# JunweiLiang/Multiverse

Measured on AMD Instinct MI355X. Metric: trajectories/sec (8-obs/12-pred, multi-scale 18x32+9x16 grid, greedy forward), higher is better.
Workload: dtype f16x3 (fp32 operands as two pre-scaled fp16 planes, fp32 accumulate and state; winograd F(3,3) over image rows on pre-transformed operands, 1.67 fp16 MFMAs issued per fp32 product over the gate kernels; error vs fp64 within 2x of the fp32-MFMA path's -- asserted under checkpoint-like dynamic range (; 1 GPU; BASELINE configs[1]: multi-scale 18x32+9x16 (scene 36x64x11), batch 64/GPU, fp32 forward-only, beam 1, obs 8 / pred 12; gate convolution on the fp16 matrix pipe (f16x3 split, fp32-class error); batch_per_gpu=64, global_batch=64, obs_len=8, pred_len=12, parallelism=batch-sharded x1, no data-path collective

## Files before the change

include/multiverse_hip.h:

```cpp
#ifndef MULTIVERSE_HIP_H_
#define MULTIVERSE_HIP_H_

#include <stdint.h>

#ifdef __cplusplus
extern "C" {
#endif

#define MV_MAX_SCALES 2
#define MV_ABI_VERSION 5

typedef struct mv_engine* mv_handle;

typedef struct mv_config {
  int32_t abi_version;
  int32_t batch_size;
  int32_t obs_len;
  int32_t max_pred_len;
  int32_t scene_h, scene_w, scene_class;
  int32_t scene_conv_dim, scene_conv_kernel;
  int32_t emb_size;
  int32_t hidden_size;
  int32_t convlstm_kernel;
  int32_t num_scales;
// ... 140 lines not shown
int  mv_run_score_resident(mv_handle h);
int  mv_download_scores(mv_handle h, mv_score_outputs* out);
int  mv_time_score_resident(mv_handle h, int32_t iters, float* ms_out);

int  mv_train_init(mv_handle h, const mv_train_config* tc);
int  mv_train_step(mv_handle h, const mv_inputs* in, const mv_targets* tg,
                   mv_losses* out);
int  mv_train_forward_backward(mv_handle h, const mv_inputs* in,
                               const mv_targets* tg, mv_losses* out);
int  mv_upload_targets(mv_handle h, const mv_targets* tg);
int  mv_grad_buffer(mv_handle h, float** device_ptr, int64_t* elems);
int  mv_train_apply(mv_handle h, float grad_scale);
#define MV_COMM_ID_BYTES 128
int  mv_comm_unique_id(uint8_t* id_out );
int  mv_allreduce_init(mv_handle h, int32_t rank, int32_t world,
                       const uint8_t* unique_id );
int  mv_allreduce_info(mv_handle h, int32_t* rank, int32_t* world, int32_t* buckets,
                       double* bytes);
int  mv_attack_begin(mv_handle h);
int  mv_attack_end(mv_handle h);
int  mv_set_scene_feat(mv_handle h, const float* scene_feat);
int  mv_get_scene_feat(mv_handle h, float* out);
int  mv_get_scene_grad(mv_handle h, float* out);
int  mv_attack_step(mv_handle h, float epsilon, float step);
int  mv_scene_mix(mv_handle h, const float* other, float weight);
int  mv_get_sample_losses(mv_handle h, int32_t scale, float* out);
int  mv_set_label_mixup(mv_handle h, const int32_t* const* obs_labels2,
                        const int32_t* const* pred_labels2, float weight,
                        const float* sample_weight);
int  mv_clear_label_mixup(mv_handle h);
int  mv_get_grad(mv_handle h, const char* tf_name, float* out, int64_t capacity_elems);
int  mv_get_global_step(mv_handle h, int64_t* step);
int  mv_set_global_step(mv_handle h, int64_t step);
int  mv_set_dropout_seed(mv_handle h, uint32_t seed);
int  mv_get_opt_scalars(mv_handle h, float* beta1_power, float* beta2_power);
int  mv_set_opt_scalars(mv_handle h, float beta1_power, float beta2_power);
int  mv_get_opt_slot(mv_handle h, const char* tf_name, int32_t slot, float* out,
                     int64_t capacity_elems);
int  mv_set_opt_slot(mv_handle h, const char* tf_name, int32_t slot,
                     const float* data, int64_t elems);

int  mv_set_compute_mode(mv_handle h, int32_t mode);

int  mv_set_graph_mode(mv_handle h, int32_t enabled);

int  mv_set_profiling(mv_handle h, int32_t enabled);
int  mv_reset_kernel_stats(mv_handle h);
int  mv_num_kernel_stats(mv_handle h);
int  mv_kernel_stat(mv_handle h, int32_t i, char* name_out, int32_t name_cap,
                    int64_t* launches, double* total_ms, double* flops,
                    double* bytes);
int  mv_kernel_stat_dense_flops(mv_handle h, int32_t i, double* flops_dense);
int  mv_kernel_stat_mfma_flops(mv_handle h, int32_t i, double* flops_mfma);
int  mv_time_greedy_resident(mv_handle h, int32_t iters, float* ms_out);
int  mv_time_beam_resident(mv_handle h, int32_t iters, float* ms_out);

int  mv_op_convlstm_step(int device, const float* x, const float* c,
                         const float* h, const float* kernel,
                         const float* biases, int32_t M, int32_t H, int32_t W,
                         int32_t Cx, int32_t C, float* c_out, float* h_out);
int  mv_op_convlstm_step16(int device, int32_t variant, const float* x, const float* c,
                           const float* h, const float* kernel, const float* biases,
                           int32_t M, int32_t H, int32_t W, int32_t Cx, int32_t C,
                           float* c_out, float* h_out, float* h16_out);
int  mv_op_gnn(int device, const float* h, const float* scene_mean, int32_t M,
               int32_t H, int32_t W, int32_t C, int32_t D, float* out);
int  mv_op_hidden2grid(int device, const float* h, const float* w, int32_t M,
                       int32_t H, int32_t W, int32_t C, int32_t P, float* out);
int  mv_op_beam_step(int device, const float* logits, const float* prev_logprob,
                     int32_t N, int32_t B, int32_t K, int32_t time,
                     int32_t diverse, float gamma, int32_t fix_num_timestep,
                     float* new_logprob, int32_t* ids, int32_t* parents);

int  mv_op_sbs_step(int device, const float* logits, const float* prev_phi,
                    const float* prev_logprob, const float* prev_gumbel, int32_t N, int32_t B,
                    int32_t K, int32_t t, float temperature, uint32_t seed, float* new_phi,
                    float* new_logprob, float* new_gumbel, int32_t* ids, int32_t* parents);

int  mv_op_sample_step(int device, const float* logits , int32_t R, int32_t S,
                       int32_t K, int32_t t, float temperature, uint32_t seed, int32_t top_k,
                       float top_p, int32_t floor, int32_t* ids, float* lp, float* qlp,
                       uint8_t* keep );

int  mv_op_convlstm_bwd(int device, const float* x, const float* c, const float* h,
                        const float* kernel, const float* biases,
                        const float* dh_new, const float* dc_new, int32_t M,
                        int32_t H, int32_t W, int32_t Cx, int32_t C, float* dx,
                        float* dh, float* dc, float* dkernel, float* dbiases);
int  mv_op_gnn_bwd(int device, const float* h, const float* scene_mean,
                   const float* g, int32_t M, int32_t H, int32_t W, int32_t C,
                   int32_t D, float* dh, float* dscene_mean);

#ifdef __cplusplus
}
#endif
#endif
```

multiverse_amd/_lib.py:

```python

from __future__ import annotations

import ctypes as C
import os

import numpy as np

MV_MAX_SCALES = 2
MV_ABI_VERSION = 5

_HERE = os.path.dirname(os.path.abspath(__file__))
LIB_PATH = os.path.join(_HERE, "libmultiverse_hip.so")

EXPORTED_SYMBOLS = [
    "mv_create", "mv_destroy", "mv_last_error", "mv_abi_version",
    "mv_set_param", "mv_get_param", "mv_num_params", "mv_param_info",
    "mv_forward_greedy", "mv_forward_beam",
    "mv_upload_inputs", "mv_run_greedy_resident", "mv_run_beam_resident",
    "mv_synchronize", "mv_download_outputs", "mv_download_beam_outputs",
    "mv_set_graph_mode", "mv_set_compute_mode", "mv_set_profiling", "mv_reset_kernel_stats", "mv_num_kernel_stats",
    "mv_kernel_stat", "mv_kernel_stat_dense_flops", "mv_kernel_stat_mfma_flops",
    "mv_time_greedy_resident",
    "mv_time_beam_resident",
    "mv_op_convlstm_step", "mv_op_convlstm_step16", "mv_op_gnn", "mv_op_hidden2grid", "mv_op_beam_step",
    "mv_train_init", "mv_train_step", "mv_train_forward_backward",
    "mv_upload_targets", "mv_grad_buffer", "mv_train_apply", "mv_get_grad", "mv_get_global_step",
    "mv_set_global_step", "mv_get_opt_slot", "mv_set_opt_slot",
    "mv_set_dropout_seed", "mv_get_opt_scalars", "mv_set_opt_scalars",
    "mv_comm_unique_id", "mv_allreduce_init", "mv_allreduce_info",
    "mv_attack_begin", "mv_attack_end", "mv_set_scene_feat", "mv_get_scene_feat",
    "mv_get_scene_grad", "mv_attack_step", "mv_scene_mix", "mv_get_sample_losses",
    "mv_set_label_mixup", "mv_clear_label_mixup",
    "mv_op_convlstm_bwd", "mv_op_gnn_bwd",
    "mv_set_grid_centers", "mv_upload_inputs_compact", "mv_upload_targets_compact",
    "mv_pipeline_create", "mv_submit_greedy", "mv_collect_greedy",
    "mv_decode_trajectories", "mv_beam_occupancy", "mv_download_beam_ids",
    "mv_set_pred_lengths", "mv_last_forward_gate_rows", "mv_set_sampling",
    "mv_score_futures", "mv_upload_score_futures", "mv_run_score_resident",
    "mv_download_scores", "mv_time_score_resident",
    "mv_set_sampling_mode", "mv_download_beam_gumbels", "mv_op_sbs_step",
    "mv_set_sampling_truncation", "mv_download_beam_proposal_logprobs", "mv_op_sample_step",
]


class MvError(RuntimeError):
  pass


class mv_config(C.Structure):
  _fields_ = [
      ("abi_version", C.c_int32),
      ("batch_size", C.c_int32),
      ("obs_len", C.c_int32),
      ("max_pred_len", C.c_int32),
      ("scene_h", C.c_int32), ("scene_w", C.c_int32), ("scene_class", C.c_int32),
      ("scene_conv_dim", C.c_int32), ("scene_conv_kernel", C.c_int32),
      ("emb_size", C.c_int32),
      ("hidden_size", C.c_int32),
      ("convlstm_kernel", C.c_int32),
      ("num_scales", C.c_int32),
      ("grid_h", C.c_int32 * MV_MAX_SCALES),
      ("grid_w", C.c_int32 * MV_MAX_SCALES),
      ("use_grid", C.c_int32 * MV_MAX_SCALES),
      ("use_gnn", C.c_int32),
      ("beam_size", C.c_int32),
      ("diverse_beam", C.c_int32),
      ("diverse_gamma", C.c_float),
      ("fix_num_timestep", C.c_int32),
      ("class_feedback_dense", C.c_int32),
      ("use_single_decoder", C.c_int32),
      ("simaug_graph", C.c_int32),
      ("activation", C.c_int32),
  ]


_fp = C.POINTER(C.c_float)
_ip = C.POINTER(C.c_int32)


class mv_inputs(C.Structure):
  _fields_ = [
      ("obs_scene", _ip),
      ("scene_feat", _fp),
      ("num_scene_frames", C.c_int32),
      ("pred_len", C.c_int32),
      ("grid_obs_labels", _ip * MV_MAX_SCALES),
      ("grid_obs_regress", _fp * MV_MAX_SCALES),
  ]


_dp = C.POINTER(C.c_double)
_u8p = C.POINTER(C.c_uint8)


class mv_inputs_compact(C.Structure):
  _fields_ = [
      ("obs_scene", _ip),
      ("scene_feat_u8", _u8p),
      ("num_scene_frames", C.c_int32),
      ("pred_len", C.c_int32),
      ("grid_obs_labels", _ip * MV_MAX_SCALES),
      ("obs_xy", _dp),
      ("num_rows", C.c_int32),
  ]


class mv_targets_compact(C.Structure):
  _fields_ = [
      ("grid_pred_labels", _ip * MV_MAX_SCALES),
      ("pred_xy", _dp),
      ("num_rows", C.c_int32),
  ]


class mv_outputs(C.Structure):
  _fields_ = [
      ("grid_pred_class", _fp * MV_MAX_SCALES),
      ("grid_pred_reg", _fp * MV_MAX_SCALES),
  ]


class mv_beam_outputs(C.Structure):
  _fields_ = [
      ("best_beam", _fp), ("grid_reg", _fp), ("logits", _fp), ("ids", _ip),
# ... 14 lines not shown
      ("optimizer", C.c_int32),
      ("init_lr", C.c_float), ("emb_lr", C.c_float),
      ("use_cosine_lr", C.c_int32),
      ("has_decay", C.c_int32), ("learning_rate_decay", C.c_float),
      ("decay_steps", C.c_int32), ("max_steps", C.c_int32),
      ("do_clip", C.c_int32), ("clip_gradient_norm", C.c_float),
      ("wd", C.c_float),
      ("grid_loss_weight", C.c_float), ("grid_reg_loss_weight", C.c_float),
      ("class_feedback", C.c_int32), ("reg_teacher_forcing", C.c_int32),
      ("use_soft_grid_class", C.c_int32), ("soft_kernel_size", C.c_int32),
      ("soft_kernel", C.c_float * 25),
      ("mask_grid_regression", C.c_int32), ("keep_prob", C.c_float),
  ]


class mv_targets(C.Structure):
  _fields_ = [
      ("grid_pred_labels", _ip * MV_MAX_SCALES),
      ("grid_pred_regress", _fp * MV_MAX_SCALES),
  ]


class mv_losses(C.Structure):
  _fields_ = [
      ("loss", C.c_float), ("wd_loss", C.c_float),
      ("pred_grid_loss", C.c_float * (2 * MV_MAX_SCALES)),
      ("num_pred_grid_loss", C.c_int32),
  ]


_lib = None


def load():
  global _lib
  if _lib is not None:
    return _lib
  path = os.environ.get("MV_LIB_PATH", LIB_PATH)
  if not os.path.exists(path):
    raise MvError(
        "%s not found: the HIP extension has not been built "
        "(run `python -c 'import __graft_entry__ as g; g.build()'`). "
        "There is no CPU fallback." % LIB_PATH)
  lib = C.CDLL(path)
  h = C.c_void_p
  lib.mv_last_error.restype = C.c_char_p
  lib.mv_last_error.argtypes = [h]
  lib.mv_abi_version.argtypes = []
  lib.mv_create.argtypes = [C.POINTER(mv_config), C.c_int, C.POINTER(h)]
  lib.mv_destroy.argtypes = [h]
  lib.mv_set_param.argtypes = [h, C.c_char_p, _fp, C.POINTER(C.c_int64), C.c_int32]
  lib.mv_get_param.argtypes = [h, C.c_char_p, _fp, C.c_int64]
  lib.mv_num_params.argtypes = [h]
  lib.mv_param_info.argtypes = [h, C.c_int32, C.c_char_p, C.c_int32,
                                C.POINTER(C.c_int64)]
  lib.mv_forward_greedy.argtypes = [h, C.POINTER(mv_inputs), C.POINTER(mv_outputs)]
  lib.mv_forward_beam.argtypes = [h, C.POINTER(mv_inputs),
                                  C.POINTER(mv_beam_outputs)]
  lib.mv_upload_inputs.argtypes = [h, C.POINTER(mv_inputs)]
  lib.mv_pipeline_create.argtypes = [h, C.c_int32]
  lib.mv_submit_greedy.argtypes = [h, C.POINTER(mv_inputs)]
  lib.mv_collect_greedy.argtypes = [h, C.POINTER(mv_outputs), C.POINTER(C.c_int32)]
  lib.mv_set_grid_centers.argtypes = [h, C.c_int32, _dp]
  lib.mv_upload_inputs_compact.argtypes = [h, C.POINTER(mv_inputs_compact)]
  lib.mv_upload_targets_compact.argtypes = [h, C.POINTER(mv_targets_compact)]
  lib.mv_run_greedy_resident.argtypes = [h]
  lib.mv_run_beam_resident.argtypes = [h]
  lib.mv_synchronize.argtypes = [h]
  lib.mv_download_outputs.argtypes = [h, C.POINTER(mv_outputs)]
  lib.mv_download_beam_outputs.argtypes = [h, C.POINTER(mv_beam_outputs)]
  lib.mv_decode_trajectories.argtypes = [h, C.c_int32, C.c_int32, _dp]
  lib.mv_beam_occupancy.argtypes = [h, _fp]
  lib.mv_download_beam_ids.argtypes = [h, _ip, _fp]
  lib.mv_set_pred_lengths.argtypes = [h, _ip]
  lib.mv_last_forward_gate_rows.argtypes = [h, C.POINTER(C.c_int64)]
  lib.mv_set_sampling.argtypes = [h, C.c_int32, C.c_float, C.c_uint32]
  lib.mv_set_sampling_mode.argtypes = [h, C.c_int32]
  lib.mv_download_beam_gumbels.argtypes = [h, _fp]
  lib.mv_set_sampling_truncation.argtypes = [h, C.c_int32, C.c_float]
  lib.mv_download_beam_proposal_logprobs.argtypes = [h, _fp]
  lib.mv_op_sample_step.argtypes = [C.c_int, _fp, C.c_int32, C.c_int32, C.c_int32, C.c_int32,
                                    C.c_float, C.c_uint32, C.c_int32, C.c_float, C.c_int32,
                                    _ip, _fp, _fp, _u8p]
  lib.mv_op_sbs_step.argtypes = [C.c_int, _fp, _fp, _fp, _fp, C.c_int32, C.c_int32, C.c_int32,
                                 C.c_int32, C.c_float, C.c_uint32, _fp, _fp, _fp, _ip, _ip]
  lib.mv_score_futures.argtypes = [h, C.POINTER(mv_inputs), C.POINTER(mv_score_futures_in),
                                   C.POINTER(mv_score_outputs)]
  lib.mv_upload_score_futures.argtypes = [h, C.POINTER(mv_score_futures_in)]
  lib.mv_run_score_resident.argtypes = [h]
  lib.mv_download_scores.argtypes = [h, C.POINTER(mv_score_outputs)]
  lib.mv_time_score_resident.argtypes = [h, C.c_int32, _fp]
  lib.mv_set_profiling.argtypes = [h, C.c_int32]
  lib.mv_set_graph_mode.argtypes = [h, C.c_int32]
  lib.mv_set_compute_mode.argtypes = [h, C.c_int32]
  lib.mv_reset_kernel_stats.argtypes = [h]
  lib.mv_num_kernel_stats.argtypes = [h]
  lib.mv_kernel_stat.argtypes = [h, C.c_int32, C.c_char_p, C.c_int32,
                                 C.POINTER(C.c_int64), C.POINTER(C.c_double),
                                 C.POINTER(C.c_double), C.POINTER(C.c_double)]
  lib.mv_kernel_stat_dense_flops.argtypes = [h, C.c_int32, C.POINTER(C.c_double)]
  lib.mv_kernel_stat_mfma_flops.argtypes = [h, C.c_int32, C.POINTER(C.c_double)]
  lib.mv_time_greedy_resident.argtypes = [h, C.c_int32, _fp]
  lib.mv_time_beam_resident.argtypes = [h, C.c_int32, _fp]
  lib.mv_op_convlstm_step.argtypes = [C.c_int, _fp, _fp, _fp, _fp, _fp] + \
      [C.c_int32] * 5 + [_fp, _fp]
  lib.mv_op_convlstm_step16.argtypes = [C.c_int, C.c_int32, _fp, _fp, _fp, _fp, _fp] + \
      [C.c_int32] * 5 + [_fp, _fp, _fp]
  lib.mv_op_gnn.argtypes = [C.c_int, _fp, _fp] + [C.c_int32] * 5 + [_fp]
  lib.mv_op_hidden2grid.argtypes = [C.c_int, _fp, _fp] + [C.c_int32] * 5 + [_fp]
  lib.mv_op_beam_step.argtypes = [C.c_int, _fp, _fp, C.c_int32, C.c_int32,
                                  C.c_int32, C.c_int32, C.c_int32, C.c_float,
                                  C.c_int32, _fp, _ip, _ip]
  lib.mv_train_init.argtypes = [h, C.POINTER(mv_train_config)]
  lib.mv_train_step.argtypes = [h, C.POINTER(mv_inputs), C.POINTER(mv_targets),
                                C.POINTER(mv_losses)]
  lib.mv_train_forward_backward.argtypes = lib.mv_train_step.argtypes
  lib.mv_upload_targets.argtypes = [h, C.POINTER(mv_targets)]
  lib.mv_grad_buffer.argtypes = [h, C.POINTER(_fp), C.POINTER(C.c_int64)]
  lib.mv_train_apply.argtypes = [h, C.c_float]
  lib.mv_get_grad.argtypes = [h, C.c_char_p, _fp, C.c_int64]
  lib.mv_get_global_step.argtypes = [h, C.POINTER(C.c_int64)]
  lib.mv_set_global_step.argtypes = [h, C.c_int64]
  lib.mv_comm_unique_id.argtypes = [_u8p]
  lib.mv_allreduce_init.argtypes = [h, C.c_int32, C.c_int32, _u8p]
  lib.mv_allreduce_info.argtypes = [h, _ip, _ip, _ip, _dp]
  lib.mv_attack_begin.argtypes = [h]
  lib.mv_attack_end.argtypes = [h]
  lib.mv_set_scene_feat.argtypes = [h, _fp]
  lib.mv_get_scene_feat.argtypes = [h, _fp]
  lib.mv_get_scene_grad.argtypes = [h, _fp]
  lib.mv_attack_step.argtypes = [h, C.c_float, C.c_float]
  lib.mv_scene_mix.argtypes = [h, _fp, C.c_float]
  lib.mv_get_sample_losses.argtypes = [h, C.c_int32, _fp]
  lib.mv_set_label_mixup.argtypes = [h, C.POINTER(_ip), C.POINTER(_ip), C.c_float, _fp]
  lib.mv_clear_label_mixup.argtypes = [h]
  lib.mv_set_dropout_seed.argtypes = [h, C.c_uint32]
  lib.mv_get_opt_scalars.argtypes = [h, _fp, _fp]
  lib.mv_set_opt_scalars.argtypes = [h, C.c_float, C.c_float]
  lib.mv_get_opt_slot.argtypes = [h, C.c_char_p, C.c_int32, _fp, C.c_int64]
  lib.mv_set_opt_slot.argtypes = [h, C.c_char_p, C.c_int32, _fp, C.c_int64]
  lib.mv_op_convlstm_bwd.argtypes = [C.c_int] + [_fp] * 7 + [C.c_int32] * 5 + [_fp] * 5
  lib.mv_op_gnn_bwd.argtypes = [C.c_int, _fp, _fp, _fp] + [C.c_int32] * 5 + [_fp, _fp]
  if lib.mv_abi_version() != MV_ABI_VERSION:
    raise MvError("ABI version mismatch: library %d, binding %d"
                  % (lib.mv_abi_version(), MV_ABI_VERSION))
  _lib = lib
  return lib


def f32(a):
  return np.ascontiguousarray(a, dtype=np.float32)


def i32(a):
  return np.ascontiguousarray(a, dtype=np.int32)


def fptr(a):
  return a.ctypes.data_as(_fp) if a is not None else _fp()


def iptr(a):
  return a.ctypes.data_as(_ip) if a is not None else _ip()


def check(rc, handle=None):
# ... 771 lines not shown
  lib = load()
  x = f32(x)
  M, H, W, Cx = x.shape
  Cc = int(kernel.shape[3]) // 4
  kernel, biases = f32(kernel), f32(biases)
  c_out = np.empty((M, H, W, Cc), dtype=np.float32)
  h_out = np.empty((M, H, W, Cc), dtype=np.float32)
  if c is None:
    cp, hp = _fp(), _fp()
  else:
    c, h = f32(c), f32(h)
    cp, hp = fptr(c), fptr(h)
  check(lib.mv_op_convlstm_step(device, fptr(x), cp, hp, fptr(kernel), fptr(biases),
                                M, H, W, Cx, Cc, fptr(c_out), fptr(h_out)))
  return c_out, h_out


def op_convlstm_step16(x, c, h, kernel, biases, variant, device=0):
  lib = load()
  x = f32(x)
  M, H, W, Cx = x.shape
  Cc = int(kernel.shape[3]) // 4
  kernel, biases = f32(kernel), f32(biases)
  c_out = np.empty((M, H, W, Cc), dtype=np.float32)
  h_out = np.empty((M, H, W, Cc), dtype=np.float32)
  h16 = np.empty((M, H, W, Cc), dtype=np.float32)
  if c is None:
    cp, hp = _fp(), _fp()
  else:
    c, h = f32(c), f32(h)
    cp, hp = fptr(c), fptr(h)
  check(lib.mv_op_convlstm_step16(device, int(variant), fptr(x), cp, hp, fptr(kernel),
                                  fptr(biases), M, H, W, Cx, Cc, fptr(c_out), fptr(h_out),
                                  fptr(h16)))
  return c_out, h_out, h16


def op_gnn(h, scene_mean, device=0):
  lib = load()
  h, scene_mean = f32(h), f32(scene_mean)
  M, H, W, Cc = h.shape
  out = np.empty_like(h)
  check(lib.mv_op_gnn(device, fptr(h), fptr(scene_mean), M, H, W, Cc,
                      scene_mean.shape[-1], fptr(out)))
  return out


def op_hidden2grid(h, w, device=0):
  lib = load()
  h, w = f32(h), f32(w)
  M, H, W, Cc = h.shape
  P = w.shape[-1]
  out = np.empty((M, H, W, P), dtype=np.float32)
  check(lib.mv_op_hidden2grid(device, fptr(h), fptr(w), M, H, W, Cc, P, fptr(out)))
  return out


def op_beam_step(logits, prev_lp, time, diverse, gamma, fix_num_timestep, device=0):
  lib = load()
  logits, prev_lp = f32(logits), f32(prev_lp)
  N, B, K = logits.shape
  new_lp = np.empty((N, B), dtype=np.float32)
  ids = np.empty((N, B), dtype=np.int32)
  parents = np.empty((N, B), dtype=np.int32)
  check(lib.mv_op_beam_step(device, fptr(logits), fptr(prev_lp), N, B, K, int(time),
                            1 if diverse else 0, float(gamma), int(fix_num_timestep),
                            fptr(new_lp), iptr(ids), iptr(parents)))
  return new_lp, ids, parents


def op_sbs_step(logits, prev_phi, prev_lp, prev_g, t, temperature=1.0, seed=0, device=0):
  lib = load()
  logits, prev_phi, prev_lp, prev_g = f32(logits), f32(prev_phi), f32(prev_lp), f32(prev_g)
  N, B, K = logits.shape
  phi, lp, g = (np.empty((N, B), dtype=np.float32) for _ in range(3))
  ids = np.empty((N, B), dtype=np.int32)
  parents = np.empty((N, B), dtype=np.int32)
  check(lib.mv_op_sbs_step(device, fptr(logits), fptr(prev_phi), fptr(prev_lp), fptr(prev_g),
                           N, B, K, int(t), float(temperature), int(seed) & 0xFFFFFFFF,
                           fptr(phi), fptr(lp), fptr(g), iptr(ids), iptr(parents)))
  return phi, lp, g, ids, parents


def op_sample_step(logits, S, t, temperature=1.0, seed=0, top_k=0, top_p=1.0, floor=1, device=0):
  lib = load()
  logits = f32(logits)
  R, K = logits.shape
  ids = np.empty(R, dtype=np.int32)
  lp, qlp = (np.empty(R, dtype=np.float32) for _ in range(2))
  keep = np.empty((R, K), dtype=np.uint8)
  check(lib.mv_op_sample_step(device, fptr(logits), R, int(S), K, int(t), float(temperature),
                              int(seed) & 0xFFFFFFFF, int(top_k), float(top_p), int(floor),
                              iptr(ids), fptr(lp), fptr(qlp), keep.ctypes.data_as(_u8p)))
  return ids, lp, qlp, keep.astype(bool)


def op_convlstm_bwd(x, c, h, kernel, biases, dh_new, dc_new, device=0):
  lib = load()
  x = f32(x)
  M, H, W, Cx = x.shape
  Cc = int(kernel.shape[3]) // 4
  kernel, biases = f32(kernel), f32(biases)
  dh_new, dc_new = f32(dh_new), f32(dc_new)
  if c is None:
    cp, hp = _fp(), _fp()
  else:
    c, h = f32(c), f32(h)
    cp, hp = fptr(c), fptr(h)
  dx = np.empty((M, H, W, Cx), dtype=np.float32)
  dh = np.empty((M, H, W, Cc), dtype=np.float32)
  dc = np.empty((M, H, W, Cc), dtype=np.float32)
  dk = np.empty(kernel.shape, dtype=np.float32)
  db = np.empty(biases.shape, dtype=np.float32)
  check(lib.mv_op_convlstm_bwd(device, fptr(x), cp, hp, fptr(kernel), fptr(biases),
                               fptr(dh_new), fptr(dc_new), M, H, W, Cx, Cc, fptr(dx),
                               fptr(dh), fptr(dc), fptr(dk), fptr(db)))
  return dx, dh, dc, dk, db


def op_gnn_bwd(h, scene_mean, g, device=0):
  lib = load()
  h, scene_mean, g = f32(h), f32(scene_mean), f32(g)
  M, H, W, Cc = h.shape
  dh = np.empty_like(h)
  ds = np.empty_like(scene_mean)
  check(lib.mv_op_gnn_bwd(device, fptr(h), fptr(scene_mean), fptr(g), M, H, W, Cc,
                          scene_mean.shape[-1], fptr(dh), fptr(ds)))
  return dh, ds
```

multiverse_amd/csrc/convlstm_mfma.h:

```cpp
#pragma once
#include <hip/hip_runtime.h>
#include <stdint.h>

#include <vector>

namespace mv {

typedef float f32x16 __attribute__((ext_vector_type(16)));
typedef float f32x4 __attribute__((ext_vector_type(4)));

constexpr int kBN = 128;
constexpr int kBK = 32;
constexpr int kChBlock = 32;
constexpr int kWaveRows = 32;
constexpr int kBlockRows = 128;
constexpr int kMaxGroup = 4;

struct ConvLstmArgs {
  const float* x;
  const float* h;
  const float* c;
  const int32_t* src_row_h;
  const int32_t* src_row_c;
  const float* wpack;
  const float* bias;
  float* h_out;
  float* c_out;
  float* gates_out;
  float* out0;
  float* out1;
  int32_t out0_cols, out1_cols;
  int32_t n_colblocks;
  int32_t ng_last;
  int32_t rows, H, W, Cx, C;
  int32_t x_row_stride;
  int32_t n_xchunks;
  int32_t n_hchunks;
  int32_t w_chunks;
  int32_t x_small;
  int32_t zero_state;
  float forget_bias;
  int32_t want_h16;
  int32_t skip_h32;
  const float* sx_bias;
  const float* sx_corr;
  const int32_t* sx_hot;
  const uint32_t* sx_cellyx;
  int32_t sx_hot_stride, sx_hot_div, sx_rad, sx_by_class;
};

struct ConvLstmGroup {
  ConvLstmArgs p[kMaxGroup];
  int32_t block_end[kMaxGroup];
  int32_t n;
};

static inline int convlstm_xchunks(int Cx) {
  if (Cx == 0) return 0;
  if (9 * Cx <= kBK) return 1;
  return 9 * (Cx / kBK);
}
static inline bool convlstm_cx_supported(int Cx) {
  return Cx == 0 || 9 * Cx <= kBK || (Cx % kBK) == 0;
}
static inline size_t convlstm_wpack_elems(int Cx, int C) {
  const size_t nch = (size_t)convlstm_xchunks(Cx) + 9 * (size_t)(C / kBK);
  return (size_t)(C / kChBlock) * nch * kBN * kBK;
}

static inline void pack_convlstm_weights(const float* w, int Cx, int C, float* out) {
  const int Cin = Cx + C, N4 = 4 * C;
  const int nx = convlstm_xchunks(Cx), nh = 9 * (C / kBK), nch = nx + nh;
  const bool small = (Cx > 0 && 9 * Cx <= kBK);
  for (int cb = 0; cb < C / kChBlock; ++cb)
    for (int q = 0; q < nch; ++q) {
      float* tile = out + ((size_t)cb * nch + q) * kBN * kBK;
      for (int kk = 0; kk < 4; ++kk)
        for (int g = 0; g < 4; ++g)
          for (int l = 0; l < 64; ++l)
            for (int j = 0; j < 4; ++j) {
              const int k = kk * 8 + (l >> 5) * 4 + j;
              const int n = g * C + cb * kChBlock + (l & 31);
              int tap = -1, ci = -1;
              if (q < nx) {
                if (small) {
                  if (k < 9 * Cx) { tap = k / Cx; ci = k % Cx; }
                } else {
                  tap = q % 9; ci = (q / 9) * kBK + k;
                }
              } else {
                const int qq = q - nx;
                tap = qq % 9; ci = Cx + (qq / 9) * kBK + k;
              }
              tile[((kk * 4 + g) * 64 + l) * 4 + j] =
                  (tap < 0) ? 0.f : w[((size_t)tap * Cin + ci) * N4 + n];
            }
    }
}

__device__ __forceinline__ float sigm_(float v) {
  const float e = __builtin_amdgcn_exp2f(-1.4426950408889634f * v);
  return __builtin_amdgcn_rcpf(1.0f + e);
}
__device__ __forceinline__ float tanh_(float v) {
  const float e = __builtin_amdgcn_exp2f(-2.8853900817779268f * __builtin_fabsf(v));
  const float t = (1.0f - e) * __builtin_amdgcn_rcpf(1.0f + e);
  return __builtin_copysignf(t, v);
}

template <int NG>
struct ConvFrag {
  f32x4 a;
  f32x4 b[NG];
  uint32_t ok;
};

constexpr int kEpiLstm = 0;
constexpr int kEpiStore = 1;

template <int EPI, int NG>
__device__ __forceinline__ void convlstm_step_body(const ConvLstmArgs& a, int block) {
  const int tid = threadIdx.x;
  const int lane = tid & 63;
  const int wave = tid >> 6;
  const int ncb = a.n_colblocks;
  const int cb = block % ncb;
  const int mt = block / ncb;
  const int H = a.H, W = a.W, HW = H * W, C = a.C, Cx = a.Cx;
  const int M_total = a.rows * HW;
  const int nx = a.n_xchunks;
  const int nchunks = nx + a.n_hchunks;
// ... 271 lines not shown
```

multiverse_amd/csrc/convlstm_wino3.h:

```cpp
#pragma once
#include "convlstm_wino.h"

namespace mv {

template <int NRB>
struct Wn3 {
  static constexpr int kCh = 8 * NRB;
  static constexpr int kChunkVec = 5 * 3 * 2 * NRB * 64;
  static constexpr uint32_t kChunkBytes = kChunkVec * 16;
  static constexpr int kTileFloats = 96 * kCh;
};

static inline size_t wino3_wpack_elems(int Cx16, int C, int nrb) {
  return (size_t)(C / (8 * nrb)) * (size_t)(Cx16 / 16 + C / 16) * 5 * 3 * 2 * nrb * 64 * 8;
}

__global__ void pack_wino3_kernel(const float* __restrict__ w, _Float16* __restrict__ out,
                                  int Cx_total, int Cx16, int C, int nrb, size_t total) {
  const size_t idx = (size_t)blockIdx.x * blockDim.x + threadIdx.x;
  if (idx >= total) return;
  const int e = idx & 7;
  const int l = (idx >> 3) & 63;
  size_t t = idx >> 9;
  const int rb = (int)(t % nrb); t /= nrb;
  const int dx = (int)(t % 3); t /= 3;
  const int comp = (int)(t % 5); t /= 5;
  const int nxc = Cx16 / 16, nch = nxc + C / 16;
  const int chunk = (int)(t % nch), cb = (int)(t / nch);
  const bool is_x = chunk < nxc;
  const int cg = is_x ? chunk : chunk - nxc;
  const int k = 8 * (l >> 5) + e;
  const int cin = (is_x ? 0 : Cx_total) + cg * 16 + k;
  const int row = l & 31;
  const int n = (row >> 3) * C + cb * 8 * nrb + rb * 8 + (row & 7);
  const int Cin = Cx_total + C, N4 = 4 * C;
  const double g0 = w[((size_t)(0 * 3 + dx) * Cin + cin) * N4 + n];
  const double g1 = w[((size_t)(1 * 3 + dx) * Cin + cin) * N4 + n];
  const double g2 = w[((size_t)(2 * 3 + dx) * Cin + cin) * N4 + n];
  double u;
  switch (comp) {
    case 0: u = 0.5 * g0; break;
    case 1: u = -0.5 * (g0 + g1 + g2); break;
    case 2: u = (-g0 + g1 - g2) / 6.0; break;
    case 3: u = (g0 + 2.0 * g1 + 4.0 * g2) / 6.0; break;
    default: u = -g2; break;
  }
  const double sv = u * 256.0;
  note_pack_range(sv);
  const _Float16 v0 = (_Float16)sv;
  const _Float16 v1 = (_Float16)(sv - (double)v0);
  const size_t vec = ((((size_t)cb * nch + chunk) * 5 + comp) * 3 + dx) * 2;
  out[(((vec + 0) * nrb + rb) * 64 + l) * 8 + e] = v0;
  out[(((vec + 1) * nrb + rb) * 64 + l) * 8 + e] = v1;
}

struct Wn3Consts { f16x8 m1, p2, m2; };

template <int KA, int KB>
__device__ __forceinline__ void wn_lin(const f16x8 a_hi, const f16x8 a_lo, const f16x8 b_hi,
                                       const f16x8 b_lo, const Wn3Consts& k, f16x8& hi,
                                       f16x8& lo) {
  static_assert((KA == 1 && (KB == 1 || KB == -1 || KB == -2)) || (KA == 2 && KB == 1), "form");
  const f16x8 nka = KA == 1 ? k.m1 : k.m2;
  f16x8 s, ne2, l1;
  if (KA == 2) {
    s = __builtin_elementwise_fma(a_hi, k.p2, b_hi);
    l1 = __builtin_elementwise_fma(a_lo, k.p2, b_lo);
  } else if (KB == 1) {
    s = a_hi + b_hi;
    l1 = a_lo + b_lo;
  } else {
    s = __builtin_elementwise_fma(b_hi, KB == -1 ? k.m1 : k.m2, a_hi);
    l1 = __builtin_elementwise_fma(b_lo, KB == -1 ? k.m1 : k.m2, a_lo);
  }
  const f16x8 bb = __builtin_elementwise_fma(a_hi, nka, s);
  const f16x8 t = __builtin_elementwise_fma(bb, k.m1, s);
  const f16x8 ne1 = __builtin_elementwise_fma(a_hi, nka, t);
  if (KB == -1) ne2 = bb + b_hi;
  else ne2 = __builtin_elementwise_fma(b_hi, KB == 1 ? k.m1 : k.p2, bb);
  hi = s;
  lo = __builtin_elementwise_fma(ne1 + ne2, k.m1, l1);
}

struct Wn3TransformItem {
  const _Float16* p0;
  int64_t pstride;
  _Float16* out;
  const int32_t* src_row;
  int32_t rows, H, W, Cc;
};
constexpr int kW3TrGroup = 8;
struct Wn3TransformGroup {
  Wn3TransformItem it[kW3TrGroup];
  int32_t blk_end[kW3TrGroup];
  int32_t n;
};
static inline size_t wino3_v_elems(int rows, int H, int W, int Cc) {
  const size_t Q = (size_t)rows * ((H + 2) / 3) * W;
  return ((Q + 31) / 32) * (size_t)(Cc / 16) * 5 * 2 * 64 * 8;
}
static inline unsigned wino3_transform_blocks(int rows, int H, int W, int Cc) {
  const size_t Q = (size_t)rows * ((H + 2) / 3) * W;
  return (unsigned)((((Q + 31) / 32) * (size_t)(Cc / 16) + 3) / 4);
}
__global__ __launch_bounds__(256)
void wino3_transform_kernel(const Wn3TransformGroup g) {
  int block = blockIdx.x, pi = 0;
#pragma unroll
  for (int i = 0; i < kW3TrGroup - 1; ++i)
    if (i + 1 < g.n && (int)blockIdx.x >= g.blk_end[i]) pi = i + 1;
  if (pi > 0) block -= g.blk_end[pi - 1];
  const Wn3TransformItem& it = g.it[pi];
  const int lane = threadIdx.x & 63, wave = threadIdx.x >> 6;
  const int KG = it.Cc >> 4;
  const int H = it.H, W = it.W, HW = H * W;
  const int Kt = ((H + 2) / 3) * W, Q_total = it.rows * Kt;
  const int ntile = (Q_total + 31) >> 5;
  const int wid = block * 4 + wave;
  if (wid >= ntile * KG) return;
  const int tile = wid / KG, cg = wid - tile * KG;
  const int col = lane & 31, half = lane >> 5;
  const int q = tile * 32 + col;
  const bool valid = q < Q_total;
  int r = 0, y0 = 0, xpos = 0;
  if (valid) {
    r = q / Kt;
    const int pc = q - r * Kt;
    const int t = pc / W;
    y0 = 3 * t;
    xpos = pc - t * W;
  }
  const int sr = (valid && it.src_row) ? it.src_row[r] : r;
  f16x8 dh[5], dl[5];
#pragma unroll
  for (int i = 0; i < 5; ++i) {
    const int rho = y0 - 1 + i;
    const bool ok = valid & (rho >= 0) & (rho < H);
    const long long m = (long long)sr * HW + rho * W + xpos;
    const size_t o = ((size_t)(m >> 5) * KG + cg) * 512 + (size_t)(half * 256 + (int)(m & 31) * 8);
    const f16x8 z = {0, 0, 0, 0, 0, 0, 0, 0};
    dh[i] = ok ? *reinterpret_cast<const f16x8*>(it.p0 + o) : z;
    dl[i] = ok ? *reinterpret_cast<const f16x8*>(it.p0 + it.pstride + o) : z;
  }
  uint32_t mone = 0xBC00BC00u, ptwo = 0x40004000u, mtwo = 0xC000C000u;
  asm volatile("" : "+s"(mone), "+s"(ptwo), "+s"(mtwo));
  Wn3Consts kc;
  kc.m1 = __builtin_bit_cast(f16x8, u32x4{mone, mone, mone, mone});
  kc.p2 = __builtin_bit_cast(f16x8, u32x4{ptwo, ptwo, ptwo, ptwo});
  kc.m2 = __builtin_bit_cast(f16x8, u32x4{mtwo, mtwo, mtwo, mtwo});
  f16x8 vh[5], vl[5], th, tl, t3h, t3l;
  wn_lin<1, -1>(dh[3], dl[3], dh[1], dl[1], kc, vh[3], vl[3]);
  wn_lin<1, -1>(dh[0], dl[0], dh[2], dl[2], kc, th, tl);
  wn_lin<2, 1>(th, tl, vh[3], vl[3], kc, vh[0], vl[0]);
  wn_lin<1, -1>(dh[3], dl[3], dh[2], dl[2], kc, t3h, t3l);
  wn_lin<1, -2>(t3h, t3l, dh[1], dl[1], kc, vh[1], vl[1]);
  wn_lin<1, -1>(dh[1], dl[1], dh[2], dl[2], kc, th, tl);
  wn_lin<2, 1>(th, tl, t3h, t3l, kc, vh[2], vl[2]);
  wn_lin<1, -1>(dh[2], dl[2], dh[4], dl[4], kc, th, tl);
  wn_lin<2, 1>(vh[3], vl[3], th, tl, kc, vh[4], vl[4]);
  f16x8* o = reinterpret_cast<f16x8*>(it.out) + ((size_t)tile * KG + cg) * (5 * 2 * 64) + lane;
#pragma unroll
  for (int c = 0; c < 5; ++c) {
    o[(c * 2 + 0) * 64] = vh[c];
    o[(c * 2 + 1) * 64] = vl[c];
  }
}
static inline void launch_wino3_transforms(const Wn3TransformItem* items, int n,
                                           hipStream_t stream) {
  for (int i0 = 0; i0 < n; i0 += kW3TrGroup) {
    Wn3TransformGroup g{};
    g.n = n - i0 < kW3TrGroup ? n - i0 : kW3TrGroup;
    unsigned nb = 0;
    for (int j = 0; j < g.n; ++j) {
      g.it[j] = items[i0 + j];
      nb += wino3_transform_blocks(g.it[j].rows, g.it[j].H, g.it[j].W, g.it[j].Cc);
      g.blk_end[j] = (int32_t)nb;
    }
    for (int j = g.n; j < kW3TrGroup; ++j) g.blk_end[j] = (int32_t)nb;
    if (nb) hipLaunchKernelGGL(wino3_transform_kernel, dim3(nb), dim3(256), 0, stream, g);
  }
}

template <int WAVES, int NRB, bool HALO, bool BF16D = false>
__device__ __forceinline__ void convlstm_wino3_body(const ConvLstmWinoArgs& p, int cb, int mt,
                                                    f16x8* lds) {
  using G = Wn3<NRB>;
  constexpr int CH = G::kCh;
  constexpr int kOwn = HALO ? 30 : 32;
  constexpr int kTriples = WAVES * kOwn;
  constexpr int kPieces = CH / 4;
  constexpr int kPasses = (96 * kPieces + 63) / 64;
  const ConvLstm16Args& q = p.b;
  const ConvLstmArgs& a = q.f;
  const int tid = threadIdx.x;
  const int lane = tid & 63;
  const int wave = tid >> 6;
  const int H = a.H, W = a.W, HW = H * W, C = a.C, Cx = a.Cx;
  const int Ht = (H + 2) / 3, Kt = Ht * W;
  const int Q_total = a.rows * Kt;
  const int q_own = mt * kTriples + wave * kOwn;
  const int q_wave = HALO ? q_own - 1 : q_own;
  const bool wave_live = q_own < Q_total;
  const int col = lane & 31, half = lane >> 5;

  int r = 0, y0 = 0, xpos = 0;
  bool valid;
  {
    const int qq = q_wave + col;
    valid = qq >= 0 && qq < Q_total;
    if (valid) {
      r = qq / Kt;
      const int pc = qq - r * Kt;
      const int t = pc / W;
      y0 = 3 * t;
      xpos = pc - t * W;
    }
  }
  const int srh = (valid && a.src_row_h) ? a.src_row_h[r] : r;
  const bool okx0 = valid & (xpos > 0), okx2 = valid & (xpos + 1 < W);

  uint32_t roffx[5], roffh[5];
  {
    const int KGx = Cx >> 4, KGh = C >> 4;
#pragma unroll
    for (int i = 0; i < 5; ++i) {
      const int rho = y0 - 1 + i;
      const bool ok = valid & (rho >= 0) & (rho < H);
      const int cx = r * HW + rho * W + xpos, chh = srh * HW + rho * W + xpos;
      roffx[i] = ok ? (uint32_t)((((cx >> 5) * KGx) * 512 + half * 256 + (cx & 31) * 8 + kPlanePad) * 2) : 0u;
      roffh[i] = ok ? (uint32_t)((((chh >> 5) * KGh) * 512 + half * 256 + (chh & 31) * 8 + kPlanePad) * 2) : 0u;
    }
  }

  constexpr int kAcc = BF16D ? 3 : 5;
  f32x16 acc[kAcc][NRB];
#pragma unroll
  for (int c = 0; c < kAcc; ++c)
#pragma unroll
    for (int rb = 0; rb < NRB; ++rb)
#pragma unroll
      for (int i = 0; i < 16; ++i) acc[c][rb][i] = 0.f;

  constexpr int kStageVec = BF16D ? 3 * 3 * NRB * 64
                                  : 2 * 3 * 2 * NRB * 64;
  constexpr uint32_t kStageBytes = kStageVec * 16;
  static_assert(2 * kStageVec * 16 >= WAVES * G::kTileFloats * 4, "h' tiles fit the stage buffers");
  float* const ctile = reinterpret_cast<float*>(lds + 2 * kStageVec) + wave * G::kTileFloats;
  uint32_t* const otab = reinterpret_cast<uint32_t*>(
      reinterpret_cast<float*>(lds + 2 * kStageVec) + WAVES * G::kTileFloats) + wave * 192;
  constexpr uint32_t kNone = 0xffffffffu;
  const uint32_t rowb = (uint32_t)C * 4u;
  bool okc[3];
  int cell[3];
  const bool owned = valid && (!HALO || (col >= 1 && col <= 30));
#pragma unroll
  for (int e = 0; e < 3; ++e) {
    okc[e] = owned & (y0 + e < H);
    cell[e] = (y0 + e) * W + xpos;
  }
  if (wave_live) {
    const int src_c0 = (valid && a.src_row_c) ? a.src_row_c[r] : r;
#pragma unroll
    for (int e = 0; e < 3; ++e) {
      otab[e * 32 + col] = okc[e] ? (uint32_t)(src_c0 * HW + cell[e]) * rowb : kNone;
      otab[96 + e * 32 + col] = okc[e] ? (uint32_t)(r * HW + cell[e]) * rowb : kNone;
    }
  }
  const uint32_t colb = (uint32_t)(cb * CH) * 4u;
  if (wave_live && !a.zero_state) {
    const __amdgpu_buffer_rsrc_t c_rs0 = __builtin_amdgcn_make_buffer_rsrc(
        uniform_ptr(const_cast<float*>(a.c)), 0, (uint32_t)(a.rows * HW) * rowb, 0x00020000);
#pragma unroll
    for (int k = 0; k < kPasses; ++k) {
      const int i = k * 64 + lane;
      const int trow = i / kPieces, piece = i - trow * kPieces;
      const uint32_t ro = trow < 96 ? otab[trow] : kNone;
      const uint32_t off = ro != kNone ? ro + colb + (uint32_t)piece * 16u : 0u;
      __builtin_amdgcn_raw_ptr_buffer_load_lds(
          c_rs0, (__attribute__((address_space(3))) void*)(ctile + k * 256), 16, off, 0, 0,
          MV_EPI_LD_AUX);
    }
  }

  if (a.x_small && wave_live) {
    const int Cin = Cx + C, N4 = 4 * C;
    const int nk = 9 * Cx;
    const int n0 = (col >> 3) * C + cb * CH + (col & 7);
    for (int k2 = 0; 2 * k2 < nk; ++k2) {
      const int k = 2 * k2 + half;
      const bool kok = k < nk;
      const int tap = kok ? k / Cx : 0, chn = kok ? k - tap * Cx : 0;
      const int dy = tap / 3 - 1, dx = tap - (tap / 3) * 3 - 1;
      float wv[NRB];
#pragma unroll
      for (int rb = 0; rb < NRB; ++rb) {
        const float tw = p.w_hwio[((size_t)tap * Cin + chn) * N4 + n0 + rb * 8];
        wv[rb] = kok ? tw * (BF16D ? 1.0f : 65536.0f) : 0.f;
      }
#pragma unroll
      for (int e = 0; e < 3; ++e) {
        const int yy = y0 + e + dy, xx = xpos + dx;
        const bool ok = kok & valid & (yy >= 0) & (yy < H) & (xx >= 0) & (xx < W);
        const int off = ok ? r * a.x_row_stride + (yy * W + xx) * Cx + chn : 0;
        const float tv = a.x[off];
        const float v = ok ? tv : 0.f;
#pragma unroll
        for (int rb = 0; rb < NRB; ++rb) {
          if constexpr (BF16D) {
            acc[e][rb] = __builtin_amdgcn_mfma_f32_32x32x2f32(wv[rb], v, acc[e][rb], 0, 0, 0);
          } else if (e == 1) {
            acc[1][rb] = __builtin_amdgcn_mfma_f32_32x32x2f32(wv[rb], 0.5f * v, acc[1][rb], 0, 0, 0);
            acc[2][rb] = __builtin_amdgcn_mfma_f32_32x32x2f32(wv[rb], -0.5f * v, acc[2][rb], 0, 0, 0);
          } else {
            acc[e == 0 ? 0 : 4][rb] =
                __builtin_amdgcn_mfma_f32_32x32x2f32(wv[rb], v, acc[e == 0 ? 0 : 4][rb], 0, 0, 0);
          }
        }
      }
    }
  }

  const int nxc = p.n_xc;
  const int ck_lo = a.sx_corr ? nxc : 0;
  const int ck_hi = a.zero_state ? nxc : nxc + (C >> 4);
  if constexpr (BF16D) {
    if (ck_hi > ck_lo) {
      constexpr int kChunkVecD = 3 * 3 * NRB * 64;
      constexpr int kPiecesD = 3 * 3 * NRB;
      const f16x8* wblk = reinterpret_cast<const f16x8*>(p.wpw) +
                          ((size_t)cb * (nxc + (C >> 4)) + ck_lo) * kChunkVecD;
      const __amdgpu_buffer_rsrc_t wrs = __builtin_amdgcn_make_buffer_rsrc(
          uniform_ptr(const_cast<f16x8*>(wblk)), 0, 0x7fffffff, 0x00020000);
      const __amdgpu_buffer_rsrc_t xrs = __builtin_amdgcn_make_buffer_rsrc(
          uniform_ptr(const_cast<_Float16*>(q.x16 ? q.x16 - kPlanePad : q.h16 - kPlanePad)), 0,
          0x7fffffff, 0x00020000);
      const __amdgpu_buffer_rsrc_t hrs = __builtin_amdgcn_make_buffer_rsrc(
          uniform_ptr(const_cast<_Float16*>(q.h16 ? q.h16 - kPlanePad : q.x16 - kPlanePad)), 0,
          0x7fffffff, 0x00020000);
      const int wave_u = __builtin_amdgcn_readfirstlane(wave);
      const uint32_t lane16 = (uint32_t)lane * 16u;
      auto stage_dma = [&](int st, f16x8* dstbuf) {
#pragma unroll
        for (int i = 0; i < (kPiecesD + WAVES - 1) / WAVES; ++i) {
          const int piece = i * WAVES + wave_u;
// ... 107 lines not shown
                                          is_x ? vxrs : vhrs, (int)(is_x ? vo_x : vo_h), so + 1024, 0));
    };
#define MV_W3_COMP(COMP, CI, VHI, VLO, BUF)                                                   \
  do {                                                                                        \
    _Pragma("unroll") for (int dx = 0; dx < 3; ++dx) {                                        \
      const bool sh_ = dx != 1;                                                               \
      const f16x8 b0 = !sh_ ? (VHI) : wn_lane_shift((VHI), dx == 0, dx == 0 ? okx0 : okx2);   \
      const f16x8 b1 = !sh_ ? (VLO) : wn_lane_shift((VLO), dx == 0, dx == 0 ? okx0 : okx2);   \
      f16x8 w0[NRB], w1[NRB];                                                                 \
      _Pragma("unroll") for (int rb = 0; rb < NRB; ++rb) {                                    \
        w0[rb] = (BUF)[((((CI) * 3 + dx) * 2 + 0) * NRB + rb) * 64 + lane];                   \
        w1[rb] = (BUF)[((((CI) * 3 + dx) * 2 + 1) * NRB + rb) * 64 + lane];                   \
      }                                                                                       \
      _Pragma("unroll") for (int rb = 0; rb < NRB; ++rb)                                      \
        acc[COMP][rb] = __builtin_amdgcn_mfma_f32_32x32x16_f16(w1[rb], b0, acc[COMP][rb], 0, 0, 0); \
      _Pragma("unroll") for (int rb = 0; rb < NRB; ++rb)                                      \
        acc[COMP][rb] = __builtin_amdgcn_mfma_f32_32x32x16_f16(w0[rb], b1, acc[COMP][rb], 0, 0, 0); \
      _Pragma("unroll") for (int rb = 0; rb < NRB; ++rb)                                      \
        acc[COMP][rb] = __builtin_amdgcn_mfma_f32_32x32x16_f16(w0[rb], b0, acc[COMP][rb], 0, 0, 0); \
    }                                                                                         \
  } while (0)
#define MV_W3_STAGE(CA, CB)                                                                   \
  do {                                                                                        \
    f16x8* const buf = lds + ((st & 1) ? kStageVec : 0);                                      \
    f16x8* const nbuf = lds + ((st & 1) ? 0 : kStageVec);                                     \
    if (st + 1 < S_total) {                                                                   \
      stage_dma(st + 1, nbuf);               \
      vload(2 * st + 2, na); vload(2 * st + 3, nb);                  \
    }                                                                                         \
    MV_W3_COMP(CA, 0, va.h, va.l, buf);                                                       \
    if ((CB) >= 0) MV_W3_COMP((CB) < 0 ? 0 : (CB), 1, vb.h, vb.l, buf);                       \
    va = na; vb = nb;                                                                         \
    ++st;                                                                                     \
    __syncthreads();                       \
  } while (0)

    Vc va, vb, na, nb;
    vload(0, va); vload(1, vb);
    na = va; nb = vb;
    stage_dma(0, lds);
    __syncthreads();
    const int nck = ck_hi - ck_lo;
    int st = 0;
    for (int pr = 0; pr < (nck >> 1); ++pr) {
      MV_W3_STAGE(0, 1); MV_W3_STAGE(2, 3); MV_W3_STAGE(4, 0); MV_W3_STAGE(1, 2); MV_W3_STAGE(3, 4);
    }
    if (nck & 1) {
      MV_W3_STAGE(0, 1); MV_W3_STAGE(2, 3); MV_W3_STAGE(4, -1);
    }
#undef MV_W3_COMP
#undef MV_W3_STAGE
  }
  if (!wave_live) return;

  int lane_e = lane;
  asm volatile("" : "+v"(lane_e));
  const int half_e = lane_e >> 5;
  const int ch0 = cb * CH + 4 * half_e;
  const uint32_t out_bytes = (uint32_t)(a.rows * HW) * rowb;
  const __amdgpu_buffer_rsrc_t co_rs = __builtin_amdgcn_make_buffer_rsrc(
      uniform_ptr(a.c_out), 0, out_bytes, 0x00020000);
  const __amdgpu_buffer_rsrc_t ho_rs = __builtin_amdgcn_make_buffer_rsrc(
      uniform_ptr(a.h_out), 0, out_bytes, 0x00020000);
  const __amdgpu_buffer_rsrc_t go_rs = __builtin_amdgcn_make_buffer_rsrc(
      uniform_ptr(a.gates_out ? a.gates_out : a.h_out), 0, a.gates_out ? 4u * out_bytes : 0u,
      0x00020000);
  float* const tl0 = ctile;
  float* const tl1 = reinterpret_cast<float*>(lds) + wave * G::kTileFloats;
  const int wr_idx = (lane_e & 31) * CH + half_e * 4;
  f32x4 cprev[3][NRB];
#pragma unroll
  for (int e = 0; e < 3; ++e)
#pragma unroll
    for (int rb = 0; rb < NRB; ++rb) cprev[e][rb] = f32x4{0.f, 0.f, 0.f, 0.f};
  if (!a.zero_state) {
    asm volatile("s_waitcnt vmcnt(0)" ::: "memory");
#pragma unroll
    for (int e = 0; e < 3; ++e)
#pragma unroll
      for (int rb = 0; rb < NRB; ++rb)
        cprev[e][rb] = *reinterpret_cast<const f32x4*>(tl0 + wr_idx + e * 32 * CH + rb * 8);
  }
  int hot_y = 0, hot_x = 0;
  if (a.sx_corr) {
    const int hr = a.sx_hot_div > 1 ? r / a.sx_hot_div : r;
    const uint32_t hyx = a.sx_cellyx[a.sx_hot[(size_t)hr * a.sx_hot_stride]];
    hot_y = (int)(hyx >> 16); hot_x = (int)(hyx & 0xffffu);
  }
  const float un = BF16D ? 1.0f : kF16Unscale;
  const bool planes = q.h16_out != nullptr;
  u32x2 ph[3][NRB], pl[3][NRB];
#pragma unroll
  for (int e = 0; e < 3; ++e) {
    const int y = y0 + e;
    const uint32_t mcell = (uint32_t)(r * HW + cell[e]);
#pragma unroll
    for (int rb = 0; rb < NRB; ++rb) {
      const int ch = ch0 + rb * 8;
      f32x4 add[4];
      {
        const float* bsrc = a.bias;
        if (a.sx_corr && a.sx_bias) {
          const int cls = 3 * (y == 0 ? 0 : (y == H - 1 ? 2 : 1)) +
                          (xpos == 0 ? 0 : (xpos == W - 1 ? 2 : 1));
          bsrc = a.sx_bias + (size_t)(okc[e] ? cls : 4) * 4 * C;
        }
#pragma unroll
        for (int g = 0; g < 4; ++g)
          add[g] = *reinterpret_cast<const f32x4*>(bsrc + g * C + ch);
        if (a.sx_corr) {
          const int dy = y - hot_y, dxh = xpos - hot_x, rad = a.sx_rad;
          const bool inr = okc[e] && dy >= -rad && dy <= rad && dxh >= -rad && dxh <= rad;
          const int dyc = dy < -rad ? -rad : (dy > rad ? rad : dy);
          const int dxc = dxh < -rad ? -rad : (dxh > rad ? rad : dxh);
          const int side = 2 * rad + 1;
          const int idx = a.sx_by_class
                              ? 3 * (hot_y == 0 ? 0 : (hot_y == H - 1 ? 2 : 1)) +
                                    (hot_x == 0 ? 0 : (hot_x == W - 1 ? 2 : 1))
                              : (valid ? r : 0);
          const float* ct = a.sx_corr +
              ((size_t)idx * side * side + (dyc + rad) * side + (dxc + rad)) * 4 * C + ch;
          const float keep = inr ? 1.0f : 0.0f;
#pragma unroll
          for (int g = 0; g < 4; ++g) {
            const f32x4 cv = *reinterpret_cast<const f32x4*>(ct + g * C);
            add[g][0] = __builtin_fmaf(cv[0], keep, add[g][0]);
            add[g][1] = __builtin_fmaf(cv[1], keep, add[g][1]);
            add[g][2] = __builtin_fmaf(cv[2], keep, add[g][2]);
            add[g][3] = __builtin_fmaf(cv[3], keep, add[g][3]);
          }
        }
      }
      f32x4 cn4, hn4, si4, tj4, sf4, so4;
#pragma unroll
      for (int j = 0; j < 4; ++j) {
        float pre[4];
#pragma unroll
        for (int g = 0; g < 4; ++g) {
          const int reg = g * 4 + j;
          float yv;
          if constexpr (BF16D) {
            yv = acc[e][rb][reg];
          } else {
            const float m0 = acc[0][rb][reg], m1 = acc[1][rb][reg], m2 = acc[2][rb][reg],
                        m3 = acc[3][rb][reg], m4 = acc[kAcc - 1][rb][reg];
            if (e == 0) yv = (m0 + m1) + (m2 + m3);
            else if (e == 1) yv = (m1 - m2) + 2.0f * m3;
            else yv = (m1 + m2) + (4.0f * m3 + m4);
          }
          pre[g] = __builtin_fmaf(yv, un, add[g][j]);
        }
        const float si = sigm_(pre[0]), tj = tanh_(pre[1]), sf = sigm_(pre[2] + a.forget_bias),
                    so = sigm_(pre[3]);
        float cn = sf * cprev[e][rb][j];
        cn = cn + si * tj;
        const float hn = tanh_(cn) * so;
        cn4[j] = cn; hn4[j] = hn; si4[j] = si; tj4[j] = tj; sf4[j] = sf; so4[j] = so;
      }
      *reinterpret_cast<f32x4*>(tl0 + wr_idx + e * 32 * CH + rb * 8) = cn4;
      if (!a.skip_h32) *reinterpret_cast<f32x4*>(tl1 + wr_idx + e * 32 * CH + rb * 8) = hn4;
      if (a.gates_out && okc[e]) {
        const uint32_t g0 = (mcell * 4u * (uint32_t)C + (uint32_t)ch) * 4u;
        __builtin_amdgcn_raw_buffer_store_b128(__builtin_bit_cast(u32x4, si4), go_rs, (int)g0,
                                               0, MV_EPI_ST_AUX);
        __builtin_amdgcn_raw_buffer_store_b128(__builtin_bit_cast(u32x4, tj4), go_rs,
                                               (int)(g0 + rowb), 0, MV_EPI_ST_AUX);
        __builtin_amdgcn_raw_buffer_store_b128(__builtin_bit_cast(u32x4, sf4), go_rs,
                                               (int)(g0 + 2 * rowb), 0, MV_EPI_ST_AUX);
        __builtin_amdgcn_raw_buffer_store_b128(__builtin_bit_cast(u32x4, so4), go_rs,
                                               (int)(g0 + 3 * rowb), 0, MV_EPI_ST_AUX);
      }
      if (planes) {
        f16x4 p0, p1;
#pragma unroll
        for (int j = 0; j < 4; ++j) {
          if constexpr (BF16D) {
            p0[j] = bf16_as_half(hn4[j]);
            p1[j] = p0[j];
          } else {
            const float sc = hn4[j] * kF16Scale;
            const _Float16 h0 = (_Float16)sc;
            p0[j] = h0;
            p1[j] = (_Float16)(sc - (float)h0);
          }
        }
        ph[e][rb] = __builtin_bit_cast(u32x2, p0);
        pl[e][rb] = __builtin_bit_cast(u32x2, p1);
      }
    }
  }
  asm volatile("s_waitcnt lgkmcnt(0)" ::: "memory");
  {
#pragma unroll
    for (int k = 0; k < kPasses; ++k) {
      const int i = k * 64 + lane_e;
      const int trow = i / kPieces, piece = i - trow * kPieces;
      if (96 * kPieces % 64 == 0 || trow < 96) {
        const uint32_t ro = otab[96 + trow];
        const u32x4 cv = *reinterpret_cast<const u32x4*>(tl0 + i * 4);
        u32x4 hv = cv;
        if (!a.skip_h32) hv = *reinterpret_cast<const u32x4*>(tl1 + i * 4);
        if (ro != kNone) {
// ... 192 lines not shown
```

multiverse_amd/csrc/engine.hip:

```cpp
#include "../../include/multiverse_hip.h"

#include <hip/hip_runtime.h>

#include <cmath>
#include <cstdio>
#include <cstdlib>
#include <cstring>
#include <algorithm>
#include <map>
#include <memory>
#include <mutex>
#include <set>
#include <string>
#include <tuple>
#include <type_traits>
#include <vector>

#include "convlstm_mfma.h"
#include "convlstm_wgrad.h"
#include "convlstm_f16x3.h"
#include "convlstm_wino.h"
#include "convlstm_wino3.h"
#include "convlstm_generic.h"
#include "convlstm_wgrad_f16x3.h"
// ... 773 lines not shown
      HIP_CHECK(hipMemcpy(t.sc[s].pred_labels2.p, pred_labels2[s],
                          (size_t)N * Tp * sizeof(int32_t), hipMemcpyHostToDevice));
    }
    if (sample_weight)
      HIP_CHECK(hipMemcpy(t.sample_w.p, sample_weight, (size_t)N * sizeof(float),
                          hipMemcpyHostToDevice));
    t.mix_on = true; t.mix_sw = sample_weight != nullptr; t.mix_w = weight;
  });
}

int mv_clear_label_mixup(mv_handle h) {
  if (!h || !h->train) return 1;
  TS(h).mix_on = TS(h).mix_sw = false;
  TS(h).mix_w = 1.f;
  return 0;
}

int mv_set_dropout_seed(mv_handle h, uint32_t seed) {
  if (!h || !h->train) return 1;
  h->train->st.dropout_seed = seed;
  return 0;
}

int mv_get_opt_scalars(mv_handle h, float* beta1_power, float* beta2_power) {
  if (!h || !h->train || !beta1_power || !beta2_power) return 1;
  *beta1_power = h->train->st.beta1_power;
  *beta2_power = h->train->st.beta2_power;
  return 0;
}

int mv_set_opt_scalars(mv_handle h, float beta1_power, float beta2_power) {
  if (!h || !h->train) return 1;
  h->train->st.beta1_power = beta1_power;
  h->train->st.beta2_power = beta2_power;
  return 0;
}

int mv_get_opt_slot(mv_handle h, const char* tf_name, int32_t slot, float* out,
                    int64_t capacity) {
  if (!h) return 1;
  return guarded(h, [&] {
    MV_REQUIRE(h->train, "mv_train_init has not been called");
    MV_REQUIRE(slot == 0 || slot == 1, "slot must be 0 or 1 (see multiverse_hip.h)");
    Param* p = find_param(h, tf_name);
    MV_REQUIRE(out && (size_t)capacity >= p->elems(), "buffer too small for %s", tf_name);
    const float* src = (slot == 0 ? TS(h).accum.p : TS(h).accum_update.p) +
                       TS(h).goff[param_index(h, p)];
    HIP_CHECK(hipMemcpy(out, src, p->elems() * sizeof(float), hipMemcpyDeviceToHost));
  });
}

int mv_set_opt_slot(mv_handle h, const char* tf_name, int32_t slot, const float* data,
                    int64_t elems) {
  if (!h) return 1;
  return guarded(h, [&] {
    MV_REQUIRE(h->train, "mv_train_init has not been called");
    MV_REQUIRE(slot == 0 || slot == 1, "slot must be 0 or 1 (see multiverse_hip.h)");
    Param* p = find_param(h, tf_name);
    MV_REQUIRE(data && (size_t)elems == p->elems(), "size mismatch for %s", tf_name);
    float* dst = (slot == 0 ? TS(h).accum.p : TS(h).accum_update.p) +
                 TS(h).goff[param_index(h, p)];
    HIP_CHECK(hipMemcpy(dst, data, p->elems() * sizeof(float), hipMemcpyHostToDevice));
  });
}

int mv_set_compute_mode(mv_handle h, int32_t mode) {
  if (!h) return 1;
  return guarded(h, [&] {
    MV_REQUIRE(mode >= 0 && mode <= 2, "compute mode %d (0 = fp32 MFMA, 1 = f16x3, 2 = bf16)",
               mode);
    MV_REQUIRE(mode == 0 || h->cfg.convlstm_kernel == 3,
               "compute mode %d needs convlstm_kernel 3 (%d given: the matrix-pipe gate kernels "
               "are 3 x 3 stencils; mode 0 runs the generic fp32 loops)", mode,
               h->cfg.convlstm_kernel);
    if (mode != 0) {
      const mv_config& c = h->cfg;
      size_t K = 0;
      for (int s = 0; s < c.num_scales; ++s)
        if (h->sc[s].use) K = std::max(K, (size_t)h->sc[s].K);
      const size_t xc = (size_t)std::max(c.scene_conv_dim, c.emb_size);
      for (int i = 0; i < mv::kMaxGroup; ++i) {
        const size_t rows = (size_t)c.batch_size * ((i % 2 == 0) ? c.beam_size : 1);
        h->px16[i].alloc(2 * (rows * K * xc + mv::kPlaneSlack + mv::kPlanePad));
        h->ph16[i].alloc(2 * (rows * K * c.hidden_size + mv::kPlaneSlack + mv::kPlanePad));
        HIP_CHECK(hipMemset(h->px16[i].p, 0, h->px16[i].n * sizeof(_Float16)));
        if (c.activation != 0) h->xexp[i].alloc(65);
        if (wino3_possible(mode, c.activation)) {
          size_t vx = 0, vh = 0;
          for (int s = 0; s < c.num_scales; ++s) {
            if (!h->sc[s].use) continue;
            vx = std::max(vx, wino3_scratch_elems((int)rows, h->sc[s].H, h->sc[s].W, (int)xc));
            vh = std::max(vh, wino3_scratch_elems((int)rows, h->sc[s].H, h->sc[s].W, c.hidden_size));
          }
          if (vx) h->pv3x[i].alloc(vx);
          if (vh) h->pv3h[i].alloc(vh);
        }
        HIP_CHECK(hipMemset(h->ph16[i].p, 0, h->ph16[i].n * sizeof(_Float16)));
      }
    }
    if (mode != 0 && h->planes.empty()) {
      for (int s = 0; s < h->cfg.num_scales; ++s) {
        ScaleState& S = h->sc[s];
        if (!S.use) continue;
        for (DevBuf<float>* b : {&S.cls_h[0], &S.cls_h[1], &S.reg_h[0], &S.reg_h[1],
                                 &S.cls_hg, &S.xbuf_cls, &S.xbuf_reg}) {
          if (!b->p) continue;
          h->plane_store.emplace_back(new DevBuf<_Float16>());
          DevBuf<_Float16>& pb = *h->plane_store.back();
          pb.alloc(2 * (b->n + mv::kPlaneSlack + mv::kPlanePad));
          HIP_CHECK(hipMemset(pb.p, 0, pb.n * sizeof(_Float16)));
          h->planes[b->p] = mv_engine::PlaneBuf{pb.p + mv::kPlanePad,
                                                b->n + mv::kPlaneSlack + mv::kPlanePad, false};
          if (b == &S.xbuf_cls || b == &S.xbuf_reg) h->xbufs.insert(b->p);
        }
      }
    }
    for (auto& kv : h->planes) kv.second.valid = false;
    if (h->compute_mode != mode) {
      h->drop_graphs();
      h->train_packs_valid = false;
    }
    h->compute_mode = mode;
  });
}

int mv_set_graph_mode(mv_handle h, int32_t enabled) {
  if (!h) return 1;
  h->graph_mode = enabled != 0;
  return 0;
}

int mv_reset_kernel_stats(mv_handle h) {
  if (!h) return 1;
  return guarded(h, [&] {
    HIP_CHECK(hipStreamSynchronize(h->stream));
    drain_events(h);
    h->stats.clear();
  });
}

int mv_num_kernel_stats(mv_handle h) { return h ? (int)h->stats.size() : -1; }

int mv_kernel_stat_dense_flops(mv_handle h, int32_t i, double* flops_dense) {
  if (!h || i < 0 || i >= (int)h->stats.size() || !flops_dense) return 1;
  *flops_dense = h->stats[i].flops_dense;
  return 0;
}

int mv_kernel_stat_mfma_flops(mv_handle h, int32_t i, double* flops_mfma) {
  if (!h || i < 0 || i >= (int)h->stats.size() || !flops_mfma) return 1;
  *flops_mfma = h->stats[i].flops_mfma;
  return 0;
}

int mv_kernel_stat(mv_handle h, int32_t i, char* name_out, int32_t name_cap,
                   int64_t* launches, double* total_ms, double* flops, double* bytes) {
  if (!h || i < 0 || i >= (int)h->stats.size()) return 1;
  const KernelStat& s = h->stats[i];
  if (name_out && name_cap > 0) {
    strncpy(name_out, s.name.c_str(), name_cap - 1);
    name_out[name_cap - 1] = 0;
  }
  if (launches) *launches = s.launches;
  if (total_ms) *total_ms = s.total_ms;
  if (flops) *flops = s.flops;
  if (bytes) *bytes = s.bytes;
  return 0;
}

static int time_resident(mv_handle h, int32_t iters, float* ms_out, ForwardKind kind) {
  return guarded(h, [&] {
    MV_REQUIRE(iters >= 1 && ms_out, "bad arguments");
    struct Event {
      hipEvent_t ev = nullptr;
      ~Event() { if (ev) (void)hipEventDestroy(ev); }
// ... 26 lines not shown
```

multiverse_amd/csrc/engine_forward.h:

```cpp
#pragma once

namespace {


using mv::ConvLstmArgs;

void set_sparse_x(mv_engine* e, ScaleState& S, ConvLstmArgs& a, bool decoder,
                  const int32_t* hot, int hot_stride, int hot_div) {
  a.sx_bias = decoder ? S.sx_dec_bias.p : nullptr;
  a.sx_corr = decoder ? S.sx_dec_corr.p : S.sx_enc_corr.p;
  a.sx_hot = hot; a.sx_hot_stride = hot_stride; a.sx_hot_div = hot_div;
  a.sx_cellyx = S.sx_cellyx.p;
  a.sx_rad = decoder ? 2 : 1;
  a.sx_by_class = decoder ? 1 : 0;
}

ConvLstmArgs conv_problem(mv_engine* e, const ConvCell& cc, const float* x,
                          const float* h, const float* c, const int32_t* src_row_h,
                          const int32_t* src_row_c, float* h_out, float* c_out,
                          int rows, int H, int W, bool zero_state,
                          size_t x_row_stride = 0, bool want_h16 = true) {
  ConvLstmArgs a{};
  const size_t xrs = x_row_stride ? x_row_stride : (size_t)H * W * cc.Cx;
  MV_REQUIRE((size_t)rows * H * W * e->cfg.hidden_size < ((size_t)1 << 31) &&
// ... 61 lines not shown
    q.n_xk = a.x_small ? 0 : xpass * mv::f16x3_xksteps(a.Cx);
    q.n_hk = a.zero_state ? 0 : 9 * (a.C / 16);
    q.w_ksteps = (a.x_small ? 0 : xpass * mv::f16x3_xksteps(a.Cx)) + 9 * (a.C / 16);
    if (bf16)
      MV_REQUIRE((q.n_xk / 3) % MV_BF16_UNITS == 0 && (q.n_hk / 3) % MV_BF16_UNITS == 0,
                 "bf16 mode: %d x / %d h k-steps do not fill whole LDS stages (emb_size and "
                 "scene_conv_dim must be multiples of 32)", q.n_xk, q.n_hk);
    q.x16 = nullptr; q.h16 = nullptr;
    q.x_plane_stride = q.h_plane_stride = 0;
    q.h16_out = nullptr;
    q.h16_out_stride = 0;
    e->plane_invalidate(a.h_out);
    if (gate_knobs().epi_planes && a.want_h16 && !a.gates_out) {
      size_t pst = 0;
      if (_Float16* po = e->plane_out(a.h_out, &pst)) {
        q.h16_out = po;
        q.h16_out_stride = (int64_t)pst;
      }
    }
    q.f.skip_h32 = (a.skip_h32 && q.h16_out && !e->train) ? 1 : 0;
    if (has_dense_x(a)) {
      MV_REQUIRE((size_t)a.x_row_stride == (size_t)a.H * a.W * a.Cx,
                 "internal: f16x3 needs a contiguous x operand");
      if (const auto* pb = ready(a.x)) {
        q.x16 = pb->p; q.x_plane_stride = (int64_t)pb->n;
      } else {
        const size_t pst = ncell * a.Cx + mv::kPlaneSlack + mv::kPlanePad;
        MV_REQUIRE(e->px16[sl].n >= 2 * pst, "internal: f16x3 x plane scratch");
        _Float16* p0 = e->px16[sl].p + mv::kPlanePad;
        q.x16 = p0; q.x_plane_stride = (int64_t)pst;
        if (e->dyn_x()) {
          MV_REQUIRE(e->xexp[sl].p, "internal: x exponent scratch");
          q.x_exp = e->xexp[sl].p + 64;
          dyn_splits.push_back(DynItem{a.x, p0, p0 + pst, (int)ncell, a.Cx, e->xexp[sl].p});
        } else {
          splits.push_back(SplitItem{a.x, p0, bf16 ? (_Float16*)nullptr : p0 + pst, (int)ncell, a.Cx});
        }
      }
      MV_REQUIRE(!(bf16 && e->dyn_x()) || q.x_exp, "internal: bf16 mode, unbounded activations: "
                 "a dense x operand came as producer planes, without its exponent");
    }
    if (!a.zero_state) {
      if (const auto* pb = ready(a.h)) {
        q.h16 = pb->p; q.h_plane_stride = (int64_t)pb->n;
      } else {
        const size_t pst = ncell * a.C + mv::kPlaneSlack + mv::kPlanePad;
        MV_REQUIRE(e->ph16[sl].n >= 2 * pst, "internal: f16x3 h plane scratch");
        _Float16* p0 = e->ph16[sl].p + mv::kPlanePad;
        q.h16 = p0; q.h_plane_stride = (int64_t)pst;
        splits.push_back(SplitItem{a.h, p0, bf16 ? (_Float16*)nullptr : p0 + pst, (int)ncell, a.C});
      }
    }
  }
  for (const DynItem& it : dyn_splits) {
    launch(e, "split_planes", 0, 12.0 * (double)it.cells * it.C, [&] {
      HIP_CHECK(hipMemsetAsync(it.bits, 0, 64 * sizeof(int32_t), e->issue));
      hipLaunchKernelGGL(mv::absmax_bits_kernel, dim3(256), dim3(256), 0, e->issue, it.in,
                         (size_t)it.cells * it.C, it.bits);
      hipLaunchKernelGGL(mv::split_planes_dyn_kernel,
                         dim3(mv::split_planes_blocks((size_t)it.cells, it.C)), dim3(256), 0,
                         e->issue, it.in, it.p0, it.p1, it.cells, it.C, it.bits, it.bits + 64);
    });
  }
  for (size_t s0 = 0; s0 < splits.size(); s0 += mv::kSplitGroup) {
    mv::SplitGroup g{};
    double sbytes = 0;
    unsigned nb = 0;
    g.n = (int)std::min<size_t>(mv::kSplitGroup, splits.size() - s0);
    for (int j = 0; j < g.n; ++j) {
      const SplitItem& it = splits[s0 + j];
      g.in[j] = it.in; g.p0[j] = it.p0; g.p1[j] = it.p1; g.M[j] = it.cells; g.C[j] = it.C;
      nb += mv::split_planes_blocks((size_t)it.cells, it.C);
      g.blk_end[j] = nb;
      sbytes += (bf16 ? 6.0 : 8.0) * (double)it.cells * it.C;
    }
    launch(e, "split_planes", 0, sbytes, [&] {
      hipLaunchKernelGGL(mv::split_planes_group_kernel, dim3(nb), dim3(256), 0, e->issue, g);
    });
  }
}

double queue_wino3_transform(std::vector<mv::Wn3TransformItem>& tr, const mv::Wn3TransformItem& it) {
  tr.push_back(it);
  return (double)it.rows * it.H * it.W * it.Cc * 4.0 * (1.0 + 5.0 / 3.0);
}

void launch_gate_group(const ForwardPlan& pl, const mv::ConvLstm16Args* p16,
                       const _Float16* const* packs, const float* const* w_hwio,
                       _Float16* const* v3x, _Float16* const* v3h, int n, hipStream_t stream) {
  if (pl.form == GateForm::Direct16)
    return mv::launch_convlstm16_steps(p16, n, pl.shift, pl.map_mode, stream);
  if (pl.form == GateForm::Bf16)
    return mv::launch_convlstm_bf16_steps(p16, n, pl.shift, pl.map_mode, pl.x_passes == 3, stream);
  mv::ConvLstmWinoArgs pw[mv::kMaxGroup] = {};
  for (int i = 0; i < n; ++i) {
    pw[i].b = p16[i];
    pw[i].wpw = packs[i];
    pw[i].w_hwio = w_hwio[i];
    pw[i].n_xc = p16[i].f.x_small ? 0 : p16[i].f.Cx / 16;
    pw[i].v3x = v3x ? v3x[i] : nullptr;
    pw[i].v3h = v3h ? v3h[i] : nullptr;
  }
  if (pl.form == GateForm::Wino2) mv::launch_convlstm_wino_steps(pw, n, pl.map_mode, stream);
  else if (pl.form == GateForm::Wino3)
    mv::launch_convlstm_wino3_steps(pw, n, pl.halo, pl.map_mode, stream);
  else mv::launch_convlstm_bf16t_steps(pw, n, pl.halo, pl.map_mode, stream);
}

struct GatePrep {
  std::vector<ConvCell*> cells;
  std::vector<mv::ConvLstm16Args> p16;
  int slot0 = 0;
  double flops = 0, bytes = 0, dense = 0;
  int n() const { return (int)p16.size(); }
};

void gate_group_cost(const std::vector<ConvLstmArgs>& probs, double& flops, double& bytes,
                     double& dense) {
  flops = bytes = dense = 0;
  for (const auto& a : probs) {
    const double M = (double)a.rows * a.H * a.W;
    dense += 2.0 * M * 9.0 * (a.Cx + a.C) * 4.0 * a.C;
    const double cx = a.sx_corr ? 0.0 : (double)a.Cx;
    flops += 2.0 * M * 9.0 * (cx + (a.zero_state ? 0 : a.C)) * 4.0 * a.C;
    bytes += M * (cx + (a.zero_state ? 2.0 : 4.0) * a.C) * 4.0;
  }
}

GatePrep prepare_gate_group(mv_engine* e, const std::vector<ConvLstmArgs>& probs) {
  GatePrep g;
  const int n = (int)probs.size();
  MV_REQUIRE(e->slot0 + n <= mv::kMaxGroup, "internal: gate group of %d problems from slot %d",
             n, e->slot0);
  g.slot0 = e->slot0;
  g.cells.resize(n);
  for (int i = 0; i < n; ++i) g.cells[i] = cell_of_pack(e, probs[i].wpack);
  g.p16.resize(n);
  prepare_gate_operands(e, probs, g.cells, g.p16);
  gate_group_cost(probs, g.flops, g.bytes, g.dense);
  return g;
}

ForwardPlan plan_gate_groups(mv_engine* e, const GatePrep* const* groups, int ngroups) {
  ForwardProblem fp[mv::kMaxGroup];
  int n = 0;
  for (int g = 0; g < ngroups; ++g)
    for (int i = 0; i < groups[g]->n(); ++i) {
      MV_REQUIRE(n < mv::kMaxGroup, "internal: more than %d gate problems in a step", mv::kMaxGroup);
      const int sl = groups[g]->slot0 + i;
      fp[n++] = ForwardProblem{&groups[g]->p16[i], groups[g]->cells[i], e->pv3x[sl].n, e->pv3h[sl].n};
    }
  return plan_forward_group(e->compute_mode, fp, n);
}

void issue_gate_group(mv_engine* e, const GatePrep& g, const ForwardPlan& pl) {
  const int n = g.n();
  const _Float16* packs[mv::kMaxGroup] = {};
  const float* w_hwio[mv::kMaxGroup] = {};
  _Float16 *v3x[mv::kMaxGroup] = {}, *v3h[mv::kMaxGroup] = {};
  std::vector<mv::Wn3TransformItem> tr3;
  double tr3_bytes = 0;
  for (int i = 0; i < n; ++i) {
    const mv::ConvLstm16Args& q = g.p16[i];
    const ConvLstmArgs& a = q.f;
    const int sl = g.slot0 + i;
    w_hwio[i] = g.cells[i]->kernel->dev.p;
    packs[i] = pl.form == GateForm::Wino2 ? g.cells[i]->wpw.p
             : pl.form == GateForm::Wino3 ? g.cells[i]->wpw3.p
             : pl.form == GateForm::Bf16T ? g.cells[i]->wpbt.p : nullptr;
    if (pl.form != GateForm::Wino3) continue;
    if (!a.zero_state) {
      v3h[i] = e->pv3h[sl].p;
      tr3_bytes += queue_wino3_transform(tr3, {q.h16, q.h_plane_stride, v3h[i], a.src_row_h,
                                               a.rows, a.H, a.W, a.C});
    }
    if (has_dense_x(a)) {
      v3x[i] = e->pv3x[sl].p;
      tr3_bytes += queue_wino3_transform(tr3, {q.x16, q.x_plane_stride, v3x[i], nullptr,
                                               a.rows, a.H, a.W, a.Cx});
    }
  }
  if (!tr3.empty())
    launch(e, "wino3_transform", 0, tr3_bytes, [&] {
      mv::launch_wino3_transforms(tr3.data(), (int)tr3.size(), e->issue);
    });
  for (int i = 0; i < n; ++i) e->gate_rows += g.p16[i].f.rows;
  launch(e, "convlstm_step", g.flops, g.bytes, [&] {
    launch_gate_group(pl, g.p16.data(), packs, w_hwio, v3x, v3h, n, e->issue);
  }, g.dense, pl.mfma_factor);
}

void run_conv_group_f16x3(mv_engine* e, const std::vector<ConvLstmArgs>& probs) {
  const GatePrep g = prepare_gate_group(e, probs);
  const GatePrep* gp = &g;
  issue_gate_group(e, g, plan_gate_groups(e, &gp, 1));
}

void run_conv_group(mv_engine* e, const std::vector<ConvLstmArgs>& probs) {
  if (probs.empty()) return;
  if (e->compute_mode != 0) {
    run_conv_group_f16x3(e, probs);
    return;
  }
  double flops = 0, bytes = 0, dense = 0;
  gate_group_cost(probs, flops, bytes, dense);
  for (const auto& a : probs) e->gate_rows += a.rows;
  if (e->cfg.convlstm_kernel != 3) {
    const double kk = (double)e->cfg.convlstm_kernel * e->cfg.convlstm_kernel / 9.0;
    launch(e, "convlstm_step", flops * kk, bytes, [&] {
      for (const auto& a : probs) {
        mv::ConvGenericArgs ga{};
        ga.f = a;
        ga.w = cell_of_bias(e, a.bias)->kernel->dev.p;
        ga.ksize = e->cfg.convlstm_kernel;
        mv::launch_convlstm_generic_step(ga, e->issue);
      }
    }, dense * kk, 0.0);
    return;
  }
  launch(e, "convlstm_step", flops, bytes, [&] {
    mv::launch_convlstm_steps(probs.data(), (int)probs.size(), e->issue);
  }, dense, 1.0);
}

void run_conv_pairs(mv_engine* e, const std::vector<ConvLstmArgs>& a,
                    const std::vector<ConvLstmArgs>& b) {
  if (e->compute_mode == 0 || a.empty() || b.empty()) {
    { IssueOn on(e, 0); run_conv_group(e, a); }
    { IssueOn on(e, 1); run_conv_group(e, b); }
    return;
  }
  MV_REQUIRE(a.size() <= 2 && b.size() <= 2, "internal: chain pairs of %zu / %zu problems",
             a.size(), b.size());
  GatePrep ga, gb;
  { IssueOn on(e, 0); ga = prepare_gate_group(e, a); }
  { IssueOn on(e, 1); gb = prepare_gate_group(e, b); }
  const GatePrep* both[2] = {&gb, &ga};
  const ForwardPlan pl = plan_gate_groups(e, both, 2);
  { IssueOn on(e, 0); issue_gate_group(e, ga, pl); }
  { IssueOn on(e, 1); issue_gate_group(e, gb, pl); }
}

void run_scene(mv_engine* e) {
  const mv_config& c = e->cfg;
  const int U = e->num_frames;
  const float* in = e->scene_feat.p;
  int Hi = c.scene_h, Wi = c.scene_w, Ci = c.scene_class;
  const int k = c.scene_conv_kernel;
  for (int i = 0; i < c.num_scales; ++i) {
    const int Ho = e->conv_h[i], Wo = e->conv_w[i], Co = c.scene_conv_dim;
    const int pad_h = std::max((Ho - 1) * 2 + k - Hi, 0);
    const int pad_w = std::max((Wo - 1) * 2 + k - Wi, 0);
    const size_t total = (size_t)U * Ho * Wo * Co;
    float* out = e->scene_conv[i].p;
    const float *w = e->scene_W[i]->dev.p, *b = e->scene_b[i]->dev.p;
    if (k == 1 && Co <= 64) {
      const size_t M = (size_t)U * Ho * Wo;
      launch(e, "scene_proj1x1_mfma", 2.0 * M * Ci * Co,
             4.0 * (total + (double)M * Ci), [&] {
        hipLaunchKernelGGL(mv::scene_proj1x1_mfma_kernel, dim3(cdiv(M, 128)), dim3(256), 0,
                           e->issue, in, w, b, out, U, Hi, Wi, Ci, Ho, Wo, Co, c.activation);
      });
    } else {
    launch(e, "scene_conv_s2_tanh", 2.0 * total * k * k * Ci,
           4.0 * (total + (double)U * Hi * Wi * Ci), [&] {
      hipLaunchKernelGGL(mv::scene_conv_s2_tanh_kernel, dim3(cdiv(total, 256)),
                         dim3(256), 0, e->issue, in, w, b, out, U, Hi, Wi, Ci,
                         Ho, Wo, Co, k, pad_h / 2, pad_w / 2, c.activation);
    });
    }
    in = out; Hi = Ho; Wi = Wo; Ci = Co;
  }
  for (int s = 0; s < c.num_scales; ++s) {
    ScaleState& S = e->sc[s];
    if (!S.use) continue;
    const int rows = e->rows_at(0);
    const size_t total = (size_t)rows * S.K * c.scene_conv_dim;
    launch(e, "scene_mean", (double)total * c.obs_len,
           4.0 * total * (c.obs_len + 1), [&] {
      hipLaunchKernelGGL(mv::scene_mean_kernel, dim3(cdiv(total, 256)), dim3(256),
                         0, e->issue, e->scene_conv[s].p, e->obs_scene.p,
                         S.scene_mean.p, rows, c.obs_len, S.K,
                         c.scene_conv_dim);
    });
  }
}

struct Cursors {
  int cls[MV_MAX_SCALES] = {0, 0};
  int reg[MV_MAX_SCALES] = {0, 0};
};

static bool beam_shared_first() {
  static const bool on =
      !(getenv("MV_BEAM_SHARED_FIRST") && atoi(getenv("MV_BEAM_SHARED_FIRST")) == 0);
  return on;
}

enum : int { kChainCls = 1, kChainReg = 2, kChainAll = 3 };

void encoder_step_problems(mv_engine* e, Cursors& cur, int t, int chains,
                           std::vector<ConvLstmArgs>& probs) {
  const mv_config& c = e->cfg;
  const int N = e->rows_at(0), Nb = c.batch_size, T = c.obs_len, D = c.scene_conv_dim;
  for (int s = 0; s < c.num_scales; ++s) {
    {
      ScaleState& S = e->sc[s];
      if (!S.use) continue;
      if (chains & kChainCls) {
      const size_t total = (size_t)N * S.K * D;
      const bool sparse = sparse_x_on(e, S);
      const size_t nc = (size_t)Nb * 9 * 4 * c.hidden_size;
      if (e->no_scene()) {
        if (!sparse) {
          const int E = S.enc_cls.Cx;
          const size_t tx = (size_t)N * S.K * E;
          launch(e, "enc_grid_emb_onehot", (double)tx, 4.0 * tx, [&] {
            size_t pst = 0;
            _Float16* p16 = e->plane_out(S.xbuf_cls.p, &pst);
            hipLaunchKernelGGL(mv::enc_grid_emb_onehot_kernel, dim3(cdiv(tx, 256)), dim3(256),
                               0, e->issue, S.labels.p, T, t, 1, e->enc_emb_W->dev.p,
                               e->enc_emb_b->dev.p, S.xbuf_cls.p, N, S.H, S.W, E, p16, pst,
                               c.activation);
          });
        }
      } else if (sparse) {
        if (t == 0)
          launch(e, "sx_encoder_corr", 2.0 * nc * D * T, 4.0 * nc * T, [&] {
            hipLaunchKernelGGL(mv::sx_encoder_corr_kernel,
                               dim3(cdiv((size_t)4 * c.hidden_size, 256), 9,
                                    cdiv((size_t)Nb, mv::kSxRows) * T),
                               dim3(256), 0, e->issue, S.enc_cls.kernel->dev.p,
                               e->scene_conv[s].p, e->obs_scene.p, S.labels.p, Nb, T, -1, S.K, D,
                               c.hidden_size, S.sx_enc_corr.p);
          });
      } else {
      launch(e, "enc_class_input", 0, 4.0 * total, [&] {
        size_t pst = 0;
        _Float16* p16 = e->plane_out(S.xbuf_cls.p, &pst);
        hipLaunchKernelGGL(mv::enc_class_input_kernel, dim3(cdiv(total, 256)),
                           dim3(256), 0, e->issue, e->scene_conv[s].p,
                           e->obs_scene.p, S.labels.p, S.xbuf_cls.p, N, T, t, S.K, D, p16,
                           pst);
      });
      }
      const int cc = cur.cls[s];
      probs.push_back(conv_problem(e, S.enc_cls, S.xbuf_cls.p, S.cls_h[cc].p,
                                   S.cls_c[cc].p, nullptr, nullptr, S.cls_h[cc ^ 1].p,
                                   S.cls_c[cc ^ 1].p, N, S.H, S.W, t == 0, 0,
                                   t + 1 < T || !c.use_gnn));
      probs.back().skip_h32 =
          (t + 1 < T || (!c.use_gnn && (c.beam_size == 1 || beam_shared_first()))) ? 1 : 0;
      if (sparse && e->no_scene()) {
        set_sparse_x(e, S, probs.back(), true, S.labels.p + t, T, 1);
        probs.back().sx_bias = S.sx_enc_bias.p;
        probs.back().sx_corr = S.sx_enc_tab.p;
      } else if (sparse) {
        set_sparse_x(e, S, probs.back(), false, S.labels.p + t, T, 1);
        probs.back().sx_corr = S.sx_enc_corr.p + (size_t)t * nc;
      }
      cur.cls[s] ^= 1;
      }
      if (!(chains & kChainReg)) continue;
      const size_t row = (size_t)S.K * 2;
      const int cr = cur.reg[s];
      if (!c.use_single_decoder)
        probs.push_back(conv_problem(e, S.enc_reg, S.obs_reg.p + (size_t)t * row,
                                     S.reg_h[cr].p, S.reg_c[cr].p, nullptr, nullptr,
                                     S.reg_h[cr ^ 1].p, S.reg_c[cr ^ 1].p, N, S.H, S.W,
                                     t == 0, (size_t)T * row));
      if (!c.use_single_decoder) probs.back().skip_h32 = 1;
      cur.reg[s] ^= 1;
    }
  }
}

void run_encoders(mv_engine* e, Cursors& cur, bool pairs) {
  for (int t = 0; t < e->cfg.obs_len; ++t) {
    if (!pairs) {
      std::vector<ConvLstmArgs> probs;
      encoder_step_problems(e, cur, t, kChainAll, probs);
      run_conv_group(e, probs);
      continue;
    }
    std::vector<ConvLstmArgs> pa, pb;
    { IssueOn on(e, 0); encoder_step_problems(e, cur, t, kChainCls, pa); }
    { IssueOn on(e, 1); encoder_step_problems(e, cur, t, kChainReg, pb); }
    run_conv_pairs(e, pa, pb);
  }
}

static int gnn_version() {
  const char* v = getenv("MV_GNN");
  if (v && strcmp(v, "v1") == 0) return 1;
  if (v && strcmp(v, "v2") == 0) return 2;
  return 3;
}

struct GnnJob {
  ScaleState* S; const float* h; const int32_t* src_row; float* out; int rows, sm_div;
  const int32_t* row_ref = nullptr;
};

void run_gnn_jobs(mv_engine* e, const std::vector<GnnJob>& jobs) {
  const mv_config& c = e->cfg;
  static const int env_ver = gnn_version();
  const size_t max_rows = (size_t)c.batch_size * (size_t)std::max(1, c.beam_size);
  auto v3_ok = [&](const GnnJob& J) {
    return (gnn_scene_dim(e) == 0 || gnn_scene_dim(e) == 64) &&
           max_rows * J.S->K * c.hidden_size * 4 < ((size_t)1 << 32);
  };
  for (size_t j0 = 0; j0 < jobs.size();) {
    const GnnJob& A = jobs[j0];
    const bool tiled = env_ver >= 2 && A.S->W <= 32 && c.hidden_size == 256 && c.scene_conv_dim <= 64;
    size_t nj = 1;
    if (tiled && j0 + 1 < jobs.size() && jobs[j0 + 1].S->W <= 32) nj = 2;
    const int ver = env_ver >= 3 && !(v3_ok(A) && (nj == 1 || v3_ok(jobs[j0 + 1]))) ? 2 : env_ver;
    mv::GnnGroup grp{};
    double flops = 0, bytes = 0;
    unsigned nblocks = 0;
    for (size_t j = 0; j < nj; ++j) {
      const GnnJob& J = jobs[j0 + j];
      const size_t cells = (size_t)J.rows * J.S->K;
      size_t pst = 0;
      _Float16* p16 = e->plane_out(J.out, &pst);
      const bool need_f32 = !(tiled && p16 && !e->train && e->compute_mode != 0);
      flops += cells * (9.0 * 2 * 2 * (c.hidden_size + gnn_scene_dim(e)) +
                        9.0 * 2 * c.hidden_size);
      bytes += 4.0 * cells * c.hidden_size *
                   (1.0 + (need_f32 ? 1.0 : 0.0) + (p16 ? 1.0 : 0.0)) +
               4.0 * (cells / J.sm_div) * gnn_scene_dim(e);
      int ng = 0;
      const unsigned nb = ver >= 3 ? mv::gnn_v3_blocks(cells, &ng) : mv::gnn_v2_blocks(cells, &ng);
// ... 792 lines not shown
```

multiverse_amd/csrc/engine_io.h:

```cpp
#pragma once

namespace {

void check_inputs(const mv_engine* e, int num_scene_frames, int pred_len,
                  const int32_t* obs_scene, int num_rows = 0) {
  const mv_config& c = e->cfg;
  const size_t N = c.batch_size, T = c.obs_len;
  const bool scene = !e->no_scene();
  MV_REQUIRE(!scene || (num_scene_frames >= 1 && (size_t)num_scene_frames <= N * T),
             "num_scene_frames %d not in [1, N*T_o=%zu]", num_scene_frames, N * T);
  MV_REQUIRE(pred_len >= 1 && pred_len <= c.max_pred_len,
             "pred_len %d not in [1, max_pred_len=%d]", pred_len, c.max_pred_len);
  MV_REQUIRE(num_rows >= 0 && (size_t)num_rows <= N, "num_rows %d not in [0, N=%zu]",
             num_rows, N);
  for (size_t i = 0; scene && i < N * T; ++i)
    MV_REQUIRE(obs_scene[i] >= 0 && obs_scene[i] < num_scene_frames,
               "obs_scene[%zu] = %d out of range [0,%d)", i, obs_scene[i], num_scene_frames);
}

void check_labels(const mv_engine* e, int s, const int32_t* labels) {
  const size_t NT = (size_t)e->cfg.batch_size * e->cfg.obs_len;
  const int K = e->sc[s].K;
  for (size_t i = 0; i < NT; ++i)
    MV_REQUIRE(labels[i] >= 0 && labels[i] < K,
               "grid_obs_labels[%d][%zu] = %d out of range [0,%d)", s, i, labels[i], K);
}

void upload_inputs(mv_engine* e, const mv_inputs* in) {
  const mv_config& c = e->cfg;
  const size_t N = c.batch_size, T = c.obs_len;
  const bool scene = !e->no_scene();
  MV_REQUIRE(!scene || (in->obs_scene && in->scene_feat), "obs_scene / scene_feat is NULL");
  check_inputs(e, in->num_scene_frames, in->pred_len, in->obs_scene);
  e->num_frames = scene ? in->num_scene_frames : 0;
  e->pred_len = in->pred_len;
  if (scene) {
    HIP_CHECK(hipMemcpyAsync(e->obs_scene.p, in->obs_scene, N * T * sizeof(int32_t),
                             hipMemcpyHostToDevice, e->stream));
    HIP_CHECK(hipMemcpyAsync(e->scene_feat.p, in->scene_feat,
                             (size_t)e->num_frames * c.scene_h * c.scene_w *
                                 c.scene_class * sizeof(float),
                             hipMemcpyHostToDevice, e->stream));
  }
  for (int s = 0; s < c.num_scales; ++s) {
    ScaleState& S = e->sc[s];
    if (!S.use) continue;
    MV_REQUIRE(in->grid_obs_labels[s] && in->grid_obs_regress[s],
               "grid_obs_labels/grid_obs_regress[%d] is NULL for an enabled scale", s);
    check_labels(e, s, in->grid_obs_labels[s]);
    HIP_CHECK(hipMemcpyAsync(S.labels.p, in->grid_obs_labels[s],
                             N * T * sizeof(int32_t), hipMemcpyHostToDevice, e->stream));
    HIP_CHECK(hipMemcpyAsync(S.obs_reg.p, in->grid_obs_regress[s],
                             N * T * S.K * 2 * sizeof(float), hipMemcpyHostToDevice,
                             e->stream));
  }
  HIP_CHECK(hipStreamSynchronize(e->stream));
  e->inputs_ready = true;
}

void upload_inputs_compact(mv_engine* e, const mv_inputs_compact* in) {
  const mv_config& c = e->cfg;
  const size_t N = c.batch_size, T = c.obs_len;
  const bool scene = !e->no_scene();
  MV_REQUIRE(in->obs_xy && (!scene || (in->obs_scene && in->scene_feat_u8)),
             "obs_scene / scene_feat_u8 / obs_xy is NULL");
  check_inputs(e, in->num_scene_frames, in->pred_len, in->obs_scene, in->num_rows);
  e->num_frames = scene ? in->num_scene_frames : 0;
  e->pred_len = in->pred_len;
  if (scene) {
    HIP_CHECK(hipMemcpyAsync(e->obs_scene.p, in->obs_scene, N * T * sizeof(int32_t),
                             hipMemcpyHostToDevice, e->stream));
    const size_t nscene = (size_t)e->num_frames * c.scene_h * c.scene_w * c.scene_class;
    e->scene_u8.alloc(N * T * c.scene_h * c.scene_w * c.scene_class);
    HIP_CHECK(hipMemcpyAsync(e->scene_u8.p, in->scene_feat_u8, nscene, hipMemcpyHostToDevice,
                             e->stream));
    hipLaunchKernelGGL(mv::u8_to_f32_kernel, dim3(cdiv(nscene, 256)), dim3(256), 0,
                       e->stream, e->scene_u8.p, e->scene_feat.p, nscene);
  }
  e->xy_dev.alloc(2 * N * std::max<size_t>(T, c.max_pred_len));
  HIP_CHECK(hipMemcpyAsync(e->xy_dev.p, in->obs_xy, 2 * N * T * sizeof(double),
                           hipMemcpyHostToDevice, e->stream));
  for (int s = 0; s < c.num_scales; ++s) {
    ScaleState& S = e->sc[s];
    if (!S.use) continue;
    MV_REQUIRE(in->grid_obs_labels[s], "grid_obs_labels[%d] is NULL for an enabled scale", s);
    MV_REQUIRE(S.centers.p, "mv_set_grid_centers(%d) has not been called", s);
    check_labels(e, s, in->grid_obs_labels[s]);
    HIP_CHECK(hipMemcpyAsync(S.labels.p, in->grid_obs_labels[s],
                             N * T * sizeof(int32_t), hipMemcpyHostToDevice, e->stream));
    hipLaunchKernelGGL(mv::regress_from_xy_kernel, dim3(cdiv(N * T * S.K, 256)), dim3(256), 0,
                       e->stream, e->xy_dev.p, S.centers.p, S.obs_reg.p, (int)(N * T), (int)T,
                       S.K, in->num_rows);
  }
  HIP_CHECK(hipStreamSynchronize(e->stream));
  e->inputs_ready = true;
}

void download_outputs(mv_engine* e, mv_outputs* out) {
  const mv_config& c = e->cfg;
  const size_t N = c.batch_size, Tp = e->pred_len;
  for (int s = 0; s < c.num_scales; ++s) {
    ScaleState& S = e->sc[s];
    if (!S.use) continue;
    if (out->grid_pred_class[s])
      HIP_CHECK(hipMemcpyAsync(out->grid_pred_class[s], S.out_cls.p,
                               N * Tp * S.K * sizeof(float), hipMemcpyDeviceToHost,
                               e->stream));
    if (out->grid_pred_reg[s])
      HIP_CHECK(hipMemcpyAsync(out->grid_pred_reg[s], S.out_reg.p,
                               N * Tp * S.K * 2 * sizeof(float), hipMemcpyDeviceToHost,
                               e->stream));
  }
  HIP_CHECK(hipStreamSynchronize(e->stream));
}

struct PipeLayout {
  size_t obs_scene = 0, scene_feat = 0, labels[MV_MAX_SCALES] = {0, 0},
         obs_reg[MV_MAX_SCALES] = {0, 0}, in_bytes = 0;
  size_t out_cls[MV_MAX_SCALES] = {0, 0}, out_reg[MV_MAX_SCALES] = {0, 0}, out_bytes = 0;
};
static PipeLayout pipe_layout(const mv_engine* e) {
  const mv_config& c = e->cfg;
  const size_t N = c.batch_size, T = c.obs_len, Tp = c.max_pred_len;
  auto al = [](size_t v) { return (v + 255) & ~(size_t)255; };
  PipeLayout L;
  size_t o = 0;
  L.obs_scene = o; o = al(o + N * T * sizeof(int32_t));
  const size_t frames = e->no_scene() ? 0 : N * T;
  L.scene_feat = o; o = al(o + frames * c.scene_h * c.scene_w * c.scene_class * sizeof(float));
  for (int s = 0; s < c.num_scales; ++s) {
    if (!e->sc[s].use) continue;
    const size_t K = e->sc[s].K;
    L.labels[s] = o; o = al(o + N * T * sizeof(int32_t));
    L.obs_reg[s] = o; o = al(o + N * T * K * 2 * sizeof(float));
  }
  L.in_bytes = o;
  for (int s = 0; s < c.num_scales; ++s) {
    if (!e->sc[s].use) continue;
    const size_t K = e->sc[s].K;
    L.out_cls[s] = o; o = al(o + N * Tp * K * sizeof(float));
    L.out_reg[s] = o; o = al(o + N * Tp * K * 2 * sizeof(float));
  }
  L.out_bytes = o - L.in_bytes;
  return L;
}

void pipeline_create(mv_engine* e, int depth) {
  MV_REQUIRE(depth >= 1 && depth <= 8, "pipeline depth %d not in [1, 8]", depth);
  MV_REQUIRE(e->cfg.beam_size == 1, "the pipelined forward is the greedy one");
  MV_REQUIRE(e->pipe.empty(), "pipeline already created");
  const PipeLayout L = pipe_layout(e);
  HIP_CHECK(hipStreamCreateWithFlags(&e->copy_stream, hipStreamNonBlocking));
  HIP_CHECK(hipStreamCreateWithFlags(&e->fetch_stream, hipStreamNonBlocking));
  e->pipe.resize(depth);
  for (auto& sl : e->pipe) {
    sl.in_bytes = L.in_bytes; sl.out_bytes = L.out_bytes;
    HIP_CHECK(hipHostMalloc(&sl.pin, L.in_bytes + L.out_bytes, hipHostMallocDefault));
    HIP_CHECK(hipMalloc((void**)&sl.dev, L.in_bytes + L.out_bytes));
    HIP_CHECK(hipEventCreateWithFlags(&sl.h2d, hipEventDisableTiming));
    HIP_CHECK(hipEventCreateWithFlags(&sl.done, hipEventDisableTiming));
    HIP_CHECK(hipEventCreateWithFlags(&sl.d2h, hipEventDisableTiming));
  }
  e->pipe_head = e->pipe_tail = 0;
}

void pipeline_destroy(mv_engine* e) {
  for (auto& sl : e->pipe) {
    if (sl.pin) (void)hipHostFree(sl.pin);
    if (sl.dev) (void)hipFree(sl.dev);
    if (sl.h2d) (void)hipEventDestroy(sl.h2d);
    if (sl.done) (void)hipEventDestroy(sl.done);
    if (sl.d2h) (void)hipEventDestroy(sl.d2h);
  }
  e->pipe.clear();
  if (e->copy_stream) { (void)hipStreamDestroy(e->copy_stream); e->copy_stream = nullptr; }
  if (e->fetch_stream) { (void)hipStreamDestroy(e->fetch_stream); e->fetch_stream = nullptr; }
}

void pipeline_submit(mv_engine* e, const mv_inputs* in) {
  const mv_config& c = e->cfg;
  const size_t N = c.batch_size, T = c.obs_len;
  MV_REQUIRE(!e->pipe.empty(), "mv_pipeline_create has not been called");
  mv_engine::PipeSlot& sl = e->pipe[e->pipe_head % e->pipe.size()];
  MV_REQUIRE(!sl.busy, "pipeline full: %zu submissions not collected (mv_collect_greedy)",
             e->pipe.size());
  const bool scene = !e->no_scene();
  MV_REQUIRE(!scene || (in->obs_scene && in->scene_feat), "obs_scene / scene_feat is NULL");
  check_inputs(e, in->num_scene_frames, in->pred_len, in->obs_scene);
  const PipeLayout L = pipe_layout(e);
  char* pin = static_cast<char*>(sl.pin);
  const size_t sf_bytes = scene ? (size_t)in->num_scene_frames * c.scene_h * c.scene_w *
                                      c.scene_class * sizeof(float) : 0;
  if (scene) {
    memcpy(pin + L.obs_scene, in->obs_scene, N * T * sizeof(int32_t));
    memcpy(pin + L.scene_feat, in->scene_feat, sf_bytes);
  }
  for (int s = 0; s < c.num_scales; ++s) {
    ScaleState& S = e->sc[s];
    if (!S.use) continue;
    MV_REQUIRE(in->grid_obs_labels[s] && in->grid_obs_regress[s],
               "grid_obs_labels/grid_obs_regress[%d] is NULL for an enabled scale", s);
    check_labels(e, s, in->grid_obs_labels[s]);
    memcpy(pin + L.labels[s], in->grid_obs_labels[s], N * T * sizeof(int32_t));
    memcpy(pin + L.obs_reg[s], in->grid_obs_regress[s], N * T * S.K * 2 * sizeof(float));
  }
  MV_REQUIRE(!e->lens_set, "mv_submit_greedy: per-row prediction lengths are set "
             "(mv_set_pred_lengths); the pipelined forward is uniform -- clear them first");
  sl.num_frames = scene ? in->num_scene_frames : 0; sl.pred_len = in->pred_len;
  HIP_CHECK(hipMemcpyAsync(sl.dev, sl.pin, L.in_bytes, hipMemcpyHostToDevice, e->copy_stream));
  HIP_CHECK(hipEventRecord(sl.h2d, e->copy_stream));
  HIP_CHECK(hipStreamWaitEvent(e->stream, sl.h2d, 0));
  auto d2d = [&](void* dst, const void* src, size_t n) {
    HIP_CHECK(hipMemcpyAsync(dst, src, n, hipMemcpyDeviceToDevice, e->stream));
  };
  if (scene) {
    d2d(e->obs_scene.p, sl.dev + L.obs_scene, N * T * sizeof(int32_t));
    d2d(e->scene_feat.p, sl.dev + L.scene_feat, sf_bytes);
  }
  for (int s = 0; s < c.num_scales; ++s) {
    ScaleState& S = e->sc[s];
    if (!S.use) continue;
    d2d(S.labels.p, sl.dev + L.labels[s], N * T * sizeof(int32_t));
    d2d(S.obs_reg.p, sl.dev + L.obs_reg[s], N * T * S.K * 2 * sizeof(float));
  }
  e->num_frames = sl.num_frames;
  e->pred_len = sl.pred_len;
  e->inputs_ready = true;
  run_forward(e, ForwardKind::Greedy);
  const size_t Tp = sl.pred_len;
  for (int s = 0; s < c.num_scales; ++s) {
    ScaleState& S = e->sc[s];
    if (!S.use) continue;
    d2d(sl.dev + L.out_cls[s], S.out_cls.p, N * Tp * S.K * sizeof(float));
    d2d(sl.dev + L.out_reg[s], S.out_reg.p, N * Tp * S.K * 2 * sizeof(float));
  }
  HIP_CHECK(hipEventRecord(sl.done, e->stream));
  HIP_CHECK(hipStreamWaitEvent(e->fetch_stream, sl.done, 0));
  HIP_CHECK(hipMemcpyAsync(pin + L.in_bytes, sl.dev + L.in_bytes, L.out_bytes,
                           hipMemcpyDeviceToHost, e->fetch_stream));
  HIP_CHECK(hipEventRecord(sl.d2h, e->fetch_stream));
  sl.busy = true;
  e->pipe_head += 1;
}

void pipeline_collect(mv_engine* e, mv_outputs* out) {
  const mv_config& c = e->cfg;
  MV_REQUIRE(!e->pipe.empty(), "mv_pipeline_create has not been called");
  mv_engine::PipeSlot& sl = e->pipe[e->pipe_tail % e->pipe.size()];
  MV_REQUIRE(sl.busy, "mv_collect_greedy: nothing submitted");
  HIP_CHECK(hipEventSynchronize(sl.d2h));
  const PipeLayout L = pipe_layout(e);
  const char* pin = static_cast<const char*>(sl.pin);
  const size_t N = c.batch_size, Tp = sl.pred_len;
  for (int s = 0; s < c.num_scales; ++s) {
    ScaleState& S = e->sc[s];
    if (!S.use) continue;
    if (out->grid_pred_class[s])
      memcpy(out->grid_pred_class[s], pin + L.out_cls[s], N * Tp * S.K * sizeof(float));
    if (out->grid_pred_reg[s])
      memcpy(out->grid_pred_reg[s], pin + L.out_reg[s], N * Tp * S.K * 2 * sizeof(float));
  }
  sl.busy = false;
  e->pipe_tail += 1;
}

void download_beam(mv_engine* e, mv_beam_outputs* out) {
  const mv_config& c = e->cfg;
  const size_t N = c.batch_size, Tp = e->pred_len, B = c.beam_size;
  ScaleState& S = e->sc[beam_scale(e)];
  const size_t K = S.K;
  if (out->logits)
    HIP_CHECK(hipMemcpyAsync(out->logits, e->bm_out_logits.p, N * B * Tp * K * sizeof(float),
                             hipMemcpyDeviceToHost, e->stream));
  if (out->ids)
    HIP_CHECK(hipMemcpyAsync(out->ids, e->bm_out_ids.p, N * B * Tp * sizeof(int32_t),
                             hipMemcpyDeviceToHost, e->stream));
  if (out->logprobs)
    HIP_CHECK(hipMemcpyAsync(out->logprobs, e->bm_lp[0].p, N * B * sizeof(float),
                             hipMemcpyDeviceToHost, e->stream));
  if (out->grid_reg) {
    if (c.use_single_decoder)
      HIP_CHECK(hipMemcpyAsync(out->grid_reg, e->bm_out_reg.p,
                               N * B * Tp * K * 2 * sizeof(float), hipMemcpyDeviceToHost,
                               e->stream));
    else
    HIP_CHECK(hipMemcpyAsync(out->grid_reg, S.out_reg.p, N * Tp * K * 2 * sizeof(float),
                             hipMemcpyDeviceToHost, e->stream));
  }
  if (out->best_beam)
    HIP_CHECK(hipMemcpy2DAsync(out->best_beam, Tp * K * sizeof(float),
                               e->bm_out_logits.p, B * Tp * K * sizeof(float),
                               Tp * K * sizeof(float), N, hipMemcpyDeviceToHost,
                               e->stream));
  HIP_CHECK(hipStreamSynchronize(e->stream));
}

static void mf_require_forward(const mv_engine* e, const char* who) {
  const mv_config& c = e->cfg;
  MV_REQUIRE(!(c.beam_size > 1 && c.use_single_decoder),
             "%s: use_single_decoder with beam search decodes on the host (the offsets come "
             "per beam, and the reference's own reshape of them mixes beams)", who);
  MV_REQUIRE(e->last != ForwardKind::None, "%s: no forward has run on this handle", who);
  MV_REQUIRE(e->last_on_beams() == (c.beam_size > 1),
             "%s: the last forward of this beam handle was a greedy one", who);
}

// ... 203 lines not shown
```

multiverse_amd/csrc/engine_ops.h:

```cpp
#pragma once

extern "C" {


int mv_op_convlstm_step(int device, const float* x, const float* c, const float* h,
                        const float* kernel, const float* biases, int32_t M,
                        int32_t H, int32_t W, int32_t Cx, int32_t C, float* c_out,
                        float* h_out) {
  return guarded(nullptr, [&] {
    MV_REQUIRE(C % mv::kChBlock == 0 && C % mv::kBK == 0, "C %d must be a multiple of 32", C);
    MV_REQUIRE(mv::convlstm_cx_supported(Cx), "Cx %d unsupported (multiple of 32, or <= 3)", Cx);
    OpCtx ctx(device);
    const size_t cells = (size_t)M * H * W;
    DevBuf<float> dx, dc, dh, dw, db, dco, dho;
    ctx.up(dx, x, cells * Cx);
    ctx.up(db, biases, (size_t)4 * C);
    std::vector<float> packed(mv::convlstm_wpack_elems(Cx, C));
    mv::pack_convlstm_weights(kernel, Cx, C, packed.data());
    ctx.up(dw, packed.data(), packed.size());
    const bool zero = (c == nullptr && h == nullptr);
    if (!zero) {
      MV_REQUIRE(c && h, "c and h must both be given or both be NULL");
      ctx.up(dc, c, cells * C);
      ctx.up(dh, h, cells * C);
// ... 230 lines not shown
    ensure_beam_step_lds(device, lds);
    DevBuf<float> dl, dp, dn;
    DevBuf<int32_t> di, dpa;
    ctx.up(dl, logits, (size_t)N * B * K);
    ctx.up(dp, prev_logprob, (size_t)N * B);
    dn.alloc((size_t)N * B); di.alloc((size_t)N * B); dpa.alloc((size_t)N * B);
    DevBuf<float> dc;
    dc.alloc((size_t)N * B * K);
    launch_beam_step(ctx.stream, dl.p, dp.p, dc.p, N, B, K, time, diverse, logf(gamma),
                     fix_num_timestep, dn.p, di.p, dpa.p, (int32_t*)nullptr, B);
    ctx.down(new_logprob, dn, (size_t)N * B);
    ctx.down(ids, di, (size_t)N * B);
    ctx.down(parents, dpa, (size_t)N * B);
  });
}

int mv_op_sbs_step(int device, const float* logits, const float* prev_phi,
                   const float* prev_logprob, const float* prev_gumbel, int32_t N, int32_t B,
                   int32_t K, int32_t t, float temperature, uint32_t seed, float* new_phi,
                   float* new_logprob, float* new_gumbel, int32_t* ids, int32_t* parents) {
  return guarded(nullptr, [&] {
    MV_REQUIRE(N > 0 && B > 0 && K > 0 && t >= 0, "mv_op_sbs_step: N, B, K > 0 and t >= 0");
    MV_REQUIRE(temperature > 0.f, "mv_op_sbs_step: temperature %g must be > 0",
               (double)temperature);
    OpCtx ctx(device);
    ensure_beam_step_lds(device, ((size_t)2 * B * K + 512) * sizeof(float));
    const size_t R = (size_t)N * B;
    DevBuf<float> dl, dphi, dlp, dg, nphi, nlp, ng, cand, lpp, qp;
    DevBuf<int32_t> di, dpa;
    DevBuf<uint32_t> dprm;
    const uint32_t params[4] = {seed, __builtin_bit_cast(uint32_t, temperature), 0u,
                                __builtin_bit_cast(uint32_t, 1.f)};
    ctx.up(dl, logits, R * K);
    ctx.up(dphi, prev_phi, R); ctx.up(dlp, prev_logprob, R); ctx.up(dg, prev_gumbel, R);
    ctx.up(dprm, params, (size_t)4);
    nphi.alloc(R); nlp.alloc(R); ng.alloc(R); di.alloc(R); dpa.alloc(R);
    cand.alloc(R * K); lpp.alloc(R * K); qp.alloc(R * K);
    launch_sbs_step(ctx.stream, dl.p, dphi.p, dlp.p, dg.p, cand.p, lpp.p, qp.p, dprm.p, N, B, K,
                    t, nphi.p, nlp.p, ng.p, di.p, dpa.p, (int32_t*)nullptr, B);
    ctx.down(new_phi, nphi, R); ctx.down(new_logprob, nlp, R); ctx.down(new_gumbel, ng, R);
    ctx.down(ids, di, R); ctx.down(parents, dpa, R);
  });
}

int mv_op_sample_step(int device, const float* logits, int32_t R, int32_t S, int32_t K, int32_t t,
                      float temperature, uint32_t seed, int32_t top_k, float top_p, int32_t floor,
                      int32_t* ids, float* lp, float* qlp, uint8_t* keep) {
  return guarded(nullptr, [&] {
    MV_REQUIRE(R > 0 && S > 0 && K > 0 && t >= 0, "mv_op_sample_step: R, S, K > 0 and t >= 0");
    MV_REQUIRE(R % S == 0, "mv_op_sample_step: R = %d rows are not S = %d futures per sample",
               (int)R, (int)S);
    MV_REQUIRE(K <= 64 * mv::kBeamRankJ, "mv_op_sample_step: K = %d cells (one wave holds a row "
               "of at most %d)", (int)K, 64 * mv::kBeamRankJ);
    MV_REQUIRE(temperature > 0.f, "mv_op_sample_step: temperature %g must be > 0",
               (double)temperature);
    MV_REQUIRE(top_k >= 0, "mv_op_sample_step: top_k %d must be >= 0 (0 = off)", (int)top_k);
    MV_REQUIRE(top_p > 0.f && top_p <= 1.f, "mv_op_sample_step: top_p %g not in (0, 1] (1 = off)",
               (double)top_p);
    MV_REQUIRE(floor >= 1, "mv_op_sample_step: floor %d must be >= 1", (int)floor);
    OpCtx ctx(device);
    DevBuf<float> dl, dlp, dq;
    DevBuf<int32_t> di;
    DevBuf<uint8_t> dk;
    DevBuf<uint32_t> dprm;
    const uint32_t params[4] = {seed, __builtin_bit_cast(uint32_t, temperature), (uint32_t)top_k,
                                __builtin_bit_cast(uint32_t, top_p)};
    ctx.up(dl, logits, (size_t)R * K);
    ctx.up(dprm, params, (size_t)4);
    dlp.alloc(R); dq.alloc(R); di.alloc(R); dk.alloc((size_t)R * K);
    HIP_CHECK(hipMemsetAsync(dlp.p, 0, (size_t)R * sizeof(float), ctx.stream));
    HIP_CHECK(hipMemsetAsync(dq.p, 0, (size_t)R * sizeof(float), ctx.stream));
    const dim3 grid(cdiv((size_t)R, 4)), block(256);
    with_rank_j(K, [&](auto j) {
      hipLaunchKernelGGL(mv::sample_step_kernel<decltype(j)::value>, grid, block, 0, ctx.stream,
                         dl.p, (int64_t)K, R, S, K, t, 0, dprm.p, floor, (const int32_t*)nullptr,
                         dlp.p, dq.p, di.p, 1, (int32_t*)nullptr, dk.p);
    });
    HIP_CHECK(hipGetLastError());
    ctx.down(ids, di, R); ctx.down(lp, dlp, R); ctx.down(qlp, dq, R);
    ctx.down(keep, dk, (size_t)R * K);
  });
}

int mv_op_convlstm_bwd(int device, const float* x, const float* c, const float* h,
                       const float* kernel, const float* biases, const float* dh_new,
                       const float* dc_new, int32_t M, int32_t H, int32_t W, int32_t Cx,
                       int32_t C, float* dx, float* dh, float* dc, float* dkernel,
                       float* dbiases) {
  return guarded(nullptr, [&] {
    MV_REQUIRE(C % 128 == 0 && C <= 512, "convlstm_bwd: C 128, 256, 384 or 512");
    MV_REQUIRE(mv::convlstm_cx_supported(Cx), "Cx %d unsupported", Cx);
    OpCtx ctx(device);
    const size_t cells = (size_t)M * H * W;
    DevBuf<float> dx_, dc_, dh_, dw, db, dco, dho, dg, ddh, ddc, dwd, dxo, dho2, part, dW,
        dB, tmp;
    dx_.alloc(cells * Cx ? cells * Cx : 1, mv::kWgradPad);
    if (cells * Cx)
      HIP_CHECK(hipMemcpy(dx_.p, x, cells * Cx * sizeof(float), hipMemcpyHostToDevice));
    ctx.up(db, biases, (size_t)4 * C);
    std::vector<float> packed(mv::convlstm_wpack_elems(Cx, C));
    mv::pack_convlstm_weights(kernel, Cx, C, packed.data());
    ctx.up(dw, packed.data(), packed.size());
    std::vector<float> packedT(mv::convlstm_dgrad_wpack_elems(Cx, C));
    mv::pack_convlstm_dgrad_weights(kernel, Cx, C, packedT.data());
    ctx.up(dwd, packedT.data(), packedT.size());
    const bool zero = (c == nullptr && h == nullptr);
    dc_.alloc(cells * C); dh_.alloc(cells * C, mv::kWgradPad);
    if (!zero) {
      MV_REQUIRE(c && h, "c and h must both be given or both be NULL");
      HIP_CHECK(hipMemcpy(dc_.p, c, cells * C * sizeof(float), hipMemcpyHostToDevice));
      HIP_CHECK(hipMemcpy(dh_.p, h, cells * C * sizeof(float), hipMemcpyHostToDevice));
    } else {
      HIP_CHECK(hipMemset(dc_.p, 0, cells * C * sizeof(float)));
      HIP_CHECK(hipMemset(dh_.p, 0, cells * C * sizeof(float)));
    }
    dco.alloc(cells * C); dho.alloc(cells * C); dg.alloc(cells * 4 * C, mv::kWgradPad);
    ctx.up(ddh, dh_new, cells * C);
    ctx.up(ddc, dc_new, cells * C);
    mv::ConvLstmArgs a{};
    a.x = dx_.p; a.h = dh_.p; a.c = dc_.p; a.wpack = dw.p; a.bias = db.p;
    a.h_out = dho.p; a.c_out = dco.p; a.gates_out = dg.p;
    a.rows = M; a.H = H; a.W = W; a.Cx = Cx; a.C = C;
    mv::convlstm_finish_args(a, zero);
    mv::launch_convlstm_steps(&a, 1, ctx.stream);
    const size_t total = cells * C;
    hipLaunchKernelGGL(mv::lstm_gate_bwd_kernel, dim3(cdiv(total, 256)), dim3(256), 0,
                       ctx.stream, dg.p, dc_.p, dco.p, ddh.p, ddc.p, total, C);
    dxo.alloc(cells * (Cx ? Cx : 1)); dho2.alloc(cells * C);
    mv::ConvLstmArgs d{};
    mv::convlstm_dgrad_args(d, dg.p, dwd.p, dho2.p, dxo.p, M, H, W, Cx, C, true, Cx > 0);
    mv::launch_convlstm_dgrads(&d, 1, ctx.stream);
    const WgradPlan wpl = plan_wgrad(0, 3, M, H, W, Cx, C);
    mv::WgradArgs wa = wpl.fp32;
    wa.x = Cx ? dx_.p : nullptr; wa.h = dh_.p; wa.g = dg.p;
    part.alloc(wpl.partial_elems);
    wa.partial = part.p;
    mv::launch_convlstm_wgrad(wa, ctx.stream);
    const size_t ncols = (size_t)9 * (Cx + C) * 4 * C;
    dW.alloc(ncols);
    hipLaunchKernelGGL(mv::colsum_kernel, dim3(1, cdiv(ncols, 256)), dim3(256), 0,
                       ctx.stream, part.p, dW.p, (size_t)wa.nsplit, ncols,
                       (size_t)wa.nsplit);
    dB.alloc((size_t)4 * C);
    hipLaunchKernelGGL(mv::colsum_kernel, dim3(1, cdiv((size_t)4 * C, 256)), dim3(256), 0,
                       ctx.stream, dg.p, dB.p, cells, (size_t)4 * C, cells);
    {
      DevBuf<float> wsrc, p1, p2;
      ctx.up(wsrc, kernel, (size_t)9 * (Cx + C) * 4 * C);
      const int nx = mv::convlstm_xchunks(Cx), nch = nx + 9 * (C / mv::kBK);
      p1.alloc(packed.size()); p2.alloc(packedT.size());
      hipLaunchKernelGGL(mv::pack_fwd_kernel, dim3(cdiv(packed.size(), 256)), dim3(256), 0,
                         ctx.stream, wsrc.p, p1.p, Cx, C, nx, nch, x_is_small(Cx) ? 1 : 0,
                         packed.size());
      hipLaunchKernelGGL(mv::pack_dgrad_kernel, dim3(cdiv(packedT.size(), 256)), dim3(256),
                         0, ctx.stream, wsrc.p, p2.p, Cx, C, 9 * (4 * C / mv::kBK),
                         packedT.size());
      std::vector<float> c1(packed.size()), c2(packedT.size());
      ctx.down(c1.data(), p1, c1.size());
      ctx.down(c2.data(), p2, c2.size());
      MV_REQUIRE(memcmp(c1.data(), packed.data(), c1.size() * 4) == 0,
                 "device forward weight pack differs from the host pack");
      MV_REQUIRE(memcmp(c2.data(), packedT.data(), c2.size() * 4) == 0,
                 "device dgrad weight pack differs from the host pack");
    }
    HIP_CHECK(hipGetLastError());
    if (dx && Cx) ctx.down(dx, dxo, cells * Cx);
// ... 59 lines not shown
```

multiverse_amd/csrc/engine_setup.h:

```cpp
#pragma once

namespace {

inline unsigned cdiv(size_t a, size_t b) { return (unsigned)((a + b - 1) / b); }

void ensure_beam_step_lds(int device, size_t lds) {
  static std::mutex mu;
  static std::map<int, size_t> granted;
  std::lock_guard<std::mutex> lk(mu);
  MV_REQUIRE(lds <= 160 * 1024, "beam_size*K too large for the LDS beam step (%zu B)", lds);
  size_t& cur = granted[device];
  if (lds > cur) {
    HIP_CHECK(hipFuncSetAttribute(reinterpret_cast<const void*>(mv::beam_step_kernel),
                                  hipFuncAttributeMaxDynamicSharedMemorySize, (int)lds));
    HIP_CHECK(hipFuncSetAttribute(reinterpret_cast<const void*>(mv::beam_select_kernel),
                                  hipFuncAttributeMaxDynamicSharedMemorySize, (int)lds));
    HIP_CHECK(hipFuncSetAttribute(reinterpret_cast<const void*>(mv::sbs_select_kernel),
                                  hipFuncAttributeMaxDynamicSharedMemorySize, (int)lds));
    cur = lds;
  }
}

template <typename F>
void with_rank_j(int K, F&& fn) {
// ... 183 lines not shown
        e->decode_reg_W = e->add_param("person_pred/decode_reg/out_dec_grid/W", {3, 3, C, 2});
      S.out_reg_W = e->decode_reg_W;
      continue;
    }
    cell(S.dec_reg, "decoder_grid_reg_%d/decoder_rnn/dec_grid_reg_%d", E);
    snprintf(nm, sizeof(nm), "person_pred/decoder_grid_reg_%d/decoder_rnn/grid_emb/W", s);
    S.emb_reg_W = e->add_param(nm, {3, 3, 2, E});
    snprintf(nm, sizeof(nm), "person_pred/decoder_grid_reg_%d/decoder_rnn/grid_emb/b", s);
    S.emb_reg_b = e->add_param(nm, {E});
    snprintf(nm, sizeof(nm), "person_pred/hidden2grid_decoder_grid_reg_%d/out_dec_grid/W", s);
    S.out_reg_W = e->add_param(nm, {3, 3, C, 2});
  }
}

std::vector<ConvCell*> active_cells(const mv_engine* e, ScaleState& S) {
  if (e->cfg.use_single_decoder) return {&S.enc_cls, &S.dec_cls};
  return {&S.enc_cls, &S.enc_reg, &S.dec_cls, &S.dec_reg};
}

void validate_config(const mv_config& c) {
  MV_REQUIRE(c.abi_version == MV_ABI_VERSION, "mv_config.abi_version %d != %d",
             c.abi_version, MV_ABI_VERSION);
  MV_REQUIRE(c.activation >= 0 && c.activation <= 2, "mv_config.activation %d (0 tanh, 1 relu, "
             "2 lrelu; reference code/pred_utils.py:86-94)", c.activation);
  MV_REQUIRE(c.batch_size > 0 && c.obs_len > 0 && c.max_pred_len > 0,
             "batch_size/obs_len/max_pred_len must be positive");
  MV_REQUIRE(c.num_scales >= 1 && c.num_scales <= MV_MAX_SCALES,
             "num_scales %d not in [1,%d]", c.num_scales, MV_MAX_SCALES);
  MV_REQUIRE(c.hidden_size == 128 || c.hidden_size == 256 || c.hidden_size == 512,
             "hidden_size %d unsupported (128, 256 or 512)", c.hidden_size);
  MV_REQUIRE(c.convlstm_kernel >= 1 && c.convlstm_kernel <= 9,
             "convlstm_kernel %d unsupported (1 .. 9)", c.convlstm_kernel);
  MV_REQUIRE(c.scene_conv_dim == 0 ||
             (c.scene_conv_dim > 0 && c.scene_conv_dim <= 128 &&
              mv::convlstm_cx_supported(c.scene_conv_dim)),
             "scene_conv_dim %d unsupported (0 = no scene encoder, or a multiple of 32 up to "
             "128)", c.scene_conv_dim);
  MV_REQUIRE(c.emb_size >= 32 && c.emb_size % 32 == 0 && c.emb_size <= 512 &&
             mv::convlstm_cx_supported(c.emb_size),
             "emb_size %d unsupported (a multiple of 32 up to 512)", c.emb_size);
  MV_REQUIRE(c.beam_size >= 1, "beam_size must be >= 1");
  MV_REQUIRE(!(c.class_feedback_dense && c.beam_size > 1), "class_feedback_dense: greedy only "
             "(grid_decoder_beam_search always feeds one-hot ids)");
  int hh = c.scene_h, ww = c.scene_w, used = 0;
  for (int s = 0; s < c.num_scales; ++s) {
    hh = (hh + 1) / 2; ww = (ww + 1) / 2;
    MV_REQUIRE(c.grid_h[s] == hh && c.grid_w[s] == ww,
               "scene_grids[%d] = %dx%d does not match the stride-2 conv chain "
               "(%dx%d); only scene_grid_strides 2,4,.. are supported",
               s, c.grid_h[s], c.grid_w[s], hh, ww);
    used += c.use_grid[s] != 0;
  }
  MV_REQUIRE(used >= 1, "no grid scale enabled");
  if (c.beam_size > 1)
    MV_REQUIRE(used == 1, "beam search: only one scale at a time "
               "(reference pred_models.py:262)");
}

void alloc_buffers(mv_engine* e) {
  const mv_config& c = e->cfg;
  const size_t N = c.batch_size, T = c.obs_len, Tp = c.max_pred_len,
               C = c.hidden_size, D = c.scene_conv_dim, B = c.beam_size;
  const size_t maxU = N * T;
  const bool scene = !e->no_scene();
  e->obs_scene.alloc(N * T);
  e->lens_dev.alloc(N);
  if (scene) e->scene_feat.alloc(maxU * c.scene_h * c.scene_w * c.scene_class);
  int hh = c.scene_h, ww = c.scene_w;
  for (int i = 0; i < c.num_scales; ++i) {
    hh = (hh + 1) / 2; ww = (ww + 1) / 2;
    e->conv_h.push_back(hh); e->conv_w.push_back(ww);
    if (scene) e->scene_conv[i].alloc(maxU * hh * ww * D);
  }
  const size_t xc = (size_t)std::max((int)D, c.emb_size);
  for (int s = 0; s < c.num_scales; ++s) {
    ScaleState& S = e->sc[s];
    if (!S.use) continue;
    const size_t K = S.K, R = N * B;
    S.scene_mean.alloc(N * K * std::max<size_t>(D, 1));
    if (!scene) HIP_CHECK(hipMemset(S.scene_mean.p, 0, N * K * sizeof(float)));
    S.labels.alloc(N * T);
    S.obs_reg.alloc(N * T * K * 2);
    for (int i = 0; i < 2; ++i) {
      S.cls_c[i].alloc(R * K * C); S.cls_h[i].alloc(R * K * C);
      S.reg_c[i].alloc(N * K * C); S.reg_h[i].alloc(N * K * C);
    }
    if (c.use_gnn) S.cls_hg.alloc(R * K * C);
    S.xbuf_cls.alloc(R * K * xc);
    S.xbuf_reg.alloc(N * K * xc);
    S.out_cls.alloc(N * Tp * K);
    S.out_reg.alloc(N * Tp * K * 2);
    S.ids.alloc(R);
    S.q_cls.alloc(R * K * 9); S.q_reg.alloc((c.use_single_decoder ? R : N) * K * 18);
    S.wq_cls.alloc(C * 32); S.wq_reg.alloc(C * 32);
    S.sx_cellyx.alloc(K);
    S.sx_dec_bias.alloc(9 * 4 * C); S.sx_dec_corr.alloc(9 * 25 * 4 * C);
    if (scene) S.sx_enc_corr.alloc(T * N * 9 * 4 * C);
    else { S.sx_enc_bias.alloc(9 * 4 * C); S.sx_enc_tab.alloc(9 * 25 * 4 * C); }
    if (B > 1) {
      e->bm_logits.alloc(Tp * R * K);
      e->bm_ids.alloc(Tp * R);
      e->bm_parents.alloc(Tp * R);
      e->bm_lp[0].alloc(R); e->bm_lp[1].alloc(R);
      e->bm_lp_final.alloc(R);
      e->bm_cand.alloc((size_t)R * K);
      for (int i = 0; i < 2; ++i) { e->bm_phi[i].alloc(R); e->bm_g[i].alloc(R); }
      e->bm_g_final.alloc(R); e->bm_phi_final.alloc(R);
      e->lq_acc.alloc(R);
      e->bm_sbs_lp.alloc((size_t)R * K); e->bm_sbs_q.alloc((size_t)R * K);
      e->bm_src_row.alloc(R);
      e->bm_ref.alloc(R);
      e->bm_trace.alloc(R * Tp);
      e->bm_out_logits.alloc(R * Tp * K);
      e->bm_out_ids.alloc(R * Tp);
      if (c.use_single_decoder) {
        e->bm_reg_steps.alloc(Tp * R * K * 2);
        e->bm_out_reg.alloc(R * Tp * K * 2);
      }
    }
  }
}

void ensure_packed(mv_engine* e, ConvCell& cc) {
  MV_REQUIRE(cc.kernel->set, "parameter %s not set", cc.kernel->name.c_str());
  MV_REQUIRE(cc.biases->set, "parameter %s not set", cc.biases->name.c_str());
  if (cc.wpack.p) return;
  if (e->cfg.convlstm_kernel != 3) return;
  const int C = e->cfg.hidden_size;
  std::vector<float> packed(mv::convlstm_wpack_elems(cc.Cx, C));
  mv::pack_convlstm_weights(cc.kernel->host.data(), cc.Cx, C, packed.data());
  cc.wpack.alloc(packed.size());
  HIP_CHECK(hipMemcpy(cc.wpack.p, packed.data(), packed.size() * sizeof(float),
                      hipMemcpyHostToDevice));
}

CellPacks packs_of(const mv_engine* e, const ConvCell& cc) {
  return cell_packs(e->compute_mode, e->cfg.activation, cc.Cx, e->cfg.hidden_size,
                    cc.wino_numerics_ok);
}

std::vector<float> kernel_h_rows(const float* kernel, int Cx, int C) {
  const int Cin = Cx + C, N4 = 4 * C;
  std::vector<float> wh((size_t)9 * C * N4);
  for (int t = 0; t < 9; ++t)
    memcpy(&wh[(size_t)t * C * N4], &kernel[((size_t)t * Cin + Cx) * N4],
           (size_t)C * N4 * sizeof(float));
  return wh;
}
std::vector<float> small_x_chunk(const float* kernel, int Cx, int C, float scale) {
  std::vector<float> packed(mv::convlstm_wpack_elems(Cx, C));
  mv::pack_convlstm_weights(kernel, Cx, C, packed.data());
  const int nch = mv::convlstm_xchunks(Cx) + 9 * (C / mv::kBK);
  std::vector<float> wx((size_t)(C / mv::kChBlock) * mv::kBN * mv::kBK);
  for (int cb = 0; cb < C / mv::kChBlock; ++cb)
    for (int i = 0; i < mv::kBN * mv::kBK; ++i)
      wx[(size_t)cb * mv::kBN * mv::kBK + i] =
          packed[((size_t)cb * nch + 0) * mv::kBN * mv::kBK + i] * scale;
  return wx;
}
template <typename T>
void upload(DevBuf<T>& dst, const std::vector<T>& src) {
  dst.alloc(src.size());
  HIP_CHECK(hipMemcpy(dst.p, src.data(), src.size() * sizeof(T), hipMemcpyHostToDevice));
}
void refresh_host_copy(ConvCell& cc) {
  if (!cc.host_stale) return;
  HIP_CHECK(hipMemcpy(cc.kernel->host.data(), cc.kernel->dev.p,
// ... 44 lines not shown
    cc.wino_numerics_ok = ok;
  }
  std::vector<_Float16> p16(mv::f16x3_wpack_elems(x_chunk16(cc.Cx), C));
  if (x_is_small(cc.Cx)) {
    mv::pack_f16x3_weights(kernel_h_rows(cc.kernel->host.data(), cc.Cx, C).data(), 0, C, p16.data());
    upload(cc.wx32, small_x_chunk(cc.kernel->host.data(), cc.Cx, C, 65536.0f));
  } else {
    mv::pack_f16x3_weights(cc.kernel->host.data(), cc.Cx, C, p16.data());
  }
  upload(cc.wp16, p16);
}

void pack_wino(hipStream_t stream, const float* w, int Cx, int C, DevBuf<_Float16>& dst) {
  const size_t halves = mv::wino_wpack_elems(x_chunk16(Cx), C);
  mv::wino_init_attributes();
  dst.alloc(halves);
  hipLaunchKernelGGL(mv::pack_wino_kernel, dim3(cdiv(halves / 2, 256)), dim3(256), 0, stream, w,
                     dst.p, Cx, x_chunk16(Cx), C, halves / 2);
}
void pack_wino3(hipStream_t stream, const float* w, int Cx, int C, DevBuf<_Float16>& dst) {
  const size_t halves = mv::wino3_wpack_elems(x_chunk16(Cx), C, mv::kW3Nrb);
  mv::wino3_init_attributes();
  dst.alloc(halves);
  hipLaunchKernelGGL(mv::pack_wino3_kernel, dim3(cdiv(halves / 2, 256)), dim3(256), 0, stream, w,
                     dst.p, Cx, x_chunk16(Cx), C, mv::kW3Nrb, halves / 2);
}
void pack_bf16t(hipStream_t stream, const float* w, int Cx, int C, DevBuf<_Float16>& dst) {
  const size_t halves = mv::bf16t_wpack_elems(x_chunk16(Cx), C, mv::kW3Nrb);
  dst.alloc(halves);
  hipLaunchKernelGGL(mv::pack_bf16t_kernel, dim3(cdiv(halves, 256)), dim3(256), 0, stream, w,
                     dst.p, Cx, x_chunk16(Cx), C, mv::kW3Nrb, halves);
}
void pack_tile_forms(mv_engine* e, ConvCell& cc) {
  const CellPacks p = packs_of(e, cc);
  const int C = e->cfg.hidden_size;
  if (e->compute_mode == 1) {
    if (p.wpw) pack_wino(e->stream, cc.kernel->dev.p, cc.Cx, C, cc.wpw); else cc.wpw.release();
    if (p.wpw3) pack_wino3(e->stream, cc.kernel->dev.p, cc.Cx, C, cc.wpw3); else cc.wpw3.release();
  } else if (e->compute_mode == 2) {
    if (p.wpbt) pack_bf16t(e->stream, cc.kernel->dev.p, cc.Cx, C, cc.wpbt); else cc.wpbt.release();
  }
}

void ensure_packed_bf16(mv_engine* e, ConvCell& cc) {
  if (cc.wpb.p) return;
  const int C = e->cfg.hidden_size;
  MV_REQUIRE(mv::f16x3_cx_supported(cc.Cx), "bf16: Cx %d unsupported", cc.Cx);
  refresh_host_copy(cc);
  const bool xf16 = bf16_x_passes(2, e->dyn_x(), x_is_small(cc.Cx)) == 3;
  std::vector<_Float16> pb(mv::bf16_wpack_elems(x_chunk16(cc.Cx), C, xf16));
  if (x_is_small(cc.Cx)) {
    mv::pack_bf16_weights(kernel_h_rows(cc.kernel->host.data(), cc.Cx, C).data(), 0, C, pb.data());
    upload(cc.wx32u, small_x_chunk(cc.kernel->host.data(), cc.Cx, C, 1.0f));
  } else {
    if (xf16) {
      const int Cin = cc.Cx + C, N4 = 4 * C;
      float mx = 0.f;
      for (int t = 0; t < 9; ++t)
        for (int ci = 0; ci < cc.Cx; ++ci)
          for (int n = 0; n < N4; ++n)
            mx = std::max(mx, std::fabs(cc.kernel->host[((size_t)t * Cin + ci) * N4 + n]));
      MV_REQUIRE(mx * mv::kF16Scale < 60000.f, "bf16 mode, unbounded activations: the x rows of "
                 "%s reach %g, outside the scaled fp16 range; use compute mode f32",
                 cc.kernel->name.c_str(), mx);
    }
    mv::pack_bf16_weights(cc.kernel->host.data(), cc.Cx, C, pb.data(), xf16);
  }
  upload(cc.wpb, pb);
  pack_tile_forms(e, cc);
}

int gnn_scene_dim(const mv_engine* e) {
  return (e->cfg.simaug_graph && e->cfg.beam_size == 1) ? 0 : e->cfg.scene_conv_dim;
}

bool sparse_x_on(const mv_engine* e, const ScaleState& S) {
  static const bool off = getenv("MV_SPARSE_X") && atoi(getenv("MV_SPARSE_X")) == 0;
  const mv_config& c = e->cfg;
  return !off && e->compute_mode != 0 && !e->train && S.use && S.H >= 3 && S.W >= 3 &&
         S.dec_cls.Cx == c.emb_size && c.emb_size % 16 == 0 && c.scene_conv_dim % 16 == 0 &&
         c.scene_conv_dim <= 64;
}

void ensure_params(mv_engine* e) {
  for (auto& p : e->params)
    MV_REQUIRE(p->set, "parameter %s not set (mv_set_param)", p->name.c_str());
  for (int s = 0; s < e->cfg.num_scales; ++s) {
    ScaleState& S = e->sc[s];
    if (!S.use) continue;
    for (ConvCell* cc : active_cells(e, S)) ensure_packed(e, *cc);
    if (e->compute_mode == 1)
      for (ConvCell* cc : active_cells(e, S)) ensure_packed16(e, *cc);
    if (e->compute_mode == 1)
      for (ConvCell* cc : active_cells(e, S))
        if (packs_of(e, *cc).wpw && !cc->wpw.p) pack_tile_forms(e, *cc);
    if (e->compute_mode == 2)
      for (ConvCell* cc : active_cells(e, S)) ensure_packed_bf16(e, *cc);
    if (!S.wq_valid) {
      const int C = e->cfg.hidden_size;
      hipLaunchKernelGGL(mv::pack_h2g_kernel, dim3(cdiv((size_t)C * 32, 256)), dim3(256), 0,
                         e->stream, S.out_cls_W->dev.p, S.wq_cls.p, C, 1);
      hipLaunchKernelGGL(mv::pack_h2g_kernel, dim3(cdiv((size_t)C * 32, 256)), dim3(256), 0,
                         e->stream, S.out_reg_W->dev.p, S.wq_reg.p, C, 2);
      S.wq_valid = true;
    }
    if (!S.sx_valid && sparse_x_on(e, S)) {
      const int C = e->cfg.hidden_size;
      hipLaunchKernelGGL(mv::cell_yx_kernel, dim3(cdiv((size_t)S.K, 256)), dim3(256), 0,
                         e->stream, S.sx_cellyx.p, S.H, S.W);
      hipLaunchKernelGGL(mv::sx_decoder_tables_kernel,
                         dim3(cdiv((size_t)(9 + 9 * 25) * 4 * C, 256)), dim3(256), 0, e->stream,
                         S.dec_cls.kernel->dev.p, S.dec_cls.biases->dev.p, S.emb_cls_W->dev.p,
                         S.emb_cls_b->dev.p, S.dec_cls.Cx, C, S.sx_dec_bias.p, S.sx_dec_corr.p,
                         e->cfg.activation);
      if (e->no_scene())
        hipLaunchKernelGGL(mv::sx_decoder_tables_kernel,
                           dim3(cdiv((size_t)(9 + 9 * 25) * 4 * C, 256)), dim3(256), 0,
                           e->stream, S.enc_cls.kernel->dev.p, S.enc_cls.biases->dev.p,
                           e->enc_emb_W->dev.p, e->enc_emb_b->dev.p, S.enc_cls.Cx, C,
                           S.sx_enc_bias.p, S.sx_enc_tab.p, e->cfg.activation);
      S.sx_valid = true;
    }
  }
}

}
```

multiverse_amd/csrc/engine_state.h:

```cpp
#pragma once

struct mv_train_holder;

namespace {

thread_local std::string g_create_error;



struct HipError { std::string msg; };

#define HIP_CHECK(expr)                                                       \
  do {                                                                        \
    hipError_t _e = (expr);                                                   \
    if (_e != hipSuccess) {                                                   \
      char _b[512];                                                           \
      snprintf(_b, sizeof(_b), "%s failed: %s (%s:%d)", #expr,                \
               hipGetErrorString(_e), __FILE__, __LINE__);                    \
      throw HipError{_b};                                                     \
    }                                                                         \
  } while (0)

#define MV_REQUIRE(cond, ...)                                                 \
  do {                                                                        \
// ... 36 lines not shown
  bool no_grad = false;
  size_t elems() const {
    size_t e = 1;
    for (auto d : shape) e *= (size_t)d;
    return e;
  }
};

struct ConvCell {
  Param* kernel = nullptr;
  Param* biases = nullptr;
  DevBuf<float> wpack;
  DevBuf<_Float16> wp16;
  DevBuf<float> wx32;
  DevBuf<_Float16> wpb;
  DevBuf<float> wx32u;
  DevBuf<_Float16> wpw;
  DevBuf<_Float16> wpw3;
  DevBuf<_Float16> wpbt;
  bool host_stale = false;
  bool wino_numerics_ok = true;
  int Cx = 0;
};
constexpr float kWinoOutlierRatio = 4096.f;

struct KernelStat {
  std::string name;
  int64_t launches = 0;
  double total_ms = 0, flops = 0, bytes = 0, flops_dense = 0;
  double flops_mfma = 0;
};

struct PendingEvent {
  int stat;
  hipEvent_t a, b;
};

enum class ForwardKind { None, Greedy, Beam, Sampled, Scored, SampledWor };

struct LengthPlan {
  bool ragged = false;
  int steps = 0;
  std::vector<int> act_rows;
  void reset() { ragged = false; steps = 0; }
  void build(const std::vector<int32_t>& L, int pred_len) {
    act_rows.assign((size_t)pred_len + 1, 0);
    steps = 0;
    for (int n = 0; n < (int)L.size(); ++n) {
      for (int t = 0; t < L[n]; ++t) act_rows[t] = n + 1;
      steps = std::max(steps, (int)L[n]);
    }
    ragged = true;
  }
  int rows_at(int t, int batch) const {
    if (!ragged) return batch;
    return t < (int)act_rows.size() ? act_rows[t] : 0;
  }
};

struct ScaleState {
  int H = 0, W = 0, K = 0;
  bool use = false;
  ConvCell enc_cls, enc_reg, dec_cls, dec_reg;
  Param *emb_cls_W = nullptr, *emb_cls_b = nullptr, *emb_reg_W = nullptr,
        *emb_reg_b = nullptr, *out_cls_W = nullptr, *out_reg_W = nullptr;
  DevBuf<float> scene_mean;
  DevBuf<int32_t> labels;
  DevBuf<float> obs_reg;
  DevBuf<double> centers;
  DevBuf<float> cls_c[2], cls_h[2], cls_hg;
  DevBuf<float> reg_c[2], reg_h[2];
  DevBuf<float> xbuf_cls, xbuf_reg;
  DevBuf<float> out_cls;
  DevBuf<float> out_reg;
  DevBuf<int32_t> ids;
  DevBuf<float> q_cls, q_reg;
  DevBuf<float> wq_cls, wq_reg;
  bool wq_valid = false;
  DevBuf<uint32_t> sx_cellyx;
  DevBuf<float> sx_dec_bias, sx_dec_corr;
  DevBuf<float> sx_enc_corr;
  DevBuf<float> sx_enc_bias, sx_enc_tab;
  bool sx_valid = false;
};

}

struct mv_engine {
  mv_config cfg{};
  int device = 0;
  hipStream_t stream = nullptr;
  hipStream_t stream_b = nullptr;
  hipEvent_t fork_ev = nullptr, join_ev = nullptr;
  hipStream_t issue = nullptr;
  int slot0 = 0;
  std::string err;
  std::vector<std::unique_ptr<Param>> params;
  Param* decode_reg_W = nullptr;
  std::map<std::string, Param*> by_name;
  std::vector<Param*> scene_W, scene_b;
  Param *enc_emb_W = nullptr, *enc_emb_b = nullptr;
  bool no_scene() const { return cfg.scene_conv_dim == 0; }
  ScaleState sc[MV_MAX_SCALES];
  DevBuf<int32_t> obs_scene;
  DevBuf<float> scene_feat;
  DevBuf<uint8_t> scene_u8;
  DevBuf<double> xy_dev;
  DevBuf<float> scene_conv[MV_MAX_SCALES];
  std::vector<int> conv_h, conv_w;
  int num_frames = 0;
  int pred_len = 0;
  bool inputs_ready = false;
  std::vector<int32_t> lens_host;
  DevBuf<int32_t> lens_dev;
  bool lens_set = false;
  LengthPlan len;
  int rows_at(int t) const { return len.rows_at(t, cfg.batch_size); }
  int64_t gate_rows = 0;
  std::map<std::tuple<ForwardKind, int, int>, int64_t> graph_gate_rows;
  DevBuf<float> bm_logits;
  DevBuf<int32_t> bm_ids, bm_parents;
  DevBuf<float> bm_lp[2];
  DevBuf<float> bm_lp_final;
  DevBuf<float> bm_cand;
  DevBuf<float> bm_phi[2], bm_g[2];
  DevBuf<float> bm_g_final;
  DevBuf<float> bm_phi_final;
  DevBuf<float> bm_sbs_lp, bm_sbs_q;
  DevBuf<int32_t> bm_src_row;
  DevBuf<int32_t> bm_ref;
  DevBuf<int32_t> bm_trace;
  DevBuf<float> bm_out_logits;
  DevBuf<float> bm_reg_steps;
  DevBuf<float> bm_out_reg;
  DevBuf<int32_t> bm_out_ids;
  bool sampling = false;
  int sampling_mode = 0;
  int32_t samp_top_k = 0;
  float samp_top_p = 1.f;
  DevBuf<uint32_t> samp_params;
  DevBuf<float> lq_acc;
  bool score_ready = false;
  int score_pred_len = 0;
  bool score_uniform = true;
  std::vector<int32_t> score_L;
  DevBuf<int32_t> score_ids;
  DevBuf<int32_t> score_len;
  DevBuf<float> score_step_lp;
  DevBuf<int32_t> score_rank;
  ForwardKind last = ForwardKind::None;
  bool last_on_beams() const { return last != ForwardKind::None && last != ForwardKind::Greedy; }
  DevBuf<double> mf_traj;
  DevBuf<float> mf_occ;
  int compute_mode = 0;
  DevBuf<_Float16> px16[mv::kMaxGroup], ph16[mv::kMaxGroup];
  DevBuf<_Float16> pv3x[mv::kMaxGroup], pv3h[mv::kMaxGroup];
  DevBuf<int32_t> xexp[mv::kMaxGroup];
  std::set<const float*> xbufs;
  bool dyn_x() const { return compute_mode != 0 && cfg.activation != 0; }
  struct PlaneBuf { _Float16* p; size_t n; bool valid; };
  std::map<const float*, PlaneBuf> planes;
  std::vector<std::unique_ptr<DevBuf<_Float16>>> plane_store;
  _Float16* plane_out(const float* dst, size_t* stride) {
    if (compute_mode == 0) return nullptr;
    if (dyn_x() && xbufs.count(dst)) return nullptr;
    auto it = planes.find(dst);
// ... 51 lines not shown
```

multiverse_amd/csrc/gate_plan.h:

```cpp
#pragma once

namespace {

struct GateKnobs {
  bool wino, wino3, bf16t, wino_dgrad;
  int wino_map_f23;
  int wino_map_f33;
  int wino_map_bf16t;
  bool conv_shift;
  int conv_map;
  bool epi_planes;
  int dgrad_kslices;
  bool transpose3;
  bool bf16_bwd;
  bool bf16_fused_split;
  bool wgrad_splits_set; int wgrad_splits;
  bool wgrad_wide;
  int wgrad_wide_map;
  int wgrad_wide_splits;
  bool wgrad_wide_x;
  bool wgrad_wino, wgrad_wino_bf16;
  int wgrad_x_splits;
};

inline const GateKnobs& gate_knobs() {
  static const GateKnobs k = [] {
    auto num = [](const char* name, int unset) {
      const char* v = getenv(name);
      return v ? atoi(v) : unset;
    };
    auto on = [&](const char* name) { return num(name, 1) != 0; };
    GateKnobs g{};
    g.wino = on("MV_WINO"); g.wino3 = on("MV_WINO3"); g.bf16t = on("MV_BF16T");
    g.wino_dgrad = on("MV_WINO_DGRAD");
    g.wino_map_f23 = num("MV_WINO_MAP", 1);
    g.wino_map_f33 = num("MV_WINO_MAP", 2);
    g.wino_map_bf16t = num("MV_WINO_MAP", 2);
    g.conv_shift = on("MV_CONV_SHIFT");
    g.conv_map = num("MV_CONV_MAP", 0);
    g.epi_planes = on("MV_EPI_PLANES");
    g.dgrad_kslices = num("MV_DGRAD_KSLICES", 0);
    g.transpose3 = on("MV_TRANSPOSE3");
    g.bf16_bwd = on("MV_BF16_BWD");
    g.bf16_fused_split = on("MV_BF16_FUSED_SPLIT");
    g.wgrad_splits_set = getenv("MV_WGRAD_SPLITS") != nullptr;
    g.wgrad_splits = num("MV_WGRAD_SPLITS", 0);
    g.wgrad_wide = on("MV_WGRAD_WIDE");
    g.wgrad_wide_map = num("MV_WGRAD_WIDE_MAP", 0);
    g.wgrad_wide_splits = num("MV_WGRAD_WIDE_SPLITS", 0);
    g.wgrad_wide_x = num("MV_WGRAD_WIDE_X", 0) == 1;
    g.wgrad_wino = on("MV_WGRAD_WINO"); g.wgrad_wino_bf16 = on("MV_WGRAD_WINO_BF16");
    g.wgrad_x_splits = num("MV_WGRAD_X_SPLITS", 12);
    return g;
  }();
  return k;
}

inline bool x_is_small(int Cx) { return Cx > 0 && 9 * Cx <= mv::kBK; }
inline int x_chunk16(int Cx) { return x_is_small(Cx) ? 0 : Cx; }
inline int bf16_x_passes(int mode, bool dyn_x, bool x_small) {
  return (mode == 2 && dyn_x && !x_small) ? 3 : 1;
}

struct CellPacks {
  bool wp16, wpw, wpw3;
  bool wpb, wpbt;
  bool wd16, wdw, wdb;
};
inline CellPacks cell_packs(int mode, int activation, int Cx, int C, bool wino_numerics_ok) {
  const GateKnobs& k = gate_knobs();
  const bool blocks_ok = C % mv::kWnCh == 0 && (Cx % 16 == 0 || x_is_small(Cx));
  CellPacks p{};
  p.wp16 = mode == 1;
  p.wpw = mode == 1 && k.wino && blocks_ok && wino_numerics_ok;
  p.wpw3 = p.wpw && k.wino3;
  p.wpb = mode == 2;
  p.wpbt = mode == 2 && k.bf16t && blocks_ok && activation == 0;
  p.wdb = mode == 2 && k.bf16_bwd;
  p.wd16 = mode != 0 && !p.wdb;
  p.wdw = p.wd16 && mode == 1 && k.wino && k.wino_dgrad;
  return p;
}

inline size_t wino3_scratch_elems(int rows, int H, int W, int Cc) {
  return H < 3 ? 0 : mv::wino3_v_elems(rows, H, W, (Cc + 15) / 16 * 16);
}
inline bool wino3_possible(int mode, int activation) {
  return mode == 1 && gate_knobs().wino && gate_knobs().wino3 && activation == 0;
}

enum class GateForm { Direct16, Wino2, Wino3, Bf16, Bf16T };
struct ForwardPlan {
  GateForm form = GateForm::Direct16;
  bool halo = false;
  bool shift = false;
  int map_mode = 0;
  int x_passes = 1;
  double mfma_factor = 3.0;
};
struct ForwardProblem {
  const mv::ConvLstm16Args* q;
  const ConvCell* cell;
  size_t v3x_cap, v3h_cap;
};
inline bool has_dense_x(const mv::ConvLstmArgs& a) { return !a.x_small && a.Cx > 0 && !a.sx_corr; }

inline ForwardPlan plan_forward_group(int mode, const ForwardProblem* p, int n) {
  const GateKnobs& k = gate_knobs();
  ForwardPlan pl;
  bool halo = false, halo_ok = true, shift = k.conv_shift, x_exp = false;
  for (int i = 0; i < n; ++i) {
    const mv::ConvLstmArgs& a = p[i].q->f;
    halo = halo || mv::wino3_needs_halo(a);
    halo_ok = halo_ok && mv::wino3_halo_addressable(a);
    shift = shift && a.W > 0 && 32 % a.W == 0;
    x_exp = x_exp || p[i].q->x_exp != nullptr;
  }
  const bool tile3_ok = !halo || halo_ok;
  bool wino = mode == 1 && k.wino, wino3 = wino && k.wino3 && tile3_ok;
  bool bf16t = mode == 2 && k.bf16t && tile3_ok;
  for (int i = 0; i < n; ++i) {
    const mv::ConvLstm16Args& q = *p[i].q;
    const mv::ConvLstmArgs& a = q.f;
    wino = wino && mv::wino_geometry_ok(a) && p[i].cell->wpw.p;
    wino3 = wino3 && mv::wino3_geometry_ok(a, q) && p[i].cell->wpw3.p &&
            (a.zero_state || p[i].v3h_cap >= wino3_scratch_elems(a.rows, a.H, a.W, a.C)) &&
            (!has_dense_x(a) || p[i].v3x_cap >= wino3_scratch_elems(a.rows, a.H, a.W, a.Cx));
    bf16t = bf16t && mv::bf16t_geometry_ok(a, q) && p[i].cell->wpbt.p;
  }
  pl.shift = shift;
  pl.map_mode = k.conv_map;
  if (mode == 2) {
    pl.form = bf16t ? GateForm::Bf16T : GateForm::Bf16;
    pl.mfma_factor = 1.0;
    if (bf16t) { pl.halo = halo; pl.map_mode = k.wino_map_bf16t; }
    else pl.x_passes = x_exp ? 3 : 1;
    return pl;
  }
  if (!wino && !wino3) return pl;
  pl.form = wino3 ? GateForm::Wino3 : GateForm::Wino2;
  pl.halo = wino3 && halo;
  pl.map_mode = wino3 ? k.wino_map_f33 : k.wino_map_f23;
  double num = 0, den = 0;
  for (int i = 0; i < n; ++i) {
    const mv::ConvLstmArgs& a = p[i].q->f;
    const double cx = a.sx_corr ? 0.0 : (double)a.Cx;
    const double fl = (double)a.rows * a.H * a.W * (cx + (a.zero_state ? 0 : a.C));
    const double per = wino3 ? 5.0 * ((a.H + 2) / 3) / a.H * (mv::wino3_needs_halo(a) ? 32.0 / 30.0 : 1.0)
                             : 4.0 * ((a.H + 1) / 2) / a.H;
    num += fl * per; den += fl;
  }
  pl.mfma_factor = den > 0 ? num / den : (wino3 ? 5.0 / 3.0 : 2.0);
  return pl;
}

struct DgradPlan {
  bool bf16 = false;
  bool wino = false;
  bool shift = false;
  double mfma_factor = 3.0;
  struct Slices { int nks_main, nks_x, n_kslice; } s[mv::kMaxGroup];
};
inline bool wino_dgrad_geometry_ok(const mv::ConvLstmArgs& a) {
  return a.W > 0 && 32 % a.W == 0 && a.H >= 2 && a.out0_cols % 64 == 0 && (a.C / 16) % 8 == 0;
}
inline DgradPlan plan_dgrad_group(int mode, const mv::ConvLstmArgs* probs, const bool* has_wdw,
                                  int n) {
  const GateKnobs& k = gate_knobs();
  DgradPlan pl;
  pl.bf16 = mode == 2 && k.bf16_bwd;
  pl.wino = mode == 1 && k.wino && k.wino_dgrad;
  pl.shift = k.conv_shift;
  for (int i = 0; i < n; ++i) {
    pl.wino = pl.wino && wino_dgrad_geometry_ok(probs[i]) && has_wdw[i];
    pl.shift = pl.shift && probs[i].W > 0 && 32 % probs[i].W == 0;
  }
  pl.mfma_factor = pl.wino ? 2.0 : (pl.bf16 ? 1.0 : 3.0);
  for (int i = 0; i < n; ++i) {
    const mv::ConvLstmArgs& a = probs[i];
    DgradPlan::Slices& s = pl.s[i];
    s = DgradPlan::Slices{0, 0, 0};
    if (pl.wino) {
      const int ncm = a.out0_cols / 64;
      int nkm = std::max(1, 8 / ncm);
      while ((a.C / 16) % nkm != 0) nkm /= 2;
      s.nks_main = nkm;
      s.nks_x = (a.out1 && a.out1_cols > 0) ? 8 : 1;
      continue;
    }
    const int nstages = 9 * (a.C / 16) / 3;
    const int ks = k.dgrad_kslices > 0 ? k.dgrad_kslices : (pl.bf16 ? 1 : 4);
    if (pl.bf16)
      MV_REQUIRE(nstages % MV_BF16_UNITS == 0, "internal: bf16 dgrad stage count %d", nstages);
    if (ks > 1 && nstages % (2 * ks) == 0) s.n_kslice = ks;
  }
  return pl;
}

struct WgradPlan {
  bool generic = false;
  bool f16 = false;
  bool one = false;
  bool wino = false;
  bool wide = false;
  bool wide_x = false;
  bool transpose3 = true;
  int map_mode = 0;
  int nsplit = 0;
  int nsplit_x = 0;
  int ntaps = 9;
  long long Mtot = 0, Mrow = 0;
  long long Mtot3 = 0, Mrow3 = 0;
  long long Mgemm = 0;
  double mfma_factor = 1.0;
  size_t partial_elems = 0;
  mv::WgradArgs fp32{};
};
inline WgradPlan plan_wgrad(int mode, int ksize, int R, int H, int W, int Cx, int C) {
  const GateKnobs& k = gate_knobs();
  WgradPlan pl;
  pl.Mtot = (long long)R * H * W;
  pl.Mrow = (pl.Mtot + 63) / 64 * 64;
  pl.Mtot3 = pl.Mtot / 3;
  pl.Mrow3 = (pl.Mtot3 + 63) / 64 * 64;
  pl.Mgemm = pl.Mtot;
  if (ksize != 3) { pl.generic = true; pl.mfma_factor = 0.0; return pl; }
  mv::WgradArgs& wa = pl.fp32;
  wa.R = R; wa.H = H; wa.W = W; wa.Cx = Cx; wa.C = C;
  mv::wgrad_plan(wa, 3072, k.wgrad_splits_set ? &k.wgrad_splits : nullptr);
  pl.nsplit = pl.nsplit_x = wa.nsplit;
  pl.partial_elems = mv::wgrad_partial_elems(wa);
  pl.f16 = mode != 0 && mv::wgrad16_ok(W, C);
  if (!pl.f16) return pl;
  pl.one = mode == 2 && k.bf16_bwd;
  pl.wino = k.wgrad_wino && (k.wgrad_wino_bf16 || !pl.one) && mv::wgrad16_wino3_ok(H);
  pl.transpose3 = k.transpose3;
// ... 16 lines not shown
```

Baseline: 4322 trajectories/sec.

## Restrict class-encoder ConvLSTM steps to the light cone of observed cells

Adds a host-built per-timestep list of Winograd F(3,3) tiles that can differ from a shared background row, derived from each trajectory's observed grid cells dilated by the receptive field over time. The class encoder then computes gates and transforms only for the listed tiles. Unlisted tiles read a shared extra background row that holds the state of an all-background input. This skips encoder work on grid regions that have not yet been reached by any observation. In exchange it adds one extra row to the state buffers, host-side cone construction and upload per batch, and geometry restrictions (W=32, H divisible by 3, wino3 path only).

```diff
diff --git a/include/multiverse_hip.h b/include/multiverse_hip.h
--- a/include/multiverse_hip.h
+++ b/include/multiverse_hip.h
@@ -246,6 +246,9 @@
                        float top_p, int32_t floor, int32_t* ids, float* lp, float* qlp,
                        uint8_t* keep );
 
+int  mv_enc_cone_build(const int32_t* labels, int32_t N, int32_t T, int32_t H, int32_t W,
+                       int32_t r0, int32_t* lists, int64_t* cells);
+
 int  mv_op_convlstm_bwd(int device, const float* x, const float* c, const float* h,
                         const float* kernel, const float* biases,
                         const float* dh_new, const float* dc_new, int32_t M,
diff --git a/multiverse_amd/_lib.py b/multiverse_amd/_lib.py
--- a/multiverse_amd/_lib.py
+++ b/multiverse_amd/_lib.py
@@ -40,6 +40,7 @@
     "mv_download_scores", "mv_time_score_resident",
     "mv_set_sampling_mode", "mv_download_beam_gumbels", "mv_op_sbs_step",
     "mv_set_sampling_truncation", "mv_download_beam_proposal_logprobs", "mv_op_sample_step",
+    "mv_enc_cone_build",
 ]
 
 
@@ -220,6 +221,8 @@
   lib.mv_op_sample_step.argtypes = [C.c_int, _fp, C.c_int32, C.c_int32, C.c_int32, C.c_int32,
                                     C.c_float, C.c_uint32, C.c_int32, C.c_float, C.c_int32,
                                     _ip, _fp, _fp, _u8p]
+  if hasattr(lib, "mv_enc_cone_build"):
+    lib.mv_enc_cone_build.argtypes = [_ip] + [C.c_int32] * 5 + [_ip, C.POINTER(C.c_int64)]
   lib.mv_op_sbs_step.argtypes = [C.c_int, _fp, _fp, _fp, _fp, C.c_int32, C.c_int32, C.c_int32,
                                  C.c_int32, C.c_float, C.c_uint32, _fp, _fp, _fp, _ip, _ip]
   lib.mv_score_futures.argtypes = [h, C.POINTER(mv_inputs), C.POINTER(mv_score_futures_in),
@@ -1157,6 +1160,22 @@
   return phi, lp, g, ids, parents
 
 
+def enc_cone_build(labels, H, W, r0=1):
+  lib = load()
+  labels = np.ascontiguousarray(labels, dtype=np.int32)
+  N, T = labels.shape
+  ip = lambda a: a.ctypes.data_as(_ip)
+  ntile = lib.mv_enc_cone_build(None, N, T, int(H), int(W), int(r0), None, None)
+  if ntile < 0:
+    raise MvError("mv_enc_cone_build: bad arguments")
+  lists = np.zeros((T, 4 + 2 * ntile), np.int32)
+  cells = np.zeros((T,), np.int64)
+  if lib.mv_enc_cone_build(ip(labels), N, T, int(H), int(W), int(r0), ip(lists),
+                           cells.ctypes.data_as(C.POINTER(C.c_int64))) < 0:
+    raise MvError("mv_enc_cone_build: a label is not a cell of the %d x %d grid" % (H, W))
+  return lists, cells, int(ntile)
+
+
 def op_sample_step(logits, S, t, temperature=1.0, seed=0, top_k=0, top_p=1.0, floor=1, device=0):
   lib = load()
   logits = f32(logits)
diff --git a/multiverse_amd/csrc/convlstm_mfma.h b/multiverse_amd/csrc/convlstm_mfma.h
--- a/multiverse_amd/csrc/convlstm_mfma.h
+++ b/multiverse_amd/csrc/convlstm_mfma.h
@@ -47,6 +47,10 @@
   const int32_t* sx_hot;
   const uint32_t* sx_cellyx;
   int32_t sx_hot_stride, sx_hot_div, sx_rad, sx_by_class;
+  const int32_t* cone_list;
+  const int32_t* cone_prev;
+  int32_t cone_on;
+  int32_t cone_cells;
 };
 
 struct ConvLstmGroup {
diff --git a/multiverse_amd/csrc/convlstm_wino3.h b/multiverse_amd/csrc/convlstm_wino3.h
--- a/multiverse_amd/csrc/convlstm_wino3.h
+++ b/multiverse_amd/csrc/convlstm_wino3.h
@@ -88,6 +88,9 @@
   _Float16* out;
   const int32_t* src_row;
   int32_t rows, H, W, Cc;
+  const int32_t* cone_list;
+  const int32_t* cone_prev;
+  int32_t cone_cells;
 };
 constexpr int kW3TrGroup = 8;
 struct Wn3TransformGroup {
@@ -118,7 +121,12 @@
   const int ntile = (Q_total + 31) >> 5;
   const int wid = block * 4 + wave;
   if (wid >= ntile * KG) return;
-  const int tile = wid / KG, cg = wid - tile * KG;
+  int tile = wid / KG;
+  const int cg = wid - tile * KG;
+  if (it.cone_list) {
+    if (tile >= it.cone_list[0]) return;
+    tile = it.cone_list[4 + tile];
+  }
   const int col = lane & 31, half = lane >> 5;
   const int q = tile * 32 + col;
   const bool valid = q < Q_total;
@@ -131,12 +139,20 @@
     xpos = pc - t * W;
   }
   const int sr = (valid && it.src_row) ? it.src_row[r] : r;
+  int sr_up = sr, sr_mid = sr, sr_dn = sr;
+  if (it.cone_prev && valid) {
+    const int bg = it.rows - 1;
+    const int* prev = it.cone_prev;
+    sr_mid = prev[q >> 5] ? sr : bg;
+    sr_up = (y0 > 0 && !prev[(q - W) >> 5]) ? bg : sr;
+    sr_dn = (y0 + 3 < H && !prev[(q + W) >> 5]) ? bg : sr;
+  }
   f16x8 dh[5], dl[5];
 #pragma unroll
   for (int i = 0; i < 5; ++i) {
     const int rho = y0 - 1 + i;
     const bool ok = valid & (rho >= 0) & (rho < H);
-    const long long m = (long long)sr * HW + rho * W + xpos;
+    const long long m = (long long)(i == 0 ? sr_up : (i == 4 ? sr_dn : sr_mid)) * HW + rho * W + xpos;
     const size_t o = ((size_t)(m >> 5) * KG + cg) * 512 + (size_t)(half * 256 + (int)(m & 31) * 8);
     const f16x8 z = {0, 0, 0, 0, 0, 0, 0, 0};
     dh[i] = ok ? *reinterpret_cast<const f16x8*>(it.p0 + o) : z;
@@ -198,7 +214,16 @@
   const int H = a.H, W = a.W, HW = H * W, C = a.C, Cx = a.Cx;
   const int Ht = (H + 2) / 3, Kt = Ht * W;
   const int Q_total = a.rows * Kt;
-  const int q_own = mt * kTriples + wave * kOwn;
+  int q_own = mt * kTriples + wave * kOwn;
+  constexpr bool kCone = !HALO && !BF16D;
+  bool cone_bg_src = false;
+  if (kCone && a.cone_list) {
+    const int cnt = a.cone_list[0];
+    if (mt * WAVES >= cnt) return;
+    const int li = mt * WAVES + wave;
+    q_own = li < cnt ? 32 * a.cone_list[4 + li] : Q_total;
+  }
+  if (kCone && a.cone_prev && q_own < Q_total) cone_bg_src = a.cone_prev[q_own >> 5] == 0;
   const int q_wave = HALO ? q_own - 1 : q_own;
   const bool wave_live = q_own < Q_total;
   const int col = lane & 31, half = lane >> 5;
@@ -259,7 +284,7 @@
     cell[e] = (y0 + e) * W + xpos;
   }
   if (wave_live) {
-    const int src_c0 = (valid && a.src_row_c) ? a.src_row_c[r] : r;
+    const int src_c0 = cone_bg_src ? a.rows - 1 : ((valid && a.src_row_c) ? a.src_row_c[r] : r);
 #pragma unroll
     for (int e = 0; e < 3; ++e) {
       otab[e * 32 + col] = okc[e] ? (uint32_t)(src_c0 * HW + cell[e]) * rowb : kNone;
@@ -533,8 +558,9 @@
         cprev[e][rb] = *reinterpret_cast<const f32x4*>(tl0 + wr_idx + e * 32 * CH + rb * 8);
   }
   int hot_y = 0, hot_x = 0;
+  const bool bg_row = kCone && a.cone_on && r == a.rows - 1;
   if (a.sx_corr) {
-    const int hr = a.sx_hot_div > 1 ? r / a.sx_hot_div : r;
+    const int hr = bg_row ? 0 : (a.sx_hot_div > 1 ? r / a.sx_hot_div : r);
     const uint32_t hyx = a.sx_cellyx[a.sx_hot[(size_t)hr * a.sx_hot_stride]];
     hot_y = (int)(hyx >> 16); hot_x = (int)(hyx & 0xffffu);
   }
@@ -561,14 +587,14 @@
           add[g] = *reinterpret_cast<const f32x4*>(bsrc + g * C + ch);
         if (a.sx_corr) {
           const int dy = y - hot_y, dxh = xpos - hot_x, rad = a.sx_rad;
-          const bool inr = okc[e] && dy >= -rad && dy <= rad && dxh >= -rad && dxh <= rad;
+          const bool inr = okc[e] && !bg_row && dy >= -rad && dy <= rad && dxh >= -rad && dxh <= rad;
           const int dyc = dy < -rad ? -rad : (dy > rad ? rad : dy);
           const int dxc = dxh < -rad ? -rad : (dxh > rad ? rad : dxh);
           const int side = 2 * rad + 1;
           const int idx = a.sx_by_class
                               ? 3 * (hot_y == 0 ? 0 : (hot_y == H - 1 ? 2 : 1)) +
                                     (hot_x == 0 ? 0 : (hot_x == W - 1 ? 2 : 1))
-                              : (valid ? r : 0);
+                              : ((valid && !bg_row) ? r : 0);
           const float* ct = a.sx_corr +
               ((size_t)idx * side * side + (dyc + rad) * side + (dxc + rad)) * 4 * C + ch;
           const float keep = inr ? 1.0f : 0.0f;
diff --git a/multiverse_amd/csrc/engine.hip b/multiverse_amd/csrc/engine.hip
--- a/multiverse_amd/csrc/engine.hip
+++ b/multiverse_amd/csrc/engine.hip
@@ -879,7 +879,7 @@
       for (int i = 0; i < mv::kMaxGroup; ++i) {
         const size_t rows = (size_t)c.batch_size * ((i % 2 == 0) ? c.beam_size : 1);
         h->px16[i].alloc(2 * (rows * K * xc + mv::kPlaneSlack + mv::kPlanePad));
-        h->ph16[i].alloc(2 * (rows * K * c.hidden_size + mv::kPlaneSlack + mv::kPlanePad));
+        h->ph16[i].alloc(2 * ((rows + 1) * K * c.hidden_size + mv::kPlaneSlack + mv::kPlanePad));
         HIP_CHECK(hipMemset(h->px16[i].p, 0, h->px16[i].n * sizeof(_Float16)));
         if (c.activation != 0) h->xexp[i].alloc(65);
         if (wino3_possible(mode, c.activation)) {
@@ -887,7 +887,7 @@
           for (int s = 0; s < c.num_scales; ++s) {
             if (!h->sc[s].use) continue;
             vx = std::max(vx, wino3_scratch_elems((int)rows, h->sc[s].H, h->sc[s].W, (int)xc));
-            vh = std::max(vh, wino3_scratch_elems((int)rows, h->sc[s].H, h->sc[s].W, c.hidden_size));
+            vh = std::max(vh, wino3_scratch_elems((int)rows + 1, h->sc[s].H, h->sc[s].W, c.hidden_size));
           }
           if (vx) h->pv3x[i].alloc(vx);
           if (vh) h->pv3h[i].alloc(vh);
diff --git a/multiverse_amd/csrc/engine_forward.h b/multiverse_amd/csrc/engine_forward.h
--- a/multiverse_amd/csrc/engine_forward.h
+++ b/multiverse_amd/csrc/engine_forward.h
@@ -167,7 +167,8 @@
 
 double queue_wino3_transform(std::vector<mv::Wn3TransformItem>& tr, const mv::Wn3TransformItem& it) {
   tr.push_back(it);
-  return (double)it.rows * it.H * it.W * it.Cc * 4.0 * (1.0 + 5.0 / 3.0);
+  const double cells = it.cone_cells ? (double)it.cone_cells : (double)it.rows * it.H * it.W;
+  return cells * it.Cc * 4.0 * (1.0 + 5.0 / 3.0);
 }
 
 void launch_gate_group(const ForwardPlan& pl, const mv::ConvLstm16Args* p16,
@@ -204,8 +205,9 @@
                      double& dense) {
   flops = bytes = dense = 0;
   for (const auto& a : probs) {
-    const double M = (double)a.rows * a.H * a.W;
-    dense += 2.0 * M * 9.0 * (a.Cx + a.C) * 4.0 * a.C;
+    const double Md = (double)(a.rows - (a.cone_on ? 1 : 0)) * a.H * a.W;
+    const double M = a.cone_cells ? (double)a.cone_cells : (double)a.rows * a.H * a.W;
+    dense += 2.0 * Md * 9.0 * (a.Cx + a.C) * 4.0 * a.C;
     const double cx = a.sx_corr ? 0.0 : (double)a.Cx;
     flops += 2.0 * M * 9.0 * (cx + (a.zero_state ? 0 : a.C)) * 4.0 * a.C;
     bytes += M * (cx + (a.zero_state ? 2.0 : 4.0) * a.C) * 4.0;
@@ -235,7 +237,9 @@
       const int sl = groups[g]->slot0 + i;
       fp[n++] = ForwardProblem{&groups[g]->p16[i], groups[g]->cells[i], e->pv3x[sl].n, e->pv3h[sl].n};
     }
-  return plan_forward_group(e->compute_mode, fp, n);
+  const ForwardPlan pl = plan_forward_group(e->compute_mode, fp, n);
+  check_cone_plan(pl, fp, n);
+  return pl;
 }
 
 void issue_gate_group(mv_engine* e, const GatePrep& g, const ForwardPlan& pl) {
@@ -257,7 +261,8 @@
     if (!a.zero_state) {
       v3h[i] = e->pv3h[sl].p;
       tr3_bytes += queue_wino3_transform(tr3, {q.h16, q.h_plane_stride, v3h[i], a.src_row_h,
-                                               a.rows, a.H, a.W, a.C});
+                                               a.rows, a.H, a.W, a.C, a.cone_list, a.cone_prev,
+                                               a.cone_cells});
     }
     if (has_dense_x(a)) {
       v3x[i] = e->pv3x[sl].p;
@@ -269,7 +274,8 @@
     launch(e, "wino3_transform", 0, tr3_bytes, [&] {
       mv::launch_wino3_transforms(tr3.data(), (int)tr3.size(), e->issue);
     });
-  for (int i = 0; i < n; ++i) e->gate_rows += g.p16[i].f.rows;
+  for (int i = 0; i < n; ++i)
+    e->gate_rows += g.p16[i].f.rows - (g.p16[i].f.cone_on ? 1 : 0);
   launch(e, "convlstm_step", g.flops, g.bytes, [&] {
     launch_gate_group(pl, g.p16.data(), packs, w_hwio, v3x, v3h, n, e->issue);
   }, g.dense, pl.mfma_factor);
@@ -430,10 +436,22 @@
       });
       }
       const int cc = cur.cls[s];
+      const bool cone = sparse && enc_cone_on(e, S);
       probs.push_back(conv_problem(e, S.enc_cls, S.xbuf_cls.p, S.cls_h[cc].p,
                                    S.cls_c[cc].p, nullptr, nullptr, S.cls_h[cc ^ 1].p,
-                                   S.cls_c[cc ^ 1].p, N, S.H, S.W, t == 0, 0,
+                                   S.cls_c[cc ^ 1].p, N + (cone ? 1 : 0), S.H, S.W, t == 0, 0,
                                    t + 1 < T || !c.use_gnn));
+      if (cone) {
+        ConvLstmArgs& a = probs.back();
+        const size_t stride = enc_cone_step_elems(Nb + 1, S.H, S.W);
+        const int ntile = enc_cone_tiles(Nb + 1, S.H, S.W);
+        a.cone_on = 1;
+        a.cone_list = (t > 0 && t + 1 < T) ? S.cone.p + (size_t)t * stride : nullptr;
+        a.cone_prev = t > 1 ? S.cone.p + (size_t)(t - 1) * stride + 4 + ntile : nullptr;
+        MV_REQUIRE(S.cone_cells[t] > 0 && S.cone_cells[t] <= (int64_t)(N + 1) * S.H * S.W,
+                   "internal: cone cell count %lld", (long long)S.cone_cells[t]);
+        a.cone_cells = (int32_t)S.cone_cells[t];
+      }
       probs.back().skip_h32 =
           (t + 1 < T || (!c.use_gnn && (c.beam_size == 1 || beam_shared_first()))) ? 1 : 0;
       if (sparse && e->no_scene()) {
diff --git a/multiverse_amd/csrc/engine_io.h b/multiverse_amd/csrc/engine_io.h
--- a/multiverse_amd/csrc/engine_io.h
+++ b/multiverse_amd/csrc/engine_io.h
@@ -24,6 +24,76 @@
   for (size_t i = 0; i < NT; ++i)
     MV_REQUIRE(labels[i] >= 0 && labels[i] < K,
                "grid_obs_labels[%d][%zu] = %d out of range [0,%d)", s, i, labels[i], K);
+}
+
+void build_enc_cone(const int32_t* labels, int N, int T, int H, int W, int r0, int32_t* out,
+                    int64_t* cells) {
+  const int Ht = (H + 2) / 3, Kt = Ht * W, Q = (N + 1) * Kt;
+  const int ntile = enc_cone_tiles(N + 1, H, W);
+  const size_t stride = enc_cone_step_elems(N + 1, H, W);
+  const uint32_t wmask = W >= 32 ? 0xffffffffu : ((1u << W) - 1u);
+  std::vector<uint32_t> dirty((size_t)N * H, 0u), tmp(H);
+  for (int t = 0; t < T; ++t) {
+    int32_t* blk = out + (size_t)t * stride;
+    int32_t* list = blk + 4;
+    int32_t* flag = blk + 4 + ntile;
+    const bool all = t == 0 || t == T - 1;
+    for (int g = 0; g < ntile; ++g) flag[g] = all ? 1 : 0;
+    if (!all)
+      for (int q = N * Kt; q < Q; ++q) flag[q >> 5] = 1;
+    for (int n = 0; n < N; ++n) {
+      uint32_t* d = &dirty[(size_t)n * H];
+      for (int k = 0; k < Ht; ++k) {
+        uint32_t m = 0;
+        for (int y = std::max(3 * k - 1, 0); y <= std::min(3 * k + 3, H - 1); ++y) m |= d[y];
+        m = (m | (m << 1) | (m >> 1)) & wmask;
+        for (int y = 3 * k; y < std::min(3 * k + 3, H); ++y) tmp[y] = m;
+      }
+      const int cell = labels[(size_t)n * T + t], ys = cell / W, xs = cell % W;
+      uint32_t xm = 0;
+      for (int x = std::max(xs - r0, 0); x <= std::min(xs + r0, W - 1); ++x) xm |= 1u << x;
+      for (int y = 0; y < H; ++y) d[y] = tmp[y] | ((y >= ys - r0 && y <= ys + r0) ? xm : 0u);
+      if (all) continue;
+      for (int k = 0; k < Ht; ++k) {
+        uint32_t m = 0;
+        for (int y = 3 * k; y < std::min(3 * k + 3, H); ++y) m |= d[y];
+        for (int x = 0; m; ++x, m >>= 1)
+          if (m & 1u) flag[(n * Kt + k * W + x) >> 5] = 1;
+      }
+    }
+    int cnt = 0;
+    int64_t nc = 0;
+    for (int g = 0; g < ntile; ++g) {
+      if (!flag[g]) continue;
+      list[cnt++] = g;
+      for (int q = 32 * g; q < std::min(32 * g + 32, Q); ++q)
+        nc += std::min(3, H - 3 * ((q % Kt) / W));
+    }
+    for (int g = cnt; g < ntile; ++g) list[g] = 0;
+    blk[0] = cnt; blk[1] = blk[2] = blk[3] = 0;
+    if (cells) cells[t] = nc;
+  }
+}
+
+bool enc_cone_wanted(const mv_engine* e, const ScaleState& S) {
+  return S.use && enc_cone_geometry(e->cfg.obs_len, S.H, S.W, e->cfg.batch_size);
+}
+size_t enc_cone_elems(const mv_engine* e, const ScaleState& S) {
+  return (size_t)e->cfg.obs_len * enc_cone_step_elems(e->cfg.batch_size + 1, S.H, S.W);
+}
+void build_scale_cone(mv_engine* e, ScaleState& S, const int32_t* labels, int32_t* dst) {
+  S.cone_cells.assign(e->cfg.obs_len, 0);
+  build_enc_cone(labels, e->cfg.batch_size, e->cfg.obs_len, S.H, S.W, e->no_scene() ? 2 : 1, dst,
+                 S.cone_cells.data());
+  S.cone_ready = true;
+}
+void upload_scale_cone(mv_engine* e, ScaleState& S, const int32_t* labels) {
+  if (!enc_cone_wanted(e, S)) return;
+  S.cone_host.resize(enc_cone_elems(e, S));
+  S.cone.alloc(S.cone_host.size());
+  build_scale_cone(e, S, labels, S.cone_host.data());
+  HIP_CHECK(hipMemcpyAsync(S.cone.p, S.cone_host.data(), S.cone_host.size() * sizeof(int32_t),
+                           hipMemcpyHostToDevice, e->stream));
 }
 
 void upload_inputs(mv_engine* e, const mv_inputs* in) {
@@ -50,6 +120,7 @@
     check_labels(e, s, in->grid_obs_labels[s]);
     HIP_CHECK(hipMemcpyAsync(S.labels.p, in->grid_obs_labels[s],
                              N * T * sizeof(int32_t), hipMemcpyHostToDevice, e->stream));
+    upload_scale_cone(e, S, in->grid_obs_labels[s]);
     HIP_CHECK(hipMemcpyAsync(S.obs_reg.p, in->grid_obs_regress[s],
                              N * T * S.K * 2 * sizeof(float), hipMemcpyHostToDevice,
                              e->stream));
@@ -88,6 +159,7 @@
     check_labels(e, s, in->grid_obs_labels[s]);
     HIP_CHECK(hipMemcpyAsync(S.labels.p, in->grid_obs_labels[s],
                              N * T * sizeof(int32_t), hipMemcpyHostToDevice, e->stream));
+    upload_scale_cone(e, S, in->grid_obs_labels[s]);
     hipLaunchKernelGGL(mv::regress_from_xy_kernel, dim3(cdiv(N * T * S.K, 256)), dim3(256), 0,
                        e->stream, e->xy_dev.p, S.centers.p, S.obs_reg.p, (int)(N * T), (int)T,
                        S.K, in->num_rows);
@@ -116,7 +188,7 @@
 
 struct PipeLayout {
   size_t obs_scene = 0, scene_feat = 0, labels[MV_MAX_SCALES] = {0, 0},
-         obs_reg[MV_MAX_SCALES] = {0, 0}, in_bytes = 0;
+         obs_reg[MV_MAX_SCALES] = {0, 0}, cone[MV_MAX_SCALES] = {0, 0}, in_bytes = 0;
   size_t out_cls[MV_MAX_SCALES] = {0, 0}, out_reg[MV_MAX_SCALES] = {0, 0}, out_bytes = 0;
 };
 static PipeLayout pipe_layout(const mv_engine* e) {
@@ -133,6 +205,8 @@
     const size_t K = e->sc[s].K;
     L.labels[s] = o; o = al(o + N * T * sizeof(int32_t));
     L.obs_reg[s] = o; o = al(o + N * T * K * 2 * sizeof(float));
+    L.cone[s] = o;
+    if (enc_cone_wanted(e, e->sc[s])) o = al(o + enc_cone_elems(e, e->sc[s]) * sizeof(int32_t));
   }
   L.in_bytes = o;
   for (int s = 0; s < c.num_scales; ++s) {
@@ -203,6 +277,8 @@
     check_labels(e, s, in->grid_obs_labels[s]);
     memcpy(pin + L.labels[s], in->grid_obs_labels[s], N * T * sizeof(int32_t));
     memcpy(pin + L.obs_reg[s], in->grid_obs_regress[s], N * T * S.K * 2 * sizeof(float));
+    if (enc_cone_wanted(e, S))
+      build_scale_cone(e, S, in->grid_obs_labels[s], reinterpret_cast<int32_t*>(pin + L.cone[s]));
   }
   MV_REQUIRE(!e->lens_set, "mv_submit_greedy: per-row prediction lengths are set "
              "(mv_set_pred_lengths); the pipelined forward is uniform -- clear them first");
@@ -222,6 +298,10 @@
     if (!S.use) continue;
     d2d(S.labels.p, sl.dev + L.labels[s], N * T * sizeof(int32_t));
     d2d(S.obs_reg.p, sl.dev + L.obs_reg[s], N * T * S.K * 2 * sizeof(float));
+    if (enc_cone_wanted(e, S)) {
+      S.cone.alloc(enc_cone_elems(e, S));
+      d2d(S.cone.p, sl.dev + L.cone[s], enc_cone_elems(e, S) * sizeof(int32_t));
+    }
   }
   e->num_frames = sl.num_frames;
   e->pred_len = sl.pred_len;
diff --git a/multiverse_amd/csrc/engine_ops.h b/multiverse_amd/csrc/engine_ops.h
--- a/multiverse_amd/csrc/engine_ops.h
+++ b/multiverse_amd/csrc/engine_ops.h
@@ -336,6 +336,18 @@
   });
 }
 
+int mv_enc_cone_build(const int32_t* labels, int32_t N, int32_t T, int32_t H, int32_t W,
+                      int32_t r0, int32_t* lists, int64_t* cells) {
+  if (N <= 0 || T <= 0 || H <= 0 || W <= 0 || W > 32 || r0 < 0) return -1;
+  if (lists) {
+    if (!labels) return -1;
+    for (size_t i = 0; i < (size_t)N * T; ++i)
+      if (labels[i] < 0 || labels[i] >= H * W) return -1;
+    build_enc_cone(labels, N, T, H, W, r0, lists, cells);
+  }
+  return enc_cone_tiles(N + 1, H, W);
+}
+
 int mv_op_convlstm_bwd(int device, const float* x, const float* c, const float* h,
                        const float* kernel, const float* biases, const float* dh_new,
                        const float* dc_new, int32_t M, int32_t H, int32_t W, int32_t Cx,
diff --git a/multiverse_amd/csrc/engine_setup.h b/multiverse_amd/csrc/engine_setup.h
--- a/multiverse_amd/csrc/engine_setup.h
+++ b/multiverse_amd/csrc/engine_setup.h
@@ -289,7 +289,7 @@
     S.labels.alloc(N * T);
     S.obs_reg.alloc(N * T * K * 2);
     for (int i = 0; i < 2; ++i) {
-      S.cls_c[i].alloc(R * K * C); S.cls_h[i].alloc(R * K * C);
+      S.cls_c[i].alloc((R + 1) * K * C); S.cls_h[i].alloc((R + 1) * K * C);
       S.reg_c[i].alloc(N * K * C); S.reg_h[i].alloc(N * K * C);
     }
     if (c.use_gnn) S.cls_hg.alloc(R * K * C);
@@ -500,6 +500,21 @@
          c.scene_conv_dim <= 64;
 }
 
+bool enc_cone_on(mv_engine* e, ScaleState& S) {
+  const mv_config& c = e->cfg;
+  bool step_exact = true;
+  for (int s = 0; s < c.num_scales; ++s) {
+    ScaleState& O = e->sc[s];
+    if (!O.use) continue;
+    step_exact = step_exact &&
+                 cone_step_member_ok(O.H, O.W, O.enc_cls.wpw3.p &&
+                                                   (c.use_single_decoder || O.enc_reg.wpw3.p));
+  }
+  return S.cone_ready && S.cone.p && e->rows_at(0) == c.batch_size &&
+         enc_cone_planned(e->compute_mode, c.activation, sparse_x_on(e, S), step_exact, c.obs_len,
+                          S.H, S.W, c.hidden_size, c.batch_size);
+}
+
 void ensure_params(mv_engine* e) {
   for (auto& p : e->params)
     MV_REQUIRE(p->set, "parameter %s not set (mv_set_param)", p->name.c_str());
diff --git a/multiverse_amd/csrc/engine_state.h b/multiverse_amd/csrc/engine_state.h
--- a/multiverse_amd/csrc/engine_state.h
+++ b/multiverse_amd/csrc/engine_state.h
@@ -142,6 +142,10 @@
   DevBuf<float> sx_enc_corr;
   DevBuf<float> sx_enc_bias, sx_enc_tab;
   bool sx_valid = false;
+  DevBuf<int32_t> cone;
+  std::vector<int32_t> cone_host;
+  std::vector<int64_t> cone_cells;
+  bool cone_ready = false;
 };
 
 }
diff --git a/multiverse_amd/csrc/gate_plan.h b/multiverse_amd/csrc/gate_plan.h
--- a/multiverse_amd/csrc/gate_plan.h
+++ b/multiverse_amd/csrc/gate_plan.h
@@ -21,6 +21,7 @@
   bool wgrad_wide_x;
   bool wgrad_wino, wgrad_wino_bf16;
   int wgrad_x_splits;
+  int enc_cone;
 };
 
 inline const GateKnobs& gate_knobs() {
@@ -51,6 +52,7 @@
     g.wgrad_wide_x = num("MV_WGRAD_WIDE_X", 0) == 1;
     g.wgrad_wino = on("MV_WGRAD_WINO"); g.wgrad_wino_bf16 = on("MV_WGRAD_WINO_BF16");
     g.wgrad_x_splits = num("MV_WGRAD_X_SPLITS", 12);
+    g.enc_cone = num("MV_ENC_CONE", 1);
     return g;
   }();
   return k;
@@ -89,6 +91,25 @@
   return mode == 1 && gate_knobs().wino && gate_knobs().wino3 && activation == 0;
 }
 
+constexpr int kEncConeMinBatch = 16;
+inline bool enc_cone_geometry(int obs_len, int H, int W, int batch) {
+  const int k = gate_knobs().enc_cone;
+  return k != 0 && (k == 2 || batch >= kEncConeMinBatch) && obs_len >= 3 && H % 3 == 0 &&
+         H / 3 >= 5 && W == 32;
+}
+inline bool cone_step_member_ok(int H, int W, bool has_packs) {
+  return H >= 3 && W > 0 && 32 % W == 0 && has_packs;
+}
+inline bool enc_cone_planned(int mode, int activation, bool sparse, bool step_exact, int obs_len,
+                             int H, int W, int C, int batch) {
+  return enc_cone_geometry(obs_len, H, W, batch) && sparse && step_exact &&
+         wino3_possible(mode, activation) && C % mv::kWnCh == 0;
+}
+inline int enc_cone_tiles(int rows, int H, int W) { return (rows * ((H + 2) / 3) * W + 31) / 32; }
+inline size_t enc_cone_step_elems(int rows, int H, int W) {
+  return 4 + 2 * (size_t)enc_cone_tiles(rows, H, W);
+}
+
 enum class GateForm { Direct16, Wino2, Wino3, Bf16, Bf16T };
 struct ForwardPlan {
   GateForm form = GateForm::Direct16;
@@ -152,6 +173,11 @@
   }
   pl.mfma_factor = den > 0 ? num / den : (wino3 ? 5.0 / 3.0 : 2.0);
   return pl;
+}
+inline void check_cone_plan(const ForwardPlan& pl, const ForwardProblem* p, int n) {
+  for (int i = 0; i < n; ++i)
+    MV_REQUIRE(!p[i].q->f.cone_on || (pl.form == GateForm::Wino3 && !pl.halo),
+               "internal: a coned class-encoder step was planned outside the exact F(3,3) tiling");
 }
 
 struct DgradPlan {
```

Result: faster. 4381 trajectories/sec (median of 6 runs) (+1.4%).
